# RichExplor/VIL_Fusion

Measured on AMD Instinct MI355X. Metric: sliding-window solve iters/sec (10 KF, ~5.5k factors) @1/2/4/8 GPU vs CPU, higher is better.
Workload: dtype f64

## Files before the change

### vil_fusion_amd/csrc/vilf_api.hip

```cpp
#include <hip/hip_runtime.h>
#include <string>
#include <vector>
#include <cstring>
#include <cstdio>
#include <cmath>
#include <algorithm>
#include <chrono>
#include <cstdlib>
#include <thread>
#include <atomic>
#include <type_traits>
#include "vilf_internal.hpp"
#include "vilf_kernels.hpp"
#include "vilf_sort.hpp"

namespace {

int class_plan(const vilf_window_in &in, int *cls, int *cstart, int *ccount) {
    int pcount[VB_NPAIR] = {0};
    for (int f = 0; f < in.n_features; f++) {
        const int s = in.feature_start_frame[f], n = in.feature_obs_offset[f + 1] - in.feature_obs_offset[f];
        for (int k = 1; k < n; k++) { const int j = s + k; pcount[j * (j - 1) / 2 + s]++; }
    }
    int order[VB_NPAIR], load[4] = {0, 0, 0, 0};
    for (int p = 0; p < VB_NPAIR; p++) order[p] = p;
    std::stable_sort(order, order + VB_NPAIR, [&](int a, int b) { return pcount[a] > pcount[b]; });
    for (int k = 0; k < VB_NPAIR; k++) { const int p = order[k]; int best = 0; for (int c = 1; c < 4; c++) if (load[c] < load[best]) best = c; cls[p] = best; load[best] += pcount[p]; }
    int pos[4] = {0, 0, 0, 0};
    for (int p = 0; p < VB_NPAIR; p++) { cstart[p] = pos[cls[p]]; ccount[p] = pcount[p]; pos[cls[p]] += pcount[p]; }
    const int longest = std::max(std::max(pos[0], pos[1]), std::max(pos[2], pos[3]));
    return VB_CHUNK * std::max(1, (longest + VB_CLS - 1) / VB_CLS);
}

void quat_from_R(const double *m, double *q ) {
    double t = m[0] + m[4] + m[8];
    if (t > 0) {
        t = std::sqrt(t + 1.0); q[3] = 0.5 * t; t = 0.5 / t;
        q[0] = (m[7] - m[5]) * t; q[1] = (m[2] - m[6]) * t; q[2] = (m[3] - m[1]) * t;
    } else {
        int i = 0;
        if (m[4] > m[0]) i = 1;
        if (m[8] > m[4 * i]) i = 2;
        int j = (i + 1) % 3, k = (j + 1) % 3;
        t = std::sqrt(m[4 * i] - m[4 * j] - m[4 * k] + 1.0);
        q[i] = 0.5 * t; t = 0.5 / t;
        q[3] = (m[3 * k + j] - m[3 * j + k]) * t;
        q[j] = (m[3 * j + i] + m[3 * i + j]) * t;
        q[k] = (m[3 * k + i] + m[3 * i + k]) * t;
    }
}
void quat_to_R(const double *q, double *R) {
    const double x = q[0], y = q[1], z = q[2], w = q[3];
    const double tx = 2 * x, ty = 2 * y, tz = 2 * z, twx = tx * w, twy = ty * w, twz = tz * w;
    const double txx = tx * x, txy = ty * x, txz = tz * x, tyy = ty * y, tyz = tz * y, tzz = tz * z;
    R[0] = 1 - (tyy + tzz); R[1] = txy - twz; R[2] = txz + twy;
    R[3] = txy + twz; R[4] = 1 - (txx + tzz); R[5] = tyz - twx;
    R[6] = txz - twy; R[7] = tyz + twx; R[8] = 1 - (txx + tyy);
}

}

struct UpJob { const char *src; char *dst; unsigned long long bytes; };
struct UpJobs { int n; UpJob j[40]; };
__global__ __launch_bounds__(256) void k_copy_spans(UpJobs jobs) {
    const UpJob jb = jobs.j[blockIdx.y];
    const unsigned long long stride = (unsigned long long)gridDim.x * 256, i0 = (unsigned long long)blockIdx.x * 256 + threadIdx.x;
    if ((((unsigned long long)jb.src | (unsigned long long)jb.dst) & 15ull) == 0) {
        const unsigned long long n16 = jb.bytes >> 4;
        const uint4 *s4 = reinterpret_cast<const uint4 *>(jb.src); uint4 *d4 = reinterpret_cast<uint4 *>(jb.dst);
        for (unsigned long long i = i0; i < n16; i += stride) d4[i] = s4[i];
        if (blockIdx.x == 0) for (unsigned long long i = (n16 << 4) + threadIdx.x; i < jb.bytes; i += 256) jb.dst[i] = jb.src[i];
    } else if ((((unsigned long long)jb.src | (unsigned long long)jb.dst) & 7ull) == 0) {
        const unsigned long long n8 = jb.bytes >> 3;
        const unsigned long long *s8 = reinterpret_cast<const unsigned long long *>(jb.src); unsigned long long *d8 = reinterpret_cast<unsigned long long *>(jb.dst);
        for (unsigned long long i = i0; i < n8; i += stride) d8[i] = s8[i];
        if (blockIdx.x == 0) for (unsigned long long i = (n8 << 3) + threadIdx.x; i < jb.bytes; i += 256) jb.dst[i] = jb.src[i];
    } else for (unsigned long long i = i0; i < jb.bytes; i += stride) jb.dst[i] = jb.src[i];
}

extern "C" const char *vilf_version(void) { return "vilfusion-hip 0.1 (gfx950)"; }

extern "C" void vilf_default_options(vilf_options *o) {
    std::memset(o, 0, sizeof(*o));
    o->window_size = 10;
    o->max_num_iterations = 8;
    o->max_solver_time = -1.0;
    o->focal_length = 460.0;
    o->cauchy_a = 1.0;
    o->G[2] = 9.81007;
    o->estimate_extrinsic = 0; o->estimate_td = 0; o->use_lidar_const = 1;
    const double ric[9] = {0.00781297, -0.0042792, 0.99996, -0.999859, -0.014868, 0.00774856, 0.0148343, -0.99988, -0.00439476};
    const double tic[3] = {1.1439, -0.312718, 0.726546};
    const double rcl[9] = {7.027555e-03, -9.999753e-01, 2.599616e-05, -2.254837e-03, -4.184312e-05, -9.999975e-01, 9.999728e-01, 7.027479e-03, -2.255075e-03};
    const double tcl[3] = {-7.137748e-03, -7.482656e-02, -3.336324e-01};
    double q[4], n;
    quat_from_R(ric, q); n = std::sqrt(q[0] * q[0] + q[1] * q[1] + q[2] * q[2] + q[3] * q[3]); for (double &v : q) v /= n; quat_to_R(q, o->RIC);
    quat_from_R(rcl, q); n = std::sqrt(q[0] * q[0] + q[1] * q[1] + q[2] * q[2] + q[3] * q[3]); for (double &v : q) v /= n; quat_to_R(q, o->RCL);
    for (int i = 0; i < 3; i++) { o->TIC[i] = tic[i]; o->TCL[i] = tcl[i]; }
    o->TR = 0; o->ROW = 370; o->init_depth = 5.0;
    o->edge_leaf_size = 0.4; o->surf_leaf_size = 0.8; o->huber_a = 0.1;
    o->s2m_outer_iterations = 2; o->s2m_max_iterations = 4; o->s2m_crop_half = 100.0;
}

extern "C" int vilf_create(const vilf_options *opts, int device, void *hip_stream, vilf_handle **out) {
    if (!opts || !out) return VILF_ERR_INVALID_ARGUMENT;
    *out = nullptr;
    int ndev = 0;
    if (hipGetDeviceCount(&ndev) != hipSuccess || ndev <= 0) return VILF_ERR_NO_GPU;
    if (device < 0 || device >= ndev) return VILF_ERR_INVALID_ARGUMENT;
    if (opts->window_size < 1 || opts->window_size > 4096) return VILF_ERR_UNSUPPORTED;
    vilf_handle *h = new vilf_handle();
    h->opts = *opts;
    h->device = device;
    if (hipSetDevice(device) != hipSuccess) { delete h; return VILF_ERR_DEVICE; }
// ... 122 lines not shown
    if (dirty.empty()) return VILF_OK;
    h->prior_backup_valid = false; h->prior_restore_needed = false;
    for (int w : dirty) {
        const vilf_prior &p = h->priors[w];
        h->prior_dev_newer[w] = 0;
        if (p.valid) for (int i = 0; i < p.n_blocks; i++) if (p.block_id[i] > 2 * VB_NF + (h->opts.estimate_td ? 1 : 0)) { h->err = "prior touches feature blocks (or Td without estimate_td): unsupported"; return VILF_ERR_UNSUPPORTED; }
        char dense_w = 0;
        if (p.valid) for (int i = 0; i < p.n_blocks; i++) if (p.block_id[i] > VB_NF && p.block_id[i] < 2 * VB_NF) dense_w = 1;
        if ((int)h->prior_dense.size() <= w) h->prior_dense.resize(w + 1, 0);
        h->prior_dense_count += dense_w - h->prior_dense[w]; h->prior_dense[w] = dense_w;
    }
    h->solve_dense_fallback = h->prior_dense_count > 0;
    auto fill = [&](const vilf_prior &p, int *hd, double *x0) {
        std::memset(hd, 0, VB_PRIOR_HDR * sizeof(int)); std::memset(x0, 0, VB_PRIOR_X0_LD * sizeof(double));
        if (!p.valid) return;
        hd[0] = 1; hd[1] = p.n; hd[2] = p.n_blocks; hd[75] = p.m;
        for (int i = 0; i < p.n_blocks; i++) {
            hd[3 + i] = p.block_id[i]; hd[27 + i] = p.block_size[i]; hd[51 + i] = p.block_idx[i];
            for (int k = 0; k < 9; k++) x0[i * 9 + k] = p.block_x0[i][k];
        }
    };
    if ((int)dirty.size() * 4 > B) {
        std::vector<int> hdr((size_t)B * VB_PRIOR_HDR, 0);
        std::vector<double> x0((size_t)B * VB_PRIOR_X0_LD, 0.0), J((size_t)B * VB_PRIOR_LD * VB_PRIOR_LD, 0.0), r((size_t)B * VB_PRIOR_LD, 0.0);
        if ((int)dirty.size() < B) {
            { int rcp = pull_device_priors(h); if (rcp != VILF_OK) return rcp; }
            for (int w = 0; w < B; w++) h->prior_dirty[w] = 1;
        }
        for (int w = 0; w < B; w++) {
            const vilf_prior &p = h->priors[w];
            fill(p, &hdr[(size_t)w * VB_PRIOR_HDR], &x0[(size_t)w * VB_PRIOR_X0_LD]);
            if (!p.valid) continue;
            std::memcpy(&J[(size_t)w * VB_PRIOR_LD * VB_PRIOR_LD], p.linearized_jacobians, sizeof(double) * p.n * p.n);
            std::memcpy(&r[(size_t)w * VB_PRIOR_LD], p.linearized_residuals, sizeof(double) * p.n);
        }
        HIPCHECK(h, hipMemcpyAsync(h->d[D_PHDR].p, hdr.data(), hdr.size() * sizeof(int), hipMemcpyHostToDevice, h->stream));
        HIPCHECK(h, hipMemcpyAsync(h->d[D_PX0].p, x0.data(), x0.size() * sizeof(double), hipMemcpyHostToDevice, h->stream));
        HIPCHECK(h, hipMemcpyAsync(h->d[D_PJ].p, J.data(), J.size() * sizeof(double), hipMemcpyHostToDevice, h->stream));
        HIPCHECK(h, hipMemcpyAsync(h->d[D_PR].p, r.data(), r.size() * sizeof(double), hipMemcpyHostToDevice, h->stream));
        HIPCHECK(h, hipStreamSynchronize(h->stream));
    } else {
        for (int w : dirty) {
            const vilf_prior &p = h->priors[w];
            int hd[VB_PRIOR_HDR]; double x0[VB_PRIOR_X0_LD];
            fill(p, hd, x0);
            HIPCHECK(h, hipMemcpyAsync(h->d[D_PHDR].as<int>() + (size_t)w * VB_PRIOR_HDR, hd, sizeof(hd), hipMemcpyHostToDevice, h->stream));
            HIPCHECK(h, hipMemcpyAsync(h->d[D_PX0].as<double>() + (size_t)w * VB_PRIOR_X0_LD, x0, sizeof(x0), hipMemcpyHostToDevice, h->stream));
            if (p.valid) {
                HIPCHECK(h, hipMemcpyAsync(h->d[D_PJ].as<double>() + (size_t)w * VB_PRIOR_LD * VB_PRIOR_LD, p.linearized_jacobians, sizeof(double) * p.n * p.n, hipMemcpyHostToDevice, h->stream));
                HIPCHECK(h, hipMemcpyAsync(h->d[D_PR].as<double>() + (size_t)w * VB_PRIOR_LD, p.linearized_residuals, sizeof(double) * p.n, hipMemcpyHostToDevice, h->stream));
            }
            HIPCHECK(h, hipStreamSynchronize(h->stream));
        }
    }
    hipLaunchKernelGGL(k_prior_prep, dim3(B), dim3(VB_NT), PRIOR_PREP_LDS_BYTES, h->stream, h->batch, h->d[D_PH].as<double>(), h->d[D_PG].as<double>(), (unsigned)PRIOR_PREP_LDS_BYTES, (const int *)nullptr);
    HIPCHECK(h, hipGetLastError());
    for (int w = 0; w < B; w++) h->prior_dirty[w] = 0;
    h->prior_slots_valid = std::max(h->prior_slots_valid, B);
    return VILF_OK;
}

enum ArrayUse : uint8_t {
    A_WINDOW,
    A_WINDOW_TD,
    A_SMALL,
    A_PRIOR,
    A_WORK,
};
struct BatchDims { size_t B, F, O, C; bool est_td; };
struct ArrayRow {
    int id; size_t elem;
    int k, f, o, c;
    ArrayUse use;
    int twin = -1;
    int copies = 1;
    size_t per_window(const BatchDims &d) const { return elem * (k + f * d.F + o * d.O + c * d.C); }
    size_t bytes(const BatchDims &d) const { return use == A_WINDOW_TD && !d.est_td ? 8 : copies * d.B * per_window(d); }
    bool by_range(const BatchDims &d) const { return use == A_WINDOW || (use == A_WINDOW_TD && d.est_td); }
    bool uploaded(const BatchDims &d) const { return by_range(d) || use == A_SMALL; }
};
constexpr ArrayRow kBatchArrays[] = {
    {D_POSE, 8, VB_POSE_LD, 0, 0, 0, A_WINDOW, D_POSE0}, {D_SB, 8, VB_SB_LD, 0, 0, 0, A_WINDOW, D_SB0}, {D_FEAT, 8, 0, 1, 0, 0, A_WINDOW, D_FEAT0},
    {D_FSTART, 4, 0, 1, 0, 0, A_WINDOW}, {D_FNOBS, 4, 0, 1, 0, 0, A_WINDOW}, {D_FFAC0, 4, 0, 1, 0, 0, A_WINDOW}, {D_FCONST, 1, 0, 1, 0, 0, A_WINDOW}, {D_PSSLOT, 4, 0, 0, 0, 1, A_WINDOW},
    {D_FOBS0, 4, 0, 1, 0, 0, A_WINDOW_TD}, {D_PSOBS, 4, 0, 0, 0, 1, A_WINDOW_TD},
    {D_FACREC, 8, 0, 0, 0, 8, A_WINDOW}, {D_IMU, 8, VB_IMU_LD, 0, 0, 0, A_WINDOW}, {D_LIDAR, 8, VB_LIDAR_LD, 0, 0, 0, A_WINDOW}, {D_COV, 8, VB_COV_LD, 0, 0, 0, A_WINDOW},
    {D_OBSV, 8, 0, 0, 2, 0, A_WINDOW_TD}, {D_OBSTD, 8, 0, 0, 1, 0, A_WINDOW_TD}, {D_OBSROW, 8, 0, 0, 1, 0, A_WINDOW_TD},
    {D_NFEAT, 4, 1, 0, 0, 0, A_SMALL}, {D_NFAC, 4, 1, 0, 0, 0, A_SMALL}, {D_EX, 8, VB_EX_LD, 0, 0, 0, A_SMALL}, {D_GR0, 8, 9, 0, 0, 0, A_SMALL}, {D_GP0, 8, 3, 0, 0, 0, A_SMALL},
    {D_PAIROFF, 4, VB_PTAB, 0, 0, 0, A_SMALL}, {D_MFLAG, 4, 1, 0, 0, 0, A_SMALL}, {D_TD, 8, 1, 0, 0, 0, A_SMALL},
    {D_PHDR, 4, VB_PRIOR_HDR, 0, 0, 0, A_PRIOR, D_PHDR0}, {D_PX0, 8, VB_PRIOR_X0_LD, 0, 0, 0, A_PRIOR, D_PX00}, {D_PJ, 8, VB_PRIOR_LD * VB_PRIOR_LD, 0, 0, 0, A_PRIOR, D_PJ0},
    {D_PR, 8, VB_PRIOR_LD, 0, 0, 0, A_PRIOR, D_PR0}, {D_PH, 8, VB_PRIOR_LD * VB_PRIOR_LD, 0, 0, 0, A_PRIOR, D_PH0}, {D_PG, 8, VB_PRIOR_LD, 0, 0, 0, A_PRIOR, D_PG0},
    {D_CPOSE, 8, VB_POSE_LD, 0, 0, 0, A_WORK}, {D_CSB, 8, VB_SB_LD, 0, 0, 0, A_WORK}, {D_CFEAT, 8, 0, 1, 0, 0, A_WORK}, {D_CF, 8, 0, 1, 0, 0, A_WORK},
    {D_FACW, 8, 0, 0, 0, VB_FACW, A_WORK}, {D_HPP, 8, 66 * 36, 0, 0, 0, A_WORK, -1, 2}, {D_W, 8, 0, VB_WLD, 0, 0, A_WORK, -1, 2}, {D_HF, 8, 0, 1, 0, 0, A_WORK, -1, 2},
    {D_GF, 8, 0, 1, 0, 0, A_WORK, -1, 2}, {D_IMUH, 8, 9000, 0, 0, 0, A_WORK, -1, 2}, {D_IMUG, 8, 300, 0, 0, 0, A_WORK, -1, 2}, {D_LIDH, 8, 1440, 0, 0, 0, A_WORK, -1, 2},
    {D_LIDG, 8, 120, 0, 0, 0, A_WORK, -1, 2}, {D_G, 8, VB_P, 0, 0, 0, A_WORK, -1, 2}, {D_DIAGH, 8, VB_P, 0, 0, 0, A_WORK, -1, 2}, {D_PAIRD, 8, VB_NPAIR * VB_PAIRD, 0, 0, 0, A_WORK, -1, 2},
    {D_SCALE, 8, VB_P, 1, 0, 0, A_WORK}, {D_DIAG, 8, VB_P, 1, 0, 0, A_WORK}, {D_GRAD, 8, VB_P, 1, 0, 0, A_WORK}, {D_GN, 8, VB_P, 1, 0, 0, A_WORK},
    {D_ST, sizeof(VbState), 1, 0, 0, 0, A_WORK}, {D_OPS, 8, VB_OUT3_LD, 0, 0, 0, A_WORK}, {D_ORS, 8, VB_OUTR_LD, 0, 0, 0, A_WORK}, {D_OVS, 8, VB_OUT3_LD, 0, 0, 0, A_WORK},
    {D_OBAS, 8, VB_OUT3_LD, 0, 0, 0, A_WORK}, {D_OBGS, 8, VB_OUT3_LD, 0, 0, 0, A_WORK}, {D_WORK, 8, 10 * 450, 0, 0, 0, A_WORK},
};
constexpr int upload_destinations() { int n = 0; for (const ArrayRow &r : kBatchArrays) if (r.use <= A_SMALL) n += 1 + (r.twin >= 0); return n; }
static_assert(upload_destinations() <= (int)(sizeof(UpJobs::j) / sizeof(UpJob)), "the staged upload hands every destination to ONE launch of k_copy_spans");
static size_t batch_array_bytes(int id, const BatchDims &d) { for (const ArrayRow &r : kBatchArrays) if (r.id == id) return r.bytes(d); return 0; }

static void bind_prior_pointers(vilf_handle *h) {
    VbBatch &b = h->batch;
    b.prior_hdr = h->d[D_PHDR].as<int>(); b.prior_x0 = h->d[D_PX0].as<double>(); b.prior_J = h->d[D_PJ].as<double>(); b.prior_r = h->d[D_PR].as<double>();
    b.prior_H = h->d[D_PH].as<double>(); b.prior_g = h->d[D_PG].as<double>();
}
static void swap_prior_sets(vilf_handle *h) {
    for (const ArrayRow &r : kBatchArrays) if (r.use == A_PRIOR) std::swap(h->d[r.id], h->d[r.twin]);
    bind_prior_pointers(h);
}
static void lidar_extrinsic(const vilf_options &o, VbBatch &b) {
    double M[9];
    for (int i = 0; i < 3; i++) for (int j = 0; j < 3; j++) M[3 * i + j] = o.RIC[3 * i] * o.RCL[j] + o.RIC[3 * i + 1] * o.RCL[3 + j] + o.RIC[3 * i + 2] * o.RCL[6 + j];
    quat_from_R(M, b.qil);
    for (int i = 0; i < 3; i++) b.til[i] = o.RIC[3 * i] * o.TCL[0] + o.RIC[3 * i + 1] * o.TCL[1] + o.RIC[3 * i + 2] * o.TCL[2] + o.TIC[i];
}
static void bind_batch_arrays(vilf_handle *h, const BatchDims &dm) {
    VbBatch &b = h->batch;
    std::memset(&b, 0, sizeof(b));
    const vilf_options &o = h->opts;
    b.B = (int)dm.B; b.w0 = 0; b.Fmax = (int)dm.F; b.Omax = (int)dm.O; b.FACmax = (int)dm.C;
    b.sqrt_info = o.focal_length / 1.5; b.cauchy_b = o.cauchy_a * o.cauchy_a;
    for (int i = 0; i < 3; i++) b.G[i] = o.G[i];
    lidar_extrinsic(o, b);
    b.use_lidar = o.use_lidar_const; b.max_iterations = o.max_num_iterations;
    b.min_relative_decrease = 1e-3; b.function_tolerance = 1e-6; b.gradient_tolerance = 1e-10; b.parameter_tolerance = 1e-8;
    b.min_radius = 1e-32; b.initial_radius = 1e4; b.min_lm_diagonal = 1e-6; b.max_lm_diagonal = 1e32;
    b.est_td = o.estimate_td ? 1 : 0; b.tr_over_row = o.TR / o.ROW; b.row_half = o.ROW / 2;
    DBuf *d = h->d;
    b.n_feat = d[D_NFEAT].as<int>(); b.n_fac = d[D_NFAC].as<int>(); b.pose = d[D_POSE].as<double>(); b.sb = d[D_SB].as<double>(); b.feat = d[D_FEAT].as<double>();
    b.cand_pose = d[D_CPOSE].as<double>(); b.cand_sb = d[D_CSB].as<double>(); b.cand_feat = d[D_CFEAT].as<double>();
    b.pose_init = d[D_POSE0].as<double>(); b.sb_init = d[D_SB0].as<double>(); b.feat_init = d[D_FEAT0].as<double>();
    b.ex = d[D_EX].as<double>(); b.gauge_R0 = d[D_GR0].as<double>(); b.gauge_P0 = d[D_GP0].as<double>(); b.td = d[D_TD].as<double>();
    b.f_start = d[D_FSTART].as<int>(); b.f_nobs = d[D_FNOBS].as<int>(); b.f_obs0 = d[D_FOBS0].as<int>(); b.f_fac0 = d[D_FFAC0].as<int>(); b.f_const = d[D_FCONST].as<uint8_t>();
    b.obs_vel = d[D_OBSV].as<double>(); b.obs_ctd = d[D_OBSTD].as<double>(); b.obs_row = d[D_OBSROW].as<double>(); b.ps_obs = d[D_PSOBS].as<int>(); b.ps_slot = d[D_PSSLOT].as<int>();
    b.pair_off = d[D_PAIROFF].as<int>(); b.facrec = d[D_FACREC].as<double>(); b.imu = d[D_IMU].as<double>(); b.lidar = d[D_LIDAR].as<double>();
    bind_prior_pointers(h);
    b.facw = d[D_FACW].as<double>(); b.Hpp = d[D_HPP].as<double>(); b.W = d[D_W].as<double>(); b.hf = d[D_HF].as<double>(); b.gf = d[D_GF].as<double>(); b.cf = d[D_CF].as<double>();
    b.imuH = d[D_IMUH].as<double>(); b.imug = d[D_IMUG].as<double>(); b.lidH = d[D_LIDH].as<double>(); b.lidg = d[D_LIDG].as<double>(); b.g = d[D_G].as<double>();
    b.diagH = d[D_DIAGH].as<double>(); b.pairD = d[D_PAIRD].as<double>(); b.scale = d[D_SCALE].as<double>(); b.diag = d[D_DIAG].as<double>(); b.grad = d[D_GRAD].as<double>(); b.gn = d[D_GN].as<double>();
    b.st = d[D_ST].as<VbState>(); b.out_Ps = d[D_OPS].as<double>(); b.out_Rs = d[D_ORS].as<double>(); b.out_Vs = d[D_OVS].as<double>(); b.out_Bas = d[D_OBAS].as<double>(); b.out_Bgs = d[D_OBGS].as<double>();
    b.sb_tab = d[D_SBTAB].as<int>();
}

namespace {
struct Lap {
    const bool on = std::getenv("VILF_DEBUG_TIMING") != nullptr;
    std::chrono::steady_clock::time_point t = std::chrono::steady_clock::now();
    void operator()(const char *what) { if (on) { const auto now = std::chrono::steady_clock::now(); fprintf(stderr, "[vilf_batch_upload] %-28s %.2f ms\n", what, std::chrono::duration<double, std::milli>(now - t).count()); t = now; } }
};
struct Upload {
    vilf_handle *h; const vilf_window_in *wins;
    int nthr;
    BatchDims dims;
    bool keep_inputs;
    char *image; size_t image_bytes;
    size_t at[D_COUNT], ld[D_COUNT];
    template <typename T> T *row(int id, int w) const { return reinterpret_cast<T *>(image + at[id] + (size_t)w * ld[id]); }
};
const char *check_window(const vilf_options &o, const vilf_window_in &in, int *mf) {
    if (in.n_frames != VB_NF) return "n_frames must be window_size + 1 = 11";
    if (in.n_features < 0 || in.n_features > VILF_MAX_FEATURES) return "n_features out of range";
    if (!in.para_pose || !in.para_speed_bias || !in.imu || (in.n_features && (!in.para_feature || !in.feature_const || !in.feature_start_frame || !in.feature_obs_offset || !in.obs_point)))
        return "null input array";
    if (o.use_lidar_const && !in.lidar) return "lidar constraints missing (use_lidar_const = 1)";
    if (o.estimate_td && in.n_features && (!in.obs_velocity || !in.obs_cur_td || !in.obs_row)) return "estimate_td needs obs_velocity / obs_cur_td / obs_row";
    if (in.n_obs < 0 || (in.n_features && (in.feature_obs_offset[0] != 0 || in.feature_obs_offset[in.n_features] != in.n_obs)) || (!in.n_features && in.n_obs != 0))
        return "feature_obs_offset must start at 0 and end at n_obs";
    *mf = 0;
    for (int f = 0; f < in.n_features; f++) {
        const int s = in.feature_start_frame[f], n = in.feature_obs_offset[f + 1] - in.feature_obs_offset[f];
        if (s < 0 || n < 2 || s + n > VB_NF) return "feature track outside the window";
        if (s == 0) (*mf)++;
    }
    return nullptr;
}
int plan_windows(Upload &u, int B) {
    vilf_handle *h = u.h;
    struct Local { int F = 4, O = 4, C = 4, M = 2; const char *err = nullptr; };
    std::vector<Local> loc(u.nthr);
    h->plans.resize(B);
    auto check = [&](int t) {
        Local &L = loc[t];
        for (int w = t; w < B; w += u.nthr) {
            const vilf_window_in &in = u.wins[w]; int mf = 0;
            if (const char *msg = check_window(h->opts, in, &mf)) { if (!L.err) L.err = msg; continue; }
            WindowPlan &pl = h->plans[w];
            pl.nslot = class_plan(in, pl.cls, pl.cstart, pl.ccount);
            L.C = std::max(L.C, pl.nslot); L.F = std::max(L.F, in.n_features); L.O = std::max(L.O, in.n_obs); L.M = std::max(L.M, MG_MD + mf + 1);
        }
    };
    std::vector<std::thread> pool;
    for (int t = 1; t < u.nthr; t++) pool.emplace_back(check, t);
    check(0);
    for (std::thread &th : pool) th.join();
    Local m;
    for (const Local &L : loc) {
        if (L.err) { h->err = L.err; return VILF_ERR_INVALID_ARGUMENT; }
        m.F = std::max(m.F, L.F); m.O = std::max(m.O, L.O); m.C = std::max(m.C, L.C); m.M = std::max(m.M, L.M);
    }
    u.dims = BatchDims{(size_t)B, (size_t)((m.F + 3) & ~3), (size_t)m.O, (size_t)((m.C + 63) & ~63), h->opts.estimate_td != 0};
    h->mg_Mcap = (m.M + 1) & ~1;
    return VILF_OK;
}
int reserve(Upload &u, Lap &lap) {
    vilf_handle *h = u.h;
    size_t off = 0;
    for (const ArrayRow &r : kBatchArrays) {
        const size_t bytes = r.bytes(u.dims);
        if (!h->d[r.id].ensure(bytes) || (r.twin >= 0 && r.use != A_PRIOR && !h->d[r.twin].ensure(bytes))) { h->err = "hipMalloc failed"; return VILF_ERR_DEVICE; }
        u.ld[r.id] = r.per_window(u.dims);
        if (!r.uploaded(u.dims)) continue;
        u.at[r.id] = off = (off + 63) & ~(size_t)63;
        off += u.dims.B * u.ld[r.id];
    }
    lap("validate + device buffers");
    u.image_bytes = (off + 63) & ~(size_t)63;
    if (!h->pin_up.ensure(off + 64)) { h->err = "hipHostMalloc failed (upload staging)"; return VILF_ERR_DEVICE; }
    u.image = static_cast<char *>(h->pin_up.p);
    h->h_nfeat.assign(u.dims.B, 0); h->h_ex.assign(u.dims.B * VB_EX_LD, 0.0); h->h_td.assign(u.dims.B, 0.0);
    h->own.clear(); h->own.resize(u.keep_inputs ? u.dims.B : 0);
    lap("host vectors");
    return VILF_OK;
}
void fill_imu_rec(const vilf_imu_preint &p, double *rec) {
    rec[0] = p.sum_dt;
    for (int i = 0; i < 3; i++) { rec[1 + i] = p.delta_p[i]; rec[8 + i] = p.delta_v[i]; rec[11 + i] = p.linearized_ba[i]; rec[14 + i] = p.linearized_bg[i]; }
    for (int i = 0; i < 4; i++) rec[4 + i] = p.delta_q[i];
    auto blk = [&](int off, int r0, int c0) { for (int i = 0; i < 3; i++) for (int j = 0; j < 3; j++) rec[off + 3 * i + j] = p.jacobian[(r0 + i) * 15 + c0 + j]; };
    blk(17, 0, 9); blk(26, 0, 12); blk(35, 3, 12); blk(44, 6, 9); blk(53, 6, 12);
}
void retain_window(OwnedWindow &o, const vilf_window_in &in) {
    const size_t F = in.n_features, O = in.n_obs;
    auto keep = [](auto &v, auto *&p, size_t n) { if (p) { v.assign(p, p + n); p = v.empty() ? nullptr : v.data(); } };
    o.in = in;
    keep(o.pose, o.in.para_pose, VB_POSE_LD); keep(o.sb, o.in.para_speed_bias, VB_SB_LD); keep(o.feat, o.in.para_feature, F); keep(o.fconst, o.in.feature_const, F);
    keep(o.fstart, o.in.feature_start_frame, F); keep(o.foff, o.in.feature_obs_offset, F + 1); keep(o.obs, o.in.obs_point, 3 * O);
    keep(o.vel, o.in.obs_velocity, 2 * O); keep(o.ctd, o.in.obs_cur_td, O); keep(o.row, o.in.obs_row, O);
    keep(o.imu, o.in.imu, VB_NF); keep(o.lidar, o.in.lidar, VB_NF); keep(o.gR0, o.in.gauge_R0, 9); keep(o.gP0, o.in.gauge_P0, 3);
}
void pack_window(const Upload &u, int w) {
    vilf_handle *h = u.h;
    const vilf_window_in &in = u.wins[w];
    const int F = in.n_features;
    *u.row<int>(D_NFEAT, w) = F; h->h_nfeat[w] = F; *u.row<int>(D_MFLAG, w) = in.marginalization_flag;
    *u.row<double>(D_TD, w) = in.para_td; h->h_td[w] = in.para_td;
    std::memcpy(u.row<double>(D_POSE, w), in.para_pose, VB_POSE_LD * 8); std::memcpy(u.row<double>(D_SB, w), in.para_speed_bias, VB_SB_LD * 8);
    std::memcpy(u.row<double>(D_EX, w), in.para_ex_pose, VB_EX_LD * 8); std::memcpy(&h->h_ex[(size_t)w * VB_EX_LD], in.para_ex_pose, VB_EX_LD * 8);
    if (in.gauge_R0) std::memcpy(u.row<double>(D_GR0, w), in.gauge_R0, 72); else quat_to_R(in.para_pose + 3, u.row<double>(D_GR0, w));
    std::memcpy(u.row<double>(D_GP0, w), in.gauge_P0 ? in.gauge_P0 : in.para_pose, 24);
    if (u.dims.est_td && in.n_obs) {
        std::memcpy(u.row<double>(D_OBSV, w), in.obs_velocity, (size_t)in.n_obs * 16);
        std::memcpy(u.row<double>(D_OBSTD, w), in.obs_cur_td, (size_t)in.n_obs * 8);
        std::memcpy(u.row<double>(D_OBSROW, w), in.obs_row, (size_t)in.n_obs * 8);
    }
    if (u.keep_inputs) retain_window(h->own[w], in);
    const WindowPlan &pl = h->plans[w];
    *u.row<int>(D_NFAC, w) = pl.nslot;
    int cur[VB_NPAIR], *po = u.row<int>(D_PAIROFF, w);
    for (int p = 0; p < VB_NPAIR; p++) { po[2 * p] = pl.cstart[p]; po[2 * p + 1] = pl.ccount[p] | (pl.cls[p] << 24); cur[p] = pl.cstart[p]; }
    po[2 * VB_NPAIR] = 0; po[2 * VB_NPAIR + 1] = 0;
    double *facrec = u.row<double>(D_FACREC, w), *feat = u.row<double>(D_FEAT, w);
    int *psslot = u.row<int>(D_PSSLOT, w), *fstart = u.row<int>(D_FSTART, w), *fnobs = u.row<int>(D_FNOBS, w), *ffac0 = u.row<int>(D_FFAC0, w);
    int *psobs = u.dims.est_td ? u.row<int>(D_PSOBS, w) : nullptr, *fobs0 = u.dims.est_td ? u.row<int>(D_FOBS0, w) : nullptr;
    uint8_t *fconst = u.row<uint8_t>(D_FCONST, w);
    const unsigned long long nul = 1ULL << 17;
    for (int g = 0; g < pl.nslot; g++) { double *rec = &facrec[(size_t)g * 8]; for (int k = 0; k < 7; k++) rec[k] = 0.0; std::memcpy(&rec[7], &nul, 8); psslot[g] = 0; if (psobs) psobs[g] = 0; }
    int q = 0;
    for (int f = 0; f < F; f++) {
        const int o0 = in.feature_obs_offset[f], o1 = in.feature_obs_offset[f + 1], s = in.feature_start_frame[f], cst = in.feature_const[f] ? 1 : 0;
        feat[f] = in.para_feature[f]; fconst[f] = (uint8_t)cst; fstart[f] = s; fnobs[f] = o1 - o0; ffac0[f] = q;
        if (fobs0) fobs0[f] = o0;
        const double *pi = in.obs_point + 3 * (size_t)o0;
        for (int t = o0 + 1; t < o1; t++, q++) {
            const int j = s + (t - o0), p = j * (j - 1) / 2 + s, pos = VB_SLOT(pl.cls[p], cur[p]);
            cur[p]++; psslot[pos] = q;
            if (psobs) psobs[pos] = t;
            double *rec = &facrec[(size_t)pos * 8]; const double *pj = in.obs_point + 3 * (size_t)t;
            for (int k = 0; k < 3; k++) { rec[k] = pi[k]; rec[3 + k] = pj[k]; }
            const unsigned long long a = (unsigned long long)(unsigned)f | ((unsigned long long)(unsigned)q << 32);
            const unsigned long long b2 = (unsigned long long)s | ((unsigned long long)j << 8) | ((unsigned long long)cst << 16);
            std::memcpy(&rec[6], &a, 8); std::memcpy(&rec[7], &b2, 8);
        }
    }
    for (int k = 0; k < 10; k++) {
        const vilf_imu_preint &p = in.imu[k + 1];
        double *rec = u.row<double>(D_IMU, w) + (size_t)k * IMU_REC, *l = u.row<double>(D_LIDAR, w) + 7 * k;
        fill_imu_rec(p, rec);
        rec[287] = (p.sum_dt > 10.0) ? 0.0 : 1.0;
        std::memcpy(u.row<double>(D_COV, w) + 225 * k, p.covariance, 225 * 8);
        if (in.lidar) { const vilf_lidar_constraint &c = in.lidar[k + 1]; for (int i = 0; i < 4; i++) l[i] = c.q[i]; for (int i = 0; i < 3; i++) l[4 + i] = c.t[i]; }
        else for (int i = 0; i < 7; i++) l[i] = (i == 3) ? 1.0 : 0.0;
    }
}
int copy_windows(const Upload &u, int w0, int w1) {
    vilf_handle *h = u.h;
    for (const ArrayRow &r : kBatchArrays) {
        if (!r.by_range(u.dims)) continue;
        const size_t at = (size_t)w0 * u.ld[r.id], bytes = (size_t)(w1 - w0) * u.ld[r.id];
        const char *src = u.image + u.at[r.id] + at;
        HIPCHECK(h, hipMemcpyAsync(h->d[r.id].as<char>() + at, src, bytes, hipMemcpyHostToDevice, h->stream));
        if (r.twin >= 0) HIPCHECK(h, hipMemcpyAsync(h->d[r.twin].as<char>() + at, src, bytes, hipMemcpyHostToDevice, h->stream));
    }
    return VILF_OK;
}
int pack_and_copy(const Upload &u, bool staged, Lap &lap) {
    vilf_handle *h = u.h;
    const int B = (int)u.dims.B;
    const int nchunk = (u.nthr > 1 && B >= 256) ? 4 : 1, csz = (B + nchunk - 1) / nchunk;
    std::atomic<int> next(0);
    std::vector<std::atomic<int>> done(nchunk); for (auto &d : done) d.store(0);
    auto packer = [&]() { for (int w = next.fetch_add(1); w < B; w = next.fetch_add(1)) { pack_window(u, w); done[w / csz].fetch_add(1, std::memory_order_release); } };
    std::vector<std::thread> pool;
    if (u.nthr <= 1) packer();
    else for (int t = 0; t < u.nthr; t++) pool.emplace_back(packer);
    int rc = VILF_OK;
    for (int c = 0; c < nchunk && !staged; c++) {
        const int w0 = c * csz, w1 = std::min(B, w0 + csz);
        while (done[c].load(std::memory_order_acquire) < w1 - w0) std::this_thread::yield();
        if (rc == VILF_OK) rc = copy_windows(u, w0, w1);
    }
    for (std::thread &th : pool) th.join();
    if (rc != VILF_OK) return rc;
    lap("pack + per-window copies");
    if (staged) {
        UpJobs jobs; jobs.n = 0; size_t big = 0;
        for (const ArrayRow &r : kBatchArrays) {
            if (!r.uploaded(u.dims)) continue;
            const size_t bytes = u.dims.B * u.ld[r.id];
            const char *src = h->d[D_UPSTAGE].as<char>() + u.at[r.id];
            jobs.j[jobs.n++] = UpJob{src, h->d[r.id].as<char>(), bytes};
            if (r.twin >= 0) jobs.j[jobs.n++] = UpJob{src, h->d[r.twin].as<char>(), bytes};
            big = std::max(big, bytes);
        }
        HIPCHECK(h, hipMemcpyAsync(h->d[D_UPSTAGE].p, u.image, u.image_bytes, hipMemcpyHostToDevice, h->stream));
        hipLaunchKernelGGL(k_copy_spans, dim3((unsigned)std::max<size_t>(1, std::min<size_t>(64, big / 65536 + 1)), (unsigned)jobs.n), dim3(256), 0, h->stream, jobs);
        HIPCHECK(h, hipGetLastError());
    } else {
        for (const ArrayRow &r : kBatchArrays)
            if (r.use == A_SMALL) HIPCHECK(h, hipMemcpyAsync(h->d[r.id].p, u.image + u.at[r.id], u.dims.B * u.ld[r.id], hipMemcpyHostToDevice, h->stream));
        if (!h->async_upload) HIPCHECK(h, hipStreamSynchronize(h->stream));
    }
    lap("small arrays + sync");
    return VILF_OK;
}
int build_scatter_tables(vilf_handle *h) {
    auto perm = [](int a, int l) { return l < 6 ? 6 * a + l : 66 + 9 * a + (l - 6); };
    auto off1 = [](int r, int c) { const int tr = r >> 4, tc = c >> 4; if (tr < tc) return 0; return (tr * (tr + 1) / 2 + tc) * 256 + 16 * (r & 15) + ((c & 15) ^ (r & 15)) + 1; };
    auto off = [&](int r, int c) { return off1(r, c) | (r << 15) | (c << 23); };
    std::vector<int> li(9000), ll(1440), lv(2 * 2376);
    for (int k = 0; k < 10; k++) {
        for (int e = 0; e < 900; e++) { const int p = e / 30, q = e % 30; li[900 * k + e] = off(perm(k + p / 15, p % 15), perm(k + q / 15, q % 15)); }
        for (int e = 0; e < 144; e++) { const int p = e / 12, q = e % 12; ll[144 * k + e] = off(perm(k + p / 6, p % 6), perm(k + q / 6, q % 6)); }
    }
    for (int t = 0; t < 2376; t++) {
        const int blk = t / 36, e = t % 36, l = e / 6, m = e % 6;
        int a = 0; while ((a + 1) * (a + 2) / 2 <= blk) a++;
        const int bb = blk - a * (a + 1) / 2, r = 6 * a + l, c = 6 * bb + m;
        lv[2 * t] = off(r, c);
        lv[2 * t + 1] = (a != bb && (r >> 4) == (c >> 4)) ? off1(c, r) : 0;
    }
    if (!h->d[D_LUTI].ensure(li.size() * 4) || !h->d[D_LUTL].ensure(ll.size() * 4) || !h->d[D_LUTV].ensure(lv.size() * 4)) return VILF_ERR_DEVICE;
    HIPCHECK(h, vilf_copy_sync(h, h->d[D_LUTI].p, li.data(), li.size() * 4, hipMemcpyHostToDevice));
    HIPCHECK(h, vilf_copy_sync(h, h->d[D_LUTL].p, ll.data(), ll.size() * 4, hipMemcpyHostToDevice));
    HIPCHECK(h, vilf_copy_sync(h, h->d[D_LUTV].p, lv.data(), lv.size() * 4, hipMemcpyHostToDevice));
    h->luts_ready = true;
    return VILF_OK;
}

}

extern "C" int vilf_batch_upload(vilf_handle *h, int B, const vilf_window_in *wins) {
    if (!h || B <= 0 || !wins) return VILF_ERR_INVALID_ARGUMENT;
    Lap lap;
    HIPCHECK(h, hipSetDevice(h->device));
    if (h->upload_inflight) { HIPCHECK(h, hipStreamSynchronize(h->stream)); h->upload_inflight = false; }
    const bool keep_priors = h->resident && B <= h->prior_slots_valid;
    if (!keep_priors) { int rcp = pull_device_priors(h); if (rcp != VILF_OK) return rcp; }
    Upload u{};
    u.h = h; u.wins = wins; u.keep_inputs = h->opts.estimate_extrinsic || h->opts.estimate_td;
    u.nthr = B >= 64 ? (int)std::max(1u, std::min(16u, std::thread::hardware_concurrency())) : 1;
    int rc = plan_windows(u, B);
    if (rc != VILF_OK) return rc;
    h->B = B; h->resident = false;
    if ((int)h->priors.size() < B) { vilf_prior z; std::memset(&z, 0, sizeof(z)); h->priors.resize(B, z); }
    if (!keep_priors) { h->prior_dirty.assign(h->priors.size(), 1); h->prior_dev_newer.assign(h->priors.size(), 0); h->prior_slots_valid = 0; }
    h->prior_dirty.resize(h->priors.size(), 1); h->prior_dev_newer.resize(h->priors.size(), 0);
    if ((rc = reserve(u, lap)) != VILF_OK) return rc;
    const bool staged = u.nthr <= 1 && u.image_bytes <= ((size_t)64 << 20) && !std::getenv("VILF_NO_STAGED_UPLOAD") && h->d[D_UPSTAGE].ensure(u.image_bytes + 4096);
    if ((rc = pack_and_copy(u, staged, lap)) != VILF_OK) return rc;
    bind_batch_arrays(h, u.dims);
    if (getenv("VILF_DEBUG_STAMPS")) { if (!h->d[D_DBG].ensure(3 * 32 * 8)) return VILF_ERR_DEVICE; hipMemsetAsync(h->d[D_DBG].p, 0, 3 * 32 * 8, h->stream); h->batch.dbg = h->d[D_DBG].as<long long>(); }
    HIPCHECK(h, hipMemsetAsync(h->d[D_W].p, 0, batch_array_bytes(D_W, u.dims), h->stream));
    if (!h->luts_ready && (rc = build_scatter_tables(h)) != VILF_OK) return rc;
    h->batch.lut_imu = h->d[D_LUTI].as<int>(); h->batch.lut_lid = h->d[D_LUTL].as<int>(); h->batch.lut_vis = h->d[D_LUTV].as<int>();
    const int nimu = B * 10;
    hipLaunchKernelGGL(k_imu_prep, dim3((nimu + 3) / 4), dim3(IMU_PREP_NT), 0, h->stream, nimu, h->d[D_COV].as<double>(), h->d[D_WORK].as<double>(), h->d[D_IMU].as<double>());
    HIPCHECK(h, hipGetLastError());
    if ((rc = upload_priors(h)) != VILF_OK) return rc;
    hipLaunchKernelGGL(k_reset, dim3(B), dim3(VB_NT), 0, h->stream, h->batch, 0);
    HIPCHECK(h, hipGetLastError());
    if (h->async_upload || (h->defer_upload_sync && staged)) h->upload_inflight = true;
    else HIPCHECK(h, hipStreamSynchronize(h->stream));
    h->resident = true;
    return VILF_OK;
}

extern "C" int vilf_debug_sort_pairs(vilf_handle *h, const void *keys, const int *vals, size_t n, int bits, int key64, void *keys_out, int *vals_out) {
    if (!h || !keys || !vals || !keys_out || !vals_out || n == 0) return VILF_ERR_INVALID_ARGUMENT;
    const size_t kb = key64 ? 8 : 4, tb = vilf_sort_temp_bytes(n, kb);
    void *dk = nullptr, *dk2 = nullptr, *dv = nullptr, *dv2 = nullptr, *dt = nullptr;
    int rc = VILF_OK;
    if (hipMalloc(&dk, n * kb) != hipSuccess || hipMalloc(&dk2, n * kb) != hipSuccess || hipMalloc(&dv, n * 4) != hipSuccess || hipMalloc(&dv2, n * 4) != hipSuccess || hipMalloc(&dt, tb) != hipSuccess) rc = VILF_ERR_DEVICE;
    if (rc == VILF_OK && (hipMemcpyAsync(dk, keys, n * kb, hipMemcpyHostToDevice, h->stream) != hipSuccess || hipMemcpyAsync(dv, vals, n * 4, hipMemcpyHostToDevice, h->stream) != hipSuccess)) rc = VILF_ERR_DEVICE;
    if (rc == VILF_OK) {
        const int r = key64 ? vilf_sort_pairs_u64(h->stream, dt, tb, (const unsigned long long *)dk, (unsigned long long *)dk2, (const int *)dv, (int *)dv2, n, bits)
                            : vilf_sort_pairs_u32(h->stream, dt, tb, (const unsigned *)dk, (unsigned *)dk2, (const int *)dv, (int *)dv2, n, bits);
        if (r != 0) rc = VILF_ERR_DEVICE;
    }
    if (rc == VILF_OK && (hipMemcpyAsync(keys_out, dk2, n * kb, hipMemcpyDeviceToHost, h->stream) != hipSuccess || hipMemcpyAsync(vals_out, dv2, n * 4, hipMemcpyDeviceToHost, h->stream) != hipSuccess ||
                          hipStreamSynchronize(h->stream) != hipSuccess)) rc = VILF_ERR_DEVICE;
    hipFree(dk); hipFree(dk2); hipFree(dv); hipFree(dv2); hipFree(dt);
    return rc;
}
extern "C" int vilf_debug_lds_bytes(vilf_handle *h, int out3[3]) {
    if (!h || !out3) return VILF_ERR_INVALID_ARGUMENT;
    out3[0] = VB_LIN_LDS_BYTES; out3[1] = SB_LDS_BYTES; out3[2] = std::max(VB_LIN_LDS_BYTES, SB_LDS_BYTES);
    return VILF_OK;
}
extern "C" int vilf_debug_stamps(vilf_handle *h, long long *out96) {
    if (!h || !h->batch.dbg) return VILF_ERR_INVALID_ARGUMENT;
    HIPCHECK(h, vilf_copy_sync(h, out96, h->batch.dbg, 96 * 8, hipMemcpyDeviceToHost));
    return VILF_OK;
}

extern "C" int vilf_batch_rewind(vilf_handle *h) {
    if (!h || !h->resident) return VILF_ERR_INVALID_ARGUMENT;
    hipLaunchKernelGGL(k_reset, dim3(h->B), dim3(VB_NT), 0, h->stream, h->batch, 1);
    HIPCHECK(h, hipGetLastError());
    if ((h->opts.estimate_extrinsic || h->opts.estimate_td) && (int)h->own.size() == h->B) {
        for (int w = 0; w < h->B; w++) { std::memcpy(&h->h_ex[(size_t)w * VB_EX_LD], h->own[w].in.para_ex_pose, VB_EX_LD * 8); h->h_td[w] = h->own[w].in.para_td; }
        HIPCHECK(h, hipMemcpyAsync(h->d[D_EX].p, h->h_ex.data(), (size_t)h->B * VB_EX_LD * 8, hipMemcpyHostToDevice, h->stream));
        HIPCHECK(h, hipMemcpyAsync(h->d[D_TD].p, h->h_td.data(), (size_t)h->B * 8, hipMemcpyHostToDevice, h->stream));
    }
    if (h->prior_restore_needed && h->prior_backup_valid) {
        swap_prior_sets(h);
        for (int w = 0; w < h->B; w++) { h->prior_dev_newer[w] = 1; h->prior_dirty[w] = 0; }
        h->prior_restore_needed = false;
    }
    return VILF_OK;
}

static void solve_time_resolve(vilf_handle *h) {
    if (!h->solve_time_pending) return;
    float ms = 0;
    if (hipEventElapsedTime(&ms, h->ev0, h->ev1) == hipSuccess) h->last_solve_usec = ms * 1000.0;
    h->solve_time_pending = false;
}
extern "C" int vilf_batch_solve(vilf_handle *h, int sync) {
    if (!h || !h->resident) return VILF_ERR_INVALID_ARGUMENT;
    HIPCHECK(h, hipSetDevice(h->device));
    if (h->opts.estimate_extrinsic || h->opts.estimate_td) {
        if ((int)h->own.size() != h->B) { h->err = "batch inputs not retained"; return VILF_ERR_INVALID_ARGUMENT; }
        { int rc = upload_priors(h); if (rc != VILF_OK) return rc; }
        const auto t0 = std::chrono::steady_clock::now();
        const size_t B = h->B;
        std::vector<double> bufP(B * VB_POSE_LD), bufS(B * VB_SB_LD), bufF(B * (h->batch.Fmax + 4)), Ps(B * VB_OUT3_LD), Rs(B * VB_OUTR_LD), Vs(B * VB_OUT3_LD), Bas(B * VB_OUT3_LD), Bgs(B * VB_OUT3_LD);
        std::vector<vilf_window_out> outv(B);
        std::vector<const vilf_window_in *> inp(B);
        std::vector<vilf_window_out *> outp(B);
        std::vector<int> slot1(B);
        for (size_t w = 0; w < B; w++) {
            vilf_window_out &out = outv[w];
            std::memset(&out, 0, sizeof(out));
            out.para_pose = &bufP[w * VB_POSE_LD]; out.para_speed_bias = &bufS[w * VB_SB_LD]; out.para_feature = &bufF[w * (h->batch.Fmax + 4)];
            out.Ps = &Ps[w * VB_OUT3_LD]; out.Rs = &Rs[w * VB_OUTR_LD]; out.Vs = &Vs[w * VB_OUT3_LD]; out.Bas = &Bas[w * VB_OUT3_LD]; out.Bgs = &Bgs[w * VB_OUT3_LD];
            inp[w] = &h->own[w].in; outp[w] = &out; slot1[w] = (int)w + 1;
        }
        const int rc = vilf_lw_group_solve(h, h->B, inp.data(), outp.data(), slot1.data());
        if (rc < 0) return rc;
        h->last_solve_usec = std::chrono::duration<double, std::micro>(std::chrono::steady_clock::now() - t0).count();
        h->solve_time_pending = false;
        (void)sync;
        return VILF_OK;
    }
    { int rc = upload_priors(h); if (rc != VILF_OK) return rc; }
    const dim3 grid(h->B), block(VB_NT);
    const bool dense = (h->solve_dense_fallback && !h->prior_restore_needed) || std::getenv("VILF_SOLVE_DENSE") != nullptr;
    const bool prof = h->profiling != 0;
    if (prof && h->prof_used.size() > 4096) { const int rcf = vilf_prof_flush(h); if (rcf != VILF_OK) return rcf; }
// ... 596 lines not shown
```

### vil_fusion_amd/csrc/vilf_batch.hpp

```cpp
#pragma once
#include <stdint.h>

#define VB_NF 11
#define VB_P 165
#define VB_NPOSE 66
#define VB_NPAIR 55
#define VB_PAIRD 120
#define VB_FACW 8
#define VB_WLD 80
#define VB_XLD 13
#define VB_CLS 56
#define VB_CHUNK (4 * VB_CLS)
#define VB_LIN_LDS_DOUBLES (2 * VB_CHUNK * VB_XLD + 8)
#define VB_LIN_SHARED_BYTES 33024
#define VB_LIN_LDS_BYTES (VB_LIN_LDS_DOUBLES * 8 + VB_LIN_SHARED_BYTES)
#define VB_PTAB (2 * VB_NPAIR + 2)
#define VB_SLOT(cls, x) (VB_CHUNK * ((x) / VB_CLS) + VB_CLS * (cls) + ((x) % VB_CLS))
#define VB_NT 256
#define VB_NTILE 11
#define VB_NPAD 176
#define VB_PRIOR_HDR 80
#define VB_PRIOR_LD 160
#define IMU_REC 288
#define IMU_SQRT 62
// ... 31 lines not shown
struct VbState {
    double x_cost, cand_cost, initial_cost;
    double radius, mu, alpha, dogleg_step_norm;
    double x_norm, gradient_max_norm;
    double grad_sqnorm;
    double Jg2;
    double gy;
    double gn_sqnorm;
    double mu_used;
    double model_cost_change, relative_decrease;
    int iteration, num_successful, num_linear_solves, num_consecutive_invalid;
    int termination, done, reuse, need_linearize, solve_failed, scaling_ready, started;
    int dev_error;
    int ws;
};

#define MG_RWP 113
#define MG_FCH 16
#define MG_MD 21
#define MG_NK 96
#define MG_ND (MG_MD + MG_NK)
#define MG_MROW 42
#define MG_PAIRM 400
#define QL_RCAP 12288
#define QL_ICAP 768
#define QL_LPW 16
#define MG_SLOTS 1024
#define MG_GCH 80
#define MG_PTRI 210
#define MG_MLDS 136
#define MG_INFO 128
#define MG_SWEEPS 24
struct VbMarg {
    int Mcap;
    double init_depth;
    const int *mflag;
    int *info;
    int *f0rank;
    double *st_pose, *st_sb, *st_feat, *st_ex;
    double *Mbuf;
    double *Hd, *gd;
    double *Wf;
    double *hfm, *gfm;
    double *Amm;
    double *X;
    double *rot;
    int pool, pool_round;
    double *lam;
    double *Ar, *br;
    double *qlV, *qlD, *qlLog;
    int *qlIt, *qlInfo;
    int *prior_hdr_out;
    double *prior_x0_out, *prior_J_out, *prior_r_out;
    double *prior_H_out, *prior_g_out;
};

#define VB_SPLIT_MAXCH 12
#define VB_SPLIT_MAXB 8
#define VB_SPLIT_CTL 64
#define VB_SPLIT_CNT 52
#define VB_SPLIT_SPIN_MAX (1 << 20)
#define VB_SPLIT_CARRY (VB_SPLIT_MAXCH * 4 * 64 * 8)
#define VB_SPLIT_DBL (VB_SPLIT_CARRY + (VB_SPLIT_MAXCH + 3) * 256)
struct VbBatch {
    int B, Fmax, Omax, FACmax;
    int w0;
    int *live_ctl, *live_buf; int live_it;
    int split_nr; int *split_ctl; double *split_buf;
    int split_fault;
    int split_gen;
    double sqrt_info, cauchy_b, G[3];
    double qil[4], til[3];
    int use_lidar, max_iterations;
    double min_relative_decrease, function_tolerance, gradient_tolerance, parameter_tolerance;
    double min_radius, initial_radius, min_lm_diagonal, max_lm_diagonal;
    const int *n_feat, *n_fac;
    double *pose, *sb, *feat;
    double *cand_pose, *cand_sb, *cand_feat;
    const double *pose_init, *sb_init, *feat_init;
    const double *ex;
    const double *gauge_R0, *gauge_P0;
    const int *f_start, *f_nobs, *f_obs0, *f_fac0;
    const uint8_t *f_const;
    const double *obs;
    const double *obs_vel, *obs_ctd, *obs_row;
    double *td;
    int est_td; double tr_over_row, row_half;
    const int *ps_feat, *ps_obs, *ps_slot;
    const int *pair_off;
    const double *facrec;
    const double *imu, *lidar;
    const int *sb_tab;
    const int *lut_imu, *lut_lid, *lut_vis;
    double *cf;
    const int *prior_hdr;
    const double *prior_x0, *prior_J, *prior_r, *prior_H, *prior_g;
    double *facw, *Hpp, *W, *hf, *gf, *imuH, *imug, *lidH, *lidg, *g;
    double *pairD;
    double *diagH;
    double *scale, *diag, *grad, *gn;
    VbState *st;
    double *out_Ps, *out_Rs, *out_Vs, *out_Bas, *out_Bgs;
    long long *dbg;
};
```

### vil_fusion_amd/csrc/vilf_internal.hpp

```cpp
#pragma once
#include <hip/hip_runtime.h>
#include <string>
#include <vector>
#include <cstring>
#include "../../include/vilfusion.h"
#include "vilf_batch.hpp"

struct DBuf {
    void *p = nullptr;
    size_t cap = 0;
    bool ensure(size_t bytes) {
        if (bytes <= cap) return true;
        if (p) hipFree(p);
        p = nullptr; cap = 0;
        size_t want = bytes + bytes / 8 + 256;
        if (hipMalloc(&p, want) != hipSuccess) return false;
        cap = want;
        return true;
    }
    void release() { if (p) hipFree(p); p = nullptr; cap = 0; }
    template <typename T> T *as() { return reinterpret_cast<T *>(p); }
};

enum {
    D_NFEAT, D_NFAC, D_POSE, D_SB, D_FEAT, D_CPOSE, D_CSB, D_CFEAT, D_POSE0, D_SB0, D_FEAT0, D_EX, D_GR0, D_GP0,
    D_FSTART, D_FNOBS, D_FOBS0, D_FFAC0, D_FCONST, D_PSOBS, D_PSSLOT, D_PAIROFF, D_IMU, D_LIDAR,
    D_PHDR, D_PX0, D_PJ, D_PR, D_PH, D_PG, D_FACW, D_HPP, D_W, D_HF, D_GF, D_IMUH, D_IMUG, D_LIDH, D_LIDG, D_G, D_DIAGH,
    D_SCALE, D_DIAG, D_GRAD, D_GN, D_ST, D_OPS, D_ORS, D_OVS, D_OBAS, D_OBGS, D_COV, D_WORK, D_HOOK, D_DBG, D_LUTI, D_LUTL, D_LUTV,
    D_MFLAG, D_MINFO, D_MF0, D_MSTP, D_MSTS, D_MSTF, D_MSTE, D_MBUF, D_MHD, D_MGD, D_MWF, D_MHF, D_MGF, D_MAMM, D_MX, D_MROT, D_MLAM, D_MAR, D_MBR, D_QLV, D_QLD, D_QLLOG, D_QLIT, D_QLINFO,
    D_PAIRD, D_FACREC, D_CF, D_STAMPS, D_LIVE, D_SBTAB, D_SPLITC, D_SPLITB, D_UPSTAGE, D_DNSTAGE, D_OBSV, D_OBSTD, D_OBSROW, D_TD, D_PHDR0, D_PX00, D_PJ0, D_PR0, D_PH0, D_PG0,
    D_COUNT
};

struct PinBuf {
    void *p = nullptr; size_t cap = 0;
    bool ensure(size_t bytes) {
        if (bytes <= cap) return true;
        if (p) hipHostFree(p);
        p = nullptr; cap = 0;
        const size_t want = bytes + bytes / 8 + 4096;
        if (hipHostMalloc(&p, want, hipHostMallocDefault) != hipSuccess) return false;
        std::memset(p, 0, want);
        cap = want;
        return true;
    }
    void release() { if (p) hipHostFree(p); p = nullptr; cap = 0; }
};

struct S2B;
struct FeatCtx;
struct PgCtx;
struct LwCtx;
struct ScCtx;
struct IcpCtx;
struct TrackCtx;
struct StartupCtx;
struct SfmCtx;
struct BaCtx;
struct TriCtx;

struct OwnedWindow {
    vilf_window_in in;
    std::vector<double> pose, sb, feat, obs, vel, ctd, row, gR0, gP0;
    std::vector<uint8_t> fconst;
    std::vector<int32_t> fstart, foff;
    std::vector<vilf_imu_preint> imu;
    std::vector<vilf_lidar_constraint> lidar;
};

struct WindowPlan { int cls[VB_NPAIR], cstart[VB_NPAIR], ccount[VB_NPAIR], nslot; };
struct vilf_handle {
    vilf_options opts;
    int device = 0;
    hipStream_t stream = nullptr;
    bool own_stream = false;
    std::string err;
    DBuf d[D_COUNT];
    VbBatch batch;
    int B = 0;
    bool resident = false;
    bool async_upload = false, upload_inflight = false;
    bool defer_upload_sync = false;
    std::vector<vilf_prior> priors;
    std::vector<char> prior_dirty;
    std::vector<char> prior_dense;
    int prior_dense_count = 0;
    std::vector<char> prior_dev_newer;
    int prior_slots_valid = 0;
    bool prior_backup_valid = false;
    bool prior_restore_needed = false;
    int mg_Mcap = 0;
    VbMarg marg;
    std::vector<int> h_nfeat, h_nframes;
    std::vector<double> h_ex, h_td;
    std::vector<OwnedWindow> own;
    PinBuf pin_up, pin_down;
    bool luts_ready = false;
    hipEvent_t ev0 = nullptr, ev1 = nullptr;
    int profiling = 0;
    struct ProfSpan { hipEvent_t a, b; double *ms; long *cnt; };
    std::vector<ProfSpan> prof_pending;
    std::vector<hipEvent_t> prof_used, prof_free;
    hipEvent_t wait_ev = nullptr;
    void *stamp_pinned = nullptr; size_t stamp_cap = 0; hipEvent_t stamp_ev = nullptr;
    double kernel_ms[4] = {0, 0, 0, 0};
    long kernel_launches[4] = {0, 0, 0, 0};
    std::vector<hipEvent_t> s2m_ev;
    std::vector<int> s2m_groups;
    double marg_ms[4] = {0, 0, 0, 0};
    long marg_launches[4] = {0, 0, 0, 0};
    double s2m_ms[8] = {0, 0, 0, 0, 0, 0, 0, 0};
    long s2m_launches[8] = {0, 0, 0, 0, 0, 0, 0, 0};
    std::vector<WindowPlan> plans;
// ... 68 lines not shown
```

### vil_fusion_amd/csrc/vilf_kernels.hip

```cpp
#include "vilf_device.hpp"
#include "vilf_kernels.hpp"

using namespace vd;

typedef double double4_t __attribute__((ext_vector_type(4)));
typedef double double2_t __attribute__((ext_vector_type(2)));

#define NT VB_NT
#ifdef VILF_STAMPS
#define STAMP(kid, i) do { if (b.dbg && blockIdx.x == 0 && threadIdx.x == 0) b.dbg[(kid) * 32 + (i)] = __builtin_readcyclecounter(); } while (0)
#define TICK() __builtin_readcyclecounter()
#else
#define STAMP(kid, i) do { } while (0)
#define TICK() 0LL
#endif
#define LSTAMP(i) do { if (JAC) STAMP(0, i); } while (0)
__device__ __forceinline__ int pair_index(int i, int j) { return j * (j - 1) / 2 + i; }
__device__ __forceinline__ int perm_index(int a, int l) { return l < 6 ? 6 * a + l : 66 + 9 * a + (l - 6); }
__device__ __forceinline__ void unperm(int p, int &a, int &l) {
    if (p < 66) { a = p / 6; l = p - 6 * a; } else { int q = p - 66; a = q / 9; l = 6 + q - 9 * a; }
}
__device__ __forceinline__ int tile_index(int ta, int tb) { return ta * (ta + 1) / 2 + tb; }
#define TIX(r, c) (16 * (r) + ((c) ^ (r)))

// ... 512 lines not shown
            for (int q = 0; q < 4; q++) {
                const int p = 16 * ti + (lane >> 4) + 4 * q, c = 16 * tj + (lane & 15);
                if (p < 30 && c < 30) { imuH[900 * k + 30 * p + c] = acc[q]; if (ti != tj) imuH[900 * k + 30 * c + p] = acc[q]; }
                if (p == 30 && c < 30) imug[30 * k + c] = acc[q];
                if (p == 30 && c == 30) cost_local += 0.5 * acc[q];
            }
        }
        LSTAMP(10);
        double *lidH = b.lidH + ww * 1440, *lidg = b.lidg + ww * 120;
        if (do_lp) {
        for (int idx = tid; idx < 1440; idx += NT) {
            const int k = idx / 144, e = idx - 144 * k, p = e / 12, q = e - 12 * p;
            double s = 0;
            for (int row = 0; row < 6; row++) s += s_lidJ[72 * k + 12 * row + p] * s_lidJ[72 * k + 12 * row + q];
            lidH[idx] = s;
        }
        for (int idx = tid; idx < 120; idx += NT) {
            const int k = idx / 12, p = idx - 12 * k;
            double s = 0;
            for (int row = 0; row < 6; row++) s += s_lidJ[72 * k + 12 * row + p] * s_lidr[6 * k + row];
            lidg[idx] = s;
        }
        }
    }
    if (SPLIT && do_imu) scost[tid] = cost_local;
    if (SPLIT) cost_local = 0;
    if (do_lp && tid >= 64 && tid < 74) { const int k = tid - 64; double s = 0; for (int m = 0; m < 6; m++) s += s_lidr[6 * k + m] * s_lidr[6 * k + m]; cost_local += 0.5 * s; }
    LSTAMP(11);
    if (SPLIT && do_lp) { scost[256 + tid] = cost_local; cost_local = 0; }
    double gprior = 0;
    if (!SPLIT || do_lp) {
        double pcost;
        prior_products_j<(JAC && !SPLIT)>(b, w, s_dx, s_pcol, s_red, s_grad, tid, pcost, gprior);
        if (SPLIT) scost[512 + tid] = pcost; else cost_local += pcost;
    }
    LSTAMP(13);
    lds_barrier();
    if (tid == 0) s_X[2 * VB_CHUNK * VB_XLD] = 0.0;
    LSTAMP(4);
    const int *f_start = b.f_start + (size_t)w * FM;
    const uint8_t *f_const = b.f_const + (size_t)w * FM;
    const double *facrec = b.facrec + (size_t)w * FC * 8;
    double *facw = b.facw + (size_t)w * VB_FACW * FC;
    double *W = b.W + ww * FM * VB_WLD;
    long long t_eval = 0, t_sync1 = 0, t_mfma = 0, t_sync2 = 0, t_a = 0;
    int pe[4];
#pragma unroll
    for (int q4 = 0; q4 < 4; q4++) pe[q4] = pair_elem((lane >> 4) + 4 * q4, lane & 15);
    double4_t cacc = {0, 0, 0, 0}, cacc1 = {0, 0, 0, 0};
    unsigned long long mrem = cls_mask;
    if (!JAC) {
        for (int fac = tid; fac < nfac; fac += NT) {
            const double4_t *rp = reinterpret_cast<const double4_t *>(facrec + (size_t)fac * 8);
            const double4_t ra = rp[0], rb = rp[1];
            const double pts_i[3] = {ra[0], ra[1], ra[2]}, pts_j[3] = {ra[3], rb[0], rb[1]};
            const unsigned long long ia = __double_as_longlong(rb[2]), ib = __double_as_longlong(rb[3]);
            if ((ib >> 17) & 1) continue;
            const int f = (int)(ia & 0xffffffffu), fi = (int)(ib & 0xff), fj = (int)((ib >> 8) & 0xff);
            double r[2];
            projection_eval_pair<false>(s_pt + PT_LD * pair_index(fi, fj), s_ric, s_tic, pts_i, pts_j, feat[f], b.sqrt_info, r, nullptr, nullptr, nullptr);
            double rho0, sw;
            cauchy(r[0] * r[0] + r[1] * r[1], b.cauchy_b, rho0, sw);
            cost_local += 0.5 * rho0;
        }
    } else {
    const int c_begin = SPLIT ? role * VB_CHUNK : 0, c_end = SPLIT ? (do_vis ? min(nfac, (role + 1) * VB_CHUNK) : 0) : nfac;
    double4_t ra_n = {0, 0, 0, 0}, rb_n = {0, 0, 0, 0};
    double fv_n = 0;
    if (c_begin < c_end) {
        const double4_t *rp = reinterpret_cast<const double4_t *>(facrec + (size_t)min(c_begin + tid, nfac - 1) * 8);
        ra_n = rp[0]; rb_n = rp[1];
        fv_n = feat[(int)(__double_as_longlong(rb_n[2]) & 0xffffffffu)];
    }
    for (int c0 = c_begin; c0 < c_end; c0 += VB_CHUNK) {
        t_a = TICK();
        const int q = c0 + tid;
        double *x0 = s_X + (2 * min(tid, VB_CHUNK - 1)) * VB_XLD, *x1 = x0 + VB_XLD;
        const double4_t ra = ra_n, rb = rb_n;
        const double fv = fv_n;
        const unsigned long long ia = __double_as_longlong(rb[2]), ib = __double_as_longlong(rb[3]);
        if (tid >= VB_CHUNK) {
        } else if (q < nfac && !((ib >> 17) & 1)) {
            const double pts_i[3] = {ra[0], ra[1], ra[2]}, pts_j[3] = {ra[3], rb[0], rb[1]};
            const int f = (int)(ia & 0xffffffffu), slot = (int)(ia >> 32), fi = (int)(ib & 0xff), fj = (int)((ib >> 8) & 0xff);
            const bool fc = ((ib >> 16) & 1) != 0;
            double r[2], Ji[12], Jj[12], Jf[2];
            projection_eval_pair<true>(s_pt + PT_LD * pair_index(fi, fj), s_ric, s_tic, pts_i, pts_j, fv, b.sqrt_info, r, Ji, Jj, Jf);
            double rho0, sw;
            cauchy(r[0] * r[0] + r[1] * r[1], b.cauchy_b, rho0, sw);
            cost_local += 0.5 * rho0;
#pragma unroll
            for (int c = 0; c < 6; c++) { x0[c] = sw * Jj[c]; x0[6 + c] = sw * Ji[c]; x1[c] = sw * Jj[6 + c]; x1[6 + c] = sw * Ji[6 + c]; }
            x0[12] = sw * r[0]; x1[12] = sw * r[1];
            if (!fc) {
                const double jf0 = sw * Jf[0], jf1 = sw * Jf[1];
                double2_t *Wr = reinterpret_cast<double2_t *>(W + (size_t)f * VB_WLD + 6 * fj);
                double2_t *fw = reinterpret_cast<double2_t *>(facw + (size_t)slot * VB_FACW);
#pragma unroll
                for (int c = 0; c < 6; c += 2) {
                    Wr[c >> 1] = double2_t{x0[c] * jf0 + x1[c] * jf1, x0[c + 1] * jf0 + x1[c + 1] * jf1};
                    fw[c >> 1] = double2_t{x0[6 + c] * jf0 + x1[6 + c] * jf1, x0[7 + c] * jf0 + x1[7 + c] * jf1};
                }
                fw[3] = double2_t{jf0 * jf0 + jf1 * jf1, jf0 * x0[12] + jf1 * x1[12]};
            }
        } else {
#pragma unroll
            for (int c = 0; c < VB_XLD; c++) { x0[c] = 0; x1[c] = 0; }
        }
        { long long t_b = TICK(); t_eval += t_b - t_a; t_a = t_b; }
        lds_barrier();
        { long long t_b = TICK(); t_sync1 += t_b - t_a; t_a = t_b; }
        if (c0 + VB_CHUNK < c_end) {
            const double4_t *rp = reinterpret_cast<const double4_t *>(facrec + (size_t)min(c0 + VB_CHUNK + tid, nfac - 1) * 8);
            ra_n = rp[0]; rb_n = rp[1];
        }
        const int x0c = VB_CLS * (c0 / VB_CHUNK);
        if constexpr (SPLIT) {
            double *carry_out = sbuf + ((size_t)(role * 4 + wave) * 64 + lane) * 8;
            const double *carry_in = sbuf + ((size_t)(max(role, 1) * 4 - 4 + wave) * 64 + lane) * 8;
            int *flag_out = sctl + 1 + 4 * role + wave, *flag_in = sctl + 1 + 4 * max(role - 1, 0) + wave;
#pragma unroll 1
            for (int pass = 0; pass < 3; pass++) {
                unsigned long long m = cls_mask;
                while (m) {
                    const int p = __builtin_amdgcn_readfirstlane(__builtin_ctzll(m));
                    m &= m - 1;
                    const int pst = __builtin_amdgcn_readlane(my_pst, p), pcn_ = __builtin_amdgcn_readlane(my_pcn, p);
                    if (pst + pcn_ <= x0c) continue;
                    if (pst >= x0c + VB_CLS) break;
                    const bool in = pst < x0c, out = pst + pcn_ > x0c + VB_CLS;
                    if ((in ? 2 : (out ? 0 : 1)) != pass) continue;
                    double4_t acc = {0, 0, 0, 0}, acc1 = {0, 0, 0, 0};
                    if (in) {
                        int spins = 0;
                        bool got = false;
                        for (; spins < VB_SPLIT_SPIN_MAX; spins++) {
                            if (__hip_atomic_load(flag_in, __ATOMIC_ACQUIRE, __HIP_MEMORY_SCOPE_AGENT) == b.split_gen) { got = true; break; }
                            __builtin_amdgcn_s_sleep(1);
                        }
                        if (got) {
                            const double2_t *ci = reinterpret_cast<const double2_t *>(carry_in);
                            const double2_t c0_ = ci[0], c1_ = ci[1], c2_ = ci[2], c3_ = ci[3];
                            acc = double4_t{c0_[0], c0_[1], c1_[0], c1_[1]}; acc1 = double4_t{c2_[0], c2_[1], c3_[0], c3_[1]};
                        } else if (lane == 0) __hip_atomic_store(&st->dev_error, 1, __ATOMIC_RELAXED, __HIP_MEMORY_SCOPE_AGENT);
                    }
                    const int lo = max(pst, x0c), hi = min(pst + pcn_, x0c + VB_CLS);
                    const int r_lo = 2 * (VB_CLS * wave + lo - x0c), r_hi = 2 * (VB_CLS * wave + hi - x0c);
                    auto ld4 = [&](int r0, double *a) {
#pragma unroll
                        for (int u = 0; u < 4; u++) {
                            const int row = r0 + 4 * u + (lane >> 4);
                            a[u] = s_X[(row < r_hi && (lane & 15) < VB_XLD) ? row * VB_XLD + (lane & 15) : 2 * VB_CHUNK * VB_XLD];
                        }
                    };
                    double a[4], an[4];
                    ld4(r_lo, a);
                    for (int r0 = r_lo; r0 < r_hi; r0 += 16) {
                        ld4(r0 + 16, an);
                        acc = __builtin_amdgcn_mfma_f64_16x16x4f64(a[0], a[0], acc, 0, 0, 0);
                        acc1 = __builtin_amdgcn_mfma_f64_16x16x4f64(a[1], a[1], acc1, 0, 0, 0);
                        acc = __builtin_amdgcn_mfma_f64_16x16x4f64(a[2], a[2], acc, 0, 0, 0);
                        acc1 = __builtin_amdgcn_mfma_f64_16x16x4f64(a[3], a[3], acc1, 0, 0, 0);
#pragma unroll
                        for (int u = 0; u < 4; u++) a[u] = an[u];
                    }
                    if (out) {
                        double2_t *co = reinterpret_cast<double2_t *>(carry_out);
                        co[0] = double2_t{acc[0], acc[1]}; co[1] = double2_t{acc[2], acc[3]}; co[2] = double2_t{acc1[0], acc1[1]}; co[3] = double2_t{acc1[2], acc1[3]};
                        __threadfence();
                        if (lane == 0 && !(b.split_fault && role == 0)) __hip_atomic_store(flag_out, b.split_gen, __ATOMIC_RELEASE, __HIP_MEMORY_SCOPE_AGENT);
                    } else {
#pragma unroll
                        for (int q4 = 0; q4 < 4; q4++) if (pe[q4] >= 0) pd[p * VB_PAIRD + pe[q4]] = acc[q4] + acc1[q4];
                    }
                }
            }
        } else
        while (mrem) {
            const int p = __builtin_amdgcn_readfirstlane(__builtin_ctzll(mrem));
            const int pst = __builtin_amdgcn_readlane(my_pst, p), pcn_ = __builtin_amdgcn_readlane(my_pcn, p);
            if (pst >= x0c + VB_CLS) break;
            const int lo = max(pst, x0c), hi = min(pst + pcn_, x0c + VB_CLS);
            if (lo >= hi) { mrem &= mrem - 1; continue; }
            const int r_lo = 2 * (VB_CLS * wave + lo - x0c), r_hi = 2 * (VB_CLS * wave + hi - x0c);
            double4_t acc = (pst < x0c) ? cacc : double4_t{0, 0, 0, 0}, acc1 = (pst < x0c) ? cacc1 : double4_t{0, 0, 0, 0};
            auto ld4 = [&](int r0, double *a) {
#pragma unroll
                for (int u = 0; u < 4; u++) {
                    const int row = r0 + 4 * u + (lane >> 4);
                    a[u] = s_X[(row < r_hi && (lane & 15) < VB_XLD) ? row * VB_XLD + (lane & 15) : 2 * VB_CHUNK * VB_XLD];
                }
            };
            double a[4], an[4];
            ld4(r_lo, a);
            for (int r0 = r_lo; r0 < r_hi; r0 += 16) {
                ld4(r0 + 16, an);
                acc = __builtin_amdgcn_mfma_f64_16x16x4f64(a[0], a[0], acc, 0, 0, 0);
                acc1 = __builtin_amdgcn_mfma_f64_16x16x4f64(a[1], a[1], acc1, 0, 0, 0);
                acc = __builtin_amdgcn_mfma_f64_16x16x4f64(a[2], a[2], acc, 0, 0, 0);
                acc1 = __builtin_amdgcn_mfma_f64_16x16x4f64(a[3], a[3], acc1, 0, 0, 0);
#pragma unroll
                for (int u = 0; u < 4; u++) a[u] = an[u];
            }
            if (pst + pcn_ > x0c + VB_CLS) { cacc = acc; cacc1 = acc1; break; }
            else {
#pragma unroll
                for (int q4 = 0; q4 < 4; q4++) if (pe[q4] >= 0) pd[p * VB_PAIRD + pe[q4]] = acc[q4] + acc1[q4];
                mrem &= mrem - 1;
            }
        }
        { long long t_b = TICK(); t_mfma += t_b - t_a; t_a = t_b; }
        if (c0 + VB_CHUNK < c_end) fv_n = feat[(int)(__double_as_longlong(rb_n[2]) & 0xffffffffu)];
        lds_barrier();
        { long long t_b = TICK(); t_sync2 += t_b - t_a; t_a = t_b; }
    }
    __syncthreads();
    }
    if (JAC && b.dbg && blockIdx.x == 0 && tid == 0) { b.dbg[64 + 16] = t_eval; b.dbg[64 + 17] = t_sync1; b.dbg[64 + 18] = t_mfma; b.dbg[64 + 19] = t_sync2; }
    if (SPLIT) {
        if (do_vis) scost[(3 + role) * 256 + tid] = cost_local;
        if (!arrive()) return 2;
        if (!iteration_zero && tid == 0) step_bookkeeping();
        double c = 0;
        c += __builtin_nontemporal_load(scost + tid); c += __builtin_nontemporal_load(scost + 256 + tid); c += __builtin_nontemporal_load(scost + 512 + tid);
        for (int k = 0; k < NCH; k++) c += __builtin_nontemporal_load(scost + (3 + k) * 256 + tid);
        cost_local = c;
        __syncthreads();
        if (JAC) { double pc_unused; prior_products_j<true>(b, w, s_dx, s_pcol, s_red, s_grad, tid, pc_unused, gprior); }
    }
    double gmax = 0, xsq = 0;
    if (JAC) {
    LSTAMP(5);
#define PD(p, e) pd_get(pd, s_pcn, (p), (e))
    double v5[8]; int dst5[8];
    {
        static_assert(55 * 36 <= 8 * NT, "one pass of eight entries per thread");
#pragma unroll
        for (int k = 0; k < 8; k++) {
            const int t = min(tid + k * NT, 55 * 36 - 1), ob = t / 36, e = t - 36 * ob;
            int a = 1; while (a * (a + 1) / 2 <= ob) a++;
            const int bb = ob - a * (a - 1) / 2;
            v5[k] = PD(pair_index(bb, a), 36 + e);
            dst5[k] = (tid + k * NT < 55 * 36) ? 36 * (a * (a + 1) / 2 + bb) + e : -1;
        }
    }
    LSTAMP(6);
    {
        const int *f_nobs = b.f_nobs + (size_t)w * FM, *f_fac0 = b.f_fac0 + (size_t)w * FM;
        double *hf = b.hf + ww * FM, *gf = b.gf + ww * FM;
        for (int f = tid; f < F; f += NT) {
            if (f_const[f]) { hf[f] = 0; gf[f] = 0; continue; }
            const int n = f_nobs[f] - 1, f0 = f_fac0[f];
            double acc[8] = {0, 0, 0, 0, 0, 0, 0, 0};
            for (int t0 = 0; t0 < n; t0 += 4) {
                double v[4][8];
#pragma unroll
                for (int u = 0; u < 4; u++) {
                    const double2_t *rp = reinterpret_cast<const double2_t *>(facw + (size_t)(f0 + min(t0 + u, n - 1)) * VB_FACW);
#pragma unroll
                    for (int c = 0; c < 4; c++) { const double2_t q2 = rp[c]; v[u][2 * c] = q2[0]; v[u][2 * c + 1] = q2[1]; }
                }
#pragma unroll
                for (int u = 0; u < 4; u++) if (t0 + u < n) {
#pragma unroll
                    for (int c = 0; c < 8; c++) acc[c] += v[u][c];
                }
            }
            double *Wr = W + (size_t)f * VB_WLD;
#pragma unroll
            for (int c = 0; c < 6; c++) Wr[6 * f_start[f] + c] = acc[c];
            Wr[VB_NPOSE] = acc[7];
            hf[f] = acc[6]; gf[f] = acc[7];
        }
    }
    {
        double *Hpp = b.Hpp + ww * 66 * 36;
#pragma unroll
        for (int k = 0; k < 8; k++) if (dst5[k] >= 0) Hpp[dst5[k]] = v5[k];
        for (int t = tid; t < VB_NF * 36; t += NT) {
            const int a = t / 36, e = t - 36 * a;
            double v[VB_NF - 1], s = 0;
#pragma unroll
            for (int k = 0; k < VB_NF - 1; k++) v[k] = (k < a) ? PD(pair_index(min(k, a - 1), a), e) : PD(pair_index(a, k + 1), 72 + e);
#pragma unroll
            for (int k = 0; k < VB_NF - 1; k++) s += v[k];
            Hpp[36 * (a * (a + 1) / 2 + a) + e] = s;
        }
    }
    lds_barrier();
    LSTAMP(7);
    double *gout = b.g + ww * VB_P;
    if (tid < VB_P) {
        const int a = tid / 15, l = tid - 15 * a;
        const double *imug = b.imug + ww * 300, *lidg = b.lidg + ww * 120;
        double s = 0;
        if (l < 6) {
            double v[VB_NF - 1];
#pragma unroll
            for (int k = 0; k < VB_NF - 1; k++) v[k] = (k < a) ? PD(pair_index(min(k, a - 1), a), 108 + l) : PD(pair_index(a, k + 1), 114 + l);
#pragma unroll
            for (int k = 0; k < VB_NF - 1; k++) s += v[k];
            if (a >= 1) s += lidg[12 * (a - 1) + 6 + l];
            if (a <= 9) s += lidg[12 * a + l];
        }
        if (a >= 1) s += imug[30 * (a - 1) + 15 + l];
        if (a <= 9) s += imug[30 * a + l];
        const int pc = s_pcol[tid];
        s += gprior;
        const double *imuHg = b.imuH + ww * 9000, *lidHg = b.lidH + ww * 1440;
        double dg = 0;
        if (l < 6) {
            double v[VB_NF - 1];
#pragma unroll
            for (int k = 0; k < VB_NF - 1; k++) v[k] = (k < a) ? PD(pair_index(min(k, a - 1), a), 7 * l) : PD(pair_index(a, k + 1), 72 + 7 * l);
#pragma unroll
            for (int k = 0; k < VB_NF - 1; k++) dg += v[k];
            if (a >= 1) dg += lidHg[144 * (a - 1) + 13 * (6 + l)];
            if (a <= 9) dg += lidHg[144 * a + 13 * l];
        }
        if (a >= 1) dg += imuHg[900 * (a - 1) + 31 * (15 + l)];
        if (a <= 9) dg += imuHg[900 * a + 31 * l];
        if (pc >= 0) dg += b.prior_H[(size_t)w * VB_PRIOR_LD * VB_PRIOR_LD + (size_t)pc * (VB_PRIOR_LD + 1)];
        gout[tid] = s;
        s_grad[tid] = s;
        b.diagH[ww * VB_P + tid] = dg;
    }
    lds_barrier();
    if (tid < VB_NF) {
        const double *gp = s_grad + 15 * tid;
        double d[6] = {-gp[0], -gp[1], -gp[2], -gp[3], -gp[4], -gp[5]}, xp[7];
        pose_plus(s_pose + 7 * tid, d, xp);
        for (int k = 0; k < 7; k++) { gmax = fmax(gmax, fabs(s_pose[7 * tid + k] - xp[k])); xsq += s_pose[7 * tid + k] * s_pose[7 * tid + k]; }
        for (int k = 0; k < 9; k++) { gmax = fmax(gmax, fabs(gp[6 + k])); xsq += s_sb[9 * tid + k] * s_sb[9 * tid + k]; }
    }
    {
        const double *gf = b.gf + ww * FM;
        for (int f = tid; f < F; f += NT) if (!f_const[f]) { gmax = fmax(gmax, fabs(gf[f])); xsq += feat[f] * feat[f]; }
    }
    }
    LSTAMP(8);
    const double cost = block_sum(cost_local, s_red);
    const double gm = block_max(gmax, s_red);
    const double xs = block_sum(xsq, s_red);
    if (iteration_zero) {
        if (tid == 0 && iteration_zero != 2) { st->x_cost = cost; st->gradient_max_norm = gm; st->x_norm = sqrt(xs); st->need_linearize = 0; st->reuse = 0; st->initial_cost = cost; st->ws = 0; }
        LSTAMP(9);
        return 0;
    }
    const double step_norm = sqrt(block_sum(stepsq, s_red));
    int *s_acc = reinterpret_cast<int *>(s_red);
    if (tid == 0) {
// ... 6 lines not shown
            const double rd = (x_cost - cost) / st->model_cost_change;
            st->relative_decrease = rd;
            if (rd > b.min_relative_decrease) {
                accept = 1;
                if (rd < 0.25) st->radius *= 0.5;
                if (rd > 0.75) st->radius = fmax(st->radius, 3.0 * st->dogleg_step_norm);
                st->mu = fmax(1e-8, 2.0 * st->mu / 10.0);
                st->reuse = 0;
                st->num_successful += 1;
                st->x_cost = cost;
                if (JAC) { st->gradient_max_norm = gm; st->x_norm = sqrt(xs); st->ws = wset; }
            } else {
                st->radius *= 0.5;
                st->reuse = 1;
            }
        }
        s_acc[0] = accept;
        still_live();
    }
    lds_barrier();
    if (s_acc[0]) {
        if (tid < 77) pose_g[tid] = s_pose[tid];
        if (tid < 99) sb_g[tid] = s_sb[tid];
        for (int f = tid; f < F; f += NT) feat_x[f] = cfeat[f];
    }
    LSTAMP(9);
    return 0;
}
extern "C" __global__ __launch_bounds__(NT) void k_linearize(VbBatch b, int iteration_zero) { (void)linearize_body<true>(b, iteration_zero); }
extern "C" __global__ __launch_bounds__(NT) void k_linearize_last(VbBatch b) { (void)linearize_body<false>(b, 0); }
extern "C" __global__ __launch_bounds__(NT) void k_linearize_split(VbBatch b, int iteration_zero) { (void)linearize_body<true, true>(b, iteration_zero); }


__device__ __forceinline__ void lds_add(double *p, double v) { __hip_atomic_fetch_add(p, v, __ATOMIC_RELAXED, __HIP_MEMORY_SCOPE_WORKGROUP); }

__device__ bool potrf_tile_wave(double *T, double *s_invd, int lane) {
    const int r = lane & 15;
    double v[16];
#pragma unroll
    for (int c = 0; c < 16; c++) v[c] = T[TIX(r, c)];
    bool ok = true;
    double myinv = 1.0;
#pragma unroll
    for (int j = 0; j < 16; j++) {
        const double djj = readlane_f64(v[j], j);
        if (!(djj > 0.0)) ok = false;
        const double inv = rsqrt_h3(djj);
        const double lrj = v[j] * inv;
        v[j] = lrj;
        if (r == j) myinv = inv;
#pragma unroll
        for (int c = j + 1; c < 16; c++) {
            const double lcj = readlane_f64(lrj, c);
            v[c] -= lrj * lcj;
        }
    }
#pragma unroll
    for (int c = 0; c < 16; c++) if (lane < 16) T[TIX(r, c)] = (c <= r) ? v[c] : 0.0;
    if (lane < 16) s_invd[r] = myinv;
    return ok;
}

__device__ __forceinline__ void tile_add(double *s_T, int r, int c, double v) {
    const int tr = r >> 4, tc = c >> 4;
    if (tr >= tc) s_T[tile_index(tr, tc) * 256 + TIX(r & 15, c & 15)] += v;
}

#define SNW (SNT / 64)
__device__ __forceinline__ double block_sum_s(double v, double *s_red) {
    const int tid = threadIdx.x;
    v = vilf_wave_sum64(v);
    __syncthreads();
    if ((tid & 63) == 0) s_red[tid >> 6] = v;
    __syncthreads();
    double r = 0;
#pragma unroll
    for (int k = 0; k < SNW; k++) r += s_red[k];
    __syncthreads();
    return r;
}


template <int HALF>
__device__ __forceinline__ void schur_mfma(const double *W, int F, const double *s_cf, const double *s_scale, double *s_T, double *s_y, int lane, int wave) {
    constexpr int TA[15] = {0, 1, 1, 2, 2, 2, 3, 3, 3, 3, 4, 4, 4, 4, 4};
    constexpr int TB[15] = {0, 0, 1, 0, 1, 2, 0, 1, 2, 3, 0, 1, 2, 3, 4};
    constexpr int NP = HALF ? 7 : 8, PB = HALF ? 8 : 0;
    const int c16 = lane & 15, grp = wave >> 1, g4 = lane >> 4;
    const int nsteps = ((F + 3) & ~3) / 4;
    double *s_t = s_T + SOLVE_OFF_RED;
    double sc5[5];
#pragma unroll
    for (int t5 = 0; t5 < 5; t5++) { const int col = 16 * t5 + c16; sc5[t5] = (col < VB_NPOSE) ? s_scale[col] : (col <= VB_NPOSE + 1 ? 1.0 : 0.0); }
    double4_t acc[NP];
#pragma unroll
    for (int i = 0; i < NP; i++) acc[i] = double4_t{0, 0, 0, 0};
    double ra[5], rb[5], rc[5];
#define SCHUR_ISSUE(ST, R)                                                                                                         \
    {                                                                                                                              \
        const int st_ = min((ST), nsteps - 1);                                                                                     \
        const double *Wr_ = W + (size_t)(4 * st_ + g4) * VB_WLD + c16;                                                            \
        asm volatile("global_load_dwordx2 %0, %5, off\n\tglobal_load_dwordx2 %1, %5, off offset:128\n\t"                           \
                     "global_load_dwordx2 %2, %5, off offset:256\n\tglobal_load_dwordx2 %3, %5, off offset:384\n\t"                \
                     "global_load_dwordx2 %4, %5, off offset:512"                                                                  \
                     : "=&v"(R[0]), "=&v"(R[1]), "=&v"(R[2]), "=&v"(R[3]), "=&v"(R[4]) : "v"(Wr_) : "memory");                      \
    }
#define SCHUR_WAIT(N, R) asm volatile("s_waitcnt vmcnt(" #N ")" : "+v"(R[0]), "+v"(R[1]), "+v"(R[2]), "+v"(R[3]), "+v"(R[4]) : : "memory");
#define SCHUR_STEP(ST, R)                                                                                                          \
    {                                                                                                                              \
        const double c_ = s_cf[4 * (ST) + g4];                                                                                     \
        double u[5];                                                                                                               \
        _Pragma("unroll") for (int t5 = 0; t5 < 5; t5++) u[t5] = R[t5] * c_ * sc5[t5];                                             \
        _Pragma("unroll") for (int i = 0; i < NP; i++) acc[i] = __builtin_amdgcn_mfma_f64_16x16x4f64(u[TA[PB + i]], u[TB[PB + i]], acc[i], 0, 0, 0); \
    }
    asm volatile("s_waitcnt vmcnt(0)" ::: "memory");
    SCHUR_ISSUE(grp, ra) SCHUR_ISSUE(grp + 4, rb)
    for (int st = grp; st < nsteps; st += 12) {
        SCHUR_ISSUE(st + 8, rc) SCHUR_WAIT(10, ra) SCHUR_STEP(st, ra)
        if (st + 4 < nsteps) { SCHUR_ISSUE(st + 12, ra) SCHUR_WAIT(10, rb) SCHUR_STEP(st + 4, rb) }
        if (st + 8 < nsteps) { SCHUR_ISSUE(st + 16, rb) SCHUR_WAIT(10, rc) SCHUR_STEP(st + 8, rc) }
    }
    asm volatile("s_waitcnt vmcnt(0)" : "+v"(ra[0]), "+v"(ra[1]), "+v"(ra[2]), "+v"(ra[3]), "+v"(ra[4]), "+v"(rb[0]), "+v"(rb[1]), "+v"(rb[2]), "+v"(rb[3]), "+v"(rb[4]),
                                        "+v"(rc[0]), "+v"(rc[1]), "+v"(rc[2]), "+v"(rc[3]), "+v"(rc[4]) : : "memory");
#undef SCHUR_ISSUE
#undef SCHUR_WAIT
#undef SCHUR_STEP
    for (int gsel = 0; gsel < 4; gsel++) {
        if (grp == gsel) {
#pragma unroll
            for (int i = 0; i < NP; i++) {
                const int ta = TA[PB + i], tb = TB[PB + i];
                double *T = s_T + tile_index(ta, tb) * 256;
#pragma unroll
                for (int q = 0; q < 4; q++) {
                    const int rl = g4 + 4 * q, col = 16 * tb + c16;
                    if (col >= VB_NPOSE) continue;
                    if (ta < 4 || rl < 2) lds_add(&T[TIX(rl, c16)], -acc[i][q]);
                    else if (rl == 2) lds_add(&s_y[col], -acc[i][q]);
                    else if (rl == 3) lds_add(&s_t[col], -acc[i][q]);
                }
            }
        }
        __syncthreads();
    }
}

__device__ __forceinline__ void feature_dots(const double *W, int F, const double *s_sv , double *out, int tid) {
    const int lane = tid & 63, wave = __builtin_amdgcn_readfirstlane(tid >> 6), c16 = lane & 15, g = lane >> 4;
    double sv[5];
#pragma unroll
    for (int t5 = 0; t5 < 5; t5++) sv[t5] = s_sv[16 * t5 + c16];
    const int Fk4 = (F + 3) & ~3;
    double ra[5], rb[5], rc[5];
#define FD_ISSUE(F0, R)                                                                                                            \
    {                                                                                                                              \
        const double *Wr_ = W + (size_t)min((F0) + g, Fk4 - 1) * VB_WLD + c16;                                                    \
        asm volatile("global_load_dwordx2 %0, %5, off\n\tglobal_load_dwordx2 %1, %5, off offset:128\n\t"                           \
                     "global_load_dwordx2 %2, %5, off offset:256\n\tglobal_load_dwordx2 %3, %5, off offset:384\n\t"                \
                     "global_load_dwordx2 %4, %5, off offset:512"                                                                  \
                     : "=&v"(R[0]), "=&v"(R[1]), "=&v"(R[2]), "=&v"(R[3]), "=&v"(R[4]) : "v"(Wr_) : "memory");                      \
    }
#define FD_WAIT(N, R) asm volatile("s_waitcnt vmcnt(" #N ")" : "+v"(R[0]), "+v"(R[1]), "+v"(R[2]), "+v"(R[3]), "+v"(R[4]) : : "memory");
#define FD_STEP(F0, R)                                                                                                             \
    {                                                                                                                              \
        const int f = (F0) + g;                                                                                                    \
        double acc = 0;                                                                                                            \
        _Pragma("unroll") for (int t5 = 0; t5 < 5; t5++) acc += R[t5] * sv[t5];                                                    \
        if (!(f < F)) acc = 0;                                                                                                     \
        _Pragma("unroll") for (int o = 8; o > 0; o >>= 1) acc += __shfl_xor(acc, o, 64);                                           \
        if (c16 == 0 && f < F) out[f] = acc;                                                                                       \
    }
    constexpr int RS = 4 * SNW;
    asm volatile("s_waitcnt vmcnt(0)" ::: "memory");
    FD_ISSUE(4 * wave, ra) FD_ISSUE(4 * wave + RS, rb)
    for (int f0 = 4 * wave; f0 < F; f0 += 3 * RS) {
        FD_ISSUE(f0 + 2 * RS, rc) FD_WAIT(10, ra) FD_STEP(f0, ra)
        if (f0 + RS < F) { FD_ISSUE(f0 + 3 * RS, ra) FD_WAIT(10, rb) FD_STEP(f0 + RS, rb) }
        if (f0 + 2 * RS < F) { FD_ISSUE(f0 + 4 * RS, rb) FD_WAIT(10, rc) FD_STEP(f0 + 2 * RS, rc) }
    }
    asm volatile("s_waitcnt vmcnt(0)" : "+v"(ra[0]), "+v"(ra[1]), "+v"(ra[2]), "+v"(ra[3]), "+v"(ra[4]), "+v"(rb[0]), "+v"(rb[1]), "+v"(rb[2]), "+v"(rb[3]), "+v"(rb[4]),
                                        "+v"(rc[0]), "+v"(rc[1]), "+v"(rc[2]), "+v"(rc[3]), "+v"(rc[4]) : : "memory");
#undef FD_ISSUE
#undef FD_WAIT
#undef FD_STEP
}

extern "C" __global__ __launch_bounds__(SNT) void k_solve(VbBatch b) {
    const int w = vb_window(b), tid = threadIdx.x, lane = tid & 63, wave = __builtin_amdgcn_readfirstlane(tid >> 6);
    if (w < 0) return;
    VbState *st = b.st + w;
    extern __shared__ double s_dyn[];
    double *s_T = s_dyn + SOLVE_OFF_T, *s_g = s_dyn + SOLVE_OFF_G, *s_diag = s_dyn + SOLVE_OFF_DIAG, *s_scale = s_dyn + SOLVE_OFF_SCALE;
    double *s_y = s_dyn + SOLVE_OFF_Y, *s_invd = s_dyn + SOLVE_OFF_INVD, *s_v = s_dyn + SOLVE_OFF_V, *s_red = s_dyn + SOLVE_OFF_RED;
    double *s_cf = s_dyn + SOLVE_OFF_CF;
    int *s_rng = (int *)(s_dyn + SOLVE_OFF_RNG);
    __shared__ int s_pcol[VB_P], s_pinv[VB_PRIOR_LD];
    __shared__ double s_dx[VB_PRIOR_LD];
    __shared__ int s_flag[4];

    if (tid == 0) {
        const int done = st->done, iteration = st->iteration, reuse = st->reuse;
        const double gmn = st->gradient_max_norm, radius = st->radius;
        int go = 1;
        if (done) go = 0;
        else if (iteration >= b.max_iterations) { st->done = 1; st->termination = 0; go = 0; }
        else if (gmn <= b.gradient_tolerance) { st->done = 1; st->termination = 3; go = 0; }
        else if (radius <= b.min_radius) { st->done = 1; st->termination = 4; go = 0; }
        if (go) st->iteration = iteration + 1;
        s_flag[0] = go;
        s_flag[1] = go ? reuse : 1;
    }
    __syncthreads();
    if (!s_flag[0] || s_flag[1]) return;

    STAMP(1, 0);
    const int F = b.n_feat[w];
    const size_t FM = b.Fmax;
    const size_t ww = (size_t)st->ws * b.B + w;
    const double *Hpp = b.Hpp + ww * 66 * 36;
    const double *imuH = b.imuH + ww * 9000, *lidH = b.lidH + ww * 1440;
    const double *priorH = b.prior_H + (size_t)w * VB_PRIOR_LD * VB_PRIOR_LD;
    double *W = b.W + ww * FM * VB_WLD;
    const double *hf = b.hf + ww * FM, *gf = b.gf + ww * FM;
    const uint8_t *f_const = b.f_const + (size_t)w * FM;
    const int *f_start = b.f_start + (size_t)w * FM, *f_nobs = b.f_nobs + (size_t)w * FM;
    double *scale_g = b.scale + (size_t)w * (VB_P + FM), *diag_g = b.diag + (size_t)w * (VB_P + FM);
    double *grad_g = b.grad + (size_t)w * (VB_P + FM), *gn_g = b.gn + (size_t)w * (VB_P + FM);
    const double *g_in = b.g + ww * VB_P;
    const int *phdr = b.prior_hdr + (size_t)w * VB_PRIOR_HDR;
    const int pn = phdr[0] ? phdr[1] : 0;

    prior_setup(b, w, b.pose + (size_t)w * 77, b.sb + (size_t)w * 99, s_pcol, s_dx, tid);
    if (tid < VB_PRIOR_LD) s_pinv[tid] = -1;
    __syncthreads();
    if (tid < VB_P) { const int pc = s_pcol[tid]; if (pc >= 0) { const int a = tid / 15, l = tid - 15 * a; s_pinv[pc] = perm_index(a, l); } }
    const int scaling_ready = st->scaling_ready;
    double mu = st->mu;
    int tries = 0;
    bool solved = false;
    double Jg2 = 0, G2 = 0;
    double g2 = 0;
    if (tid < VB_NPAD) {
        double sc = 1.0, d = 1.0, gs = 0.0, vv = 0.0;
        if (tid < VB_P) {
            int a, l; unperm(tid, a, l);
            const double dh = b.diagH[ww * VB_P + 15 * a + l];
            if (scaling_ready) sc = scale_g[tid]; else { sc = 1.0 / (1.0 + sqrt(dh)); scale_g[tid] = sc; }
            d = sqrt(fmin(fmax(sc * sc * dh, b.min_lm_diagonal), b.max_lm_diagonal));
            gs = g_in[15 * a + l] * sc;
            diag_g[tid] = d;
            const double gr = gs / d;
            grad_g[tid] = gr;
            g2 = gr * gr;
            vv = gr / d;
        }
        s_scale[tid] = sc; s_diag[tid] = d; s_g[tid] = gs; s_v[tid] = vv;
    }
#pragma unroll
    for (int u = 0; u < 2; u++) {
        const int f = tid + u * SNT;
        if (f < F) {
            s_rng[f] = (6 * f_start[f]) | ((6 * (f_start[f] + f_nobs[f])) << 16);
            if (!f_const[f]) {
                const double hfv = hf[f], gfv = gf[f];
                double sf;
                if (scaling_ready) sf = scale_g[VB_P + f]; else { sf = 1.0 / (1.0 + sqrt(hfv)); scale_g[VB_P + f] = sf; }
                const double d = sqrt(fmin(fmax(sf * sf * hfv, b.min_lm_diagonal), b.max_lm_diagonal));
                diag_g[VB_P + f] = d;
                const double gr = sf * gfv / d;
                grad_g[VB_P + f] = gr;
                g2 += gr * gr;
            }
        }
    }
    __syncthreads();
    STAMP(1, 1);
    for (;;) {
        double part = 0;
        for (int i = tid; i < 66 * 256; i += SNT) s_T[i] = 0.0;
        __syncthreads();
        if (tid < VB_NPAD - VB_P) s_T[tile_index(10, 10) * 256 + TIX(5 + tid, 5 + tid)] = 1.0;
        {
            const int2 *lv = (const int2 *)b.lut_vis;
            for (int t0 = tid; t0 < 66 * 36; t0 += 5 * SNT) {
                double v[5]; int2 o[5];
#pragma unroll
                for (int u = 0; u < 5; u++) { const int t = min(t0 + u * SNT, 66 * 36 - 1); v[u] = Hpp[t]; o[u] = lv[t]; }
#pragma unroll
                for (int u = 0; u < 5; u++) {
                    if (t0 + u * SNT >= 66 * 36) continue;
                    const int r = (o[u].x >> 15) & 255, c = (o[u].x >> 23) & 255;
                    const double val = v[u] * s_scale[r] * s_scale[c];
                    const int off = (o[u].x & 0x7fff) - 1;
                    if (off >= 0) lds_add(&s_T[off], val);
                    if (o[u].y > 0) lds_add(&s_T[o[u].y - 1], val);
                    part += (((r / 6) != (c / 6)) ? 2.0 : 1.0) * s_v[r] * val * s_v[c];
                }
            }
        }
        __syncthreads();
        for (int par = 0; par < 2; par++) {
            for (int t0 = tid; t0 < 5 * 900; t0 += 5 * SNT) {
                double v[5]; int o[5];
#pragma unroll
                for (int u = 0; u < 5; u++) {
                    const int t = min(t0 + u * SNT, 5 * 900 - 1);
                    const int k2 = t / 900, src = 900 * (2 * k2 + par) + (t - 900 * k2);
                    o[u] = b.lut_imu[src]; v[u] = imuH[src];
                }
#pragma unroll
                for (int u = 0; u < 5; u++) {
                    if (t0 + u * SNT >= 5 * 900) continue;
                    const int r = (o[u] >> 15) & 255, c = (o[u] >> 23) & 255;
                    const double val = v[u] * s_scale[r] * s_scale[c];
                    const int off = (o[u] & 0x7fff) - 1;
                    if (off >= 0) lds_add(&s_T[off], val);
                    part += s_v[r] * val * s_v[c];
                }
            }
            __syncthreads();
            for (int t = tid; t < 5 * 144; t += SNT) {
                const int k2 = t / 144, src = 144 * (2 * k2 + par) + (t - 144 * k2);
                const int o0 = b.lut_lid[src];
                const int r = (o0 >> 15) & 255, c = (o0 >> 23) & 255;
                const double val = lidH[src] * s_scale[r] * s_scale[c];
                const int off = (o0 & 0x7fff) - 1;
                if (off >= 0) lds_add(&s_T[off], val);
                part += s_v[r] * val * s_v[c];
            }
            __syncthreads();
        }
        if (pn > 0) for (int t0 = tid; t0 < pn * pn; t0 += 6 * SNT) {
            double v[6]; int rr[6], cc[6];
#pragma unroll
            for (int u = 0; u < 6; u++) {
                const int t = min(t0 + u * SNT, pn * pn - 1);
                const int i = t / pn, j = t - pn * i;
                rr[u] = s_pinv[i]; cc[u] = s_pinv[j]; v[u] = priorH[i * VB_PRIOR_LD + j];
            }
#pragma unroll
            for (int u = 0; u < 6; u++) {
                const int r = rr[u], c = cc[u];
                if (t0 + u * SNT >= pn * pn || r < 0 || c < 0) continue;
                const double val = v[u] * s_scale[r] * s_scale[c];
                if ((r >> 4) >= (c >> 4)) lds_add(&s_T[tile_index(r >> 4, c >> 4) * 256 + TIX(r & 15, c & 15)], val);
                part += s_v[r] * val * s_v[c];
            }
        }
        __syncthreads();
        STAMP(1, 2);
        if (tries == 0) {
#pragma unroll
            for (int u = 0; u < 2; u++) {
                const int f = tid + u * SNT;
                if (f < F) {
                    double xf = 0.0;
                    if (!f_const[f]) {
                        const double sf = scale_g[VB_P + f], df = diag_g[VB_P + f], hfv = hf[f], gfv = gf[f];
                        const double vf = sf * gfv / (df * df);
                        part += sf * sf * hfv * vf * vf;
                        xf = vf * (sf * sf * hfv + mu * df * df) / sf;
                    }
                    W[(size_t)f * VB_WLD + VB_NPOSE + 1] = xf;
                }
            }
            __threadfence_block();
            G2 = block_sum_s(g2, s_red);
            Jg2 = block_sum_s(part, s_red);
        }
        STAMP(1, 3);
        if (tid < VB_P) { const int tt = tid >> 4, e = tid & 15; s_T[tile_index(tt, tt) * 256 + TIX(e, e)] += mu * s_diag[tid] * s_diag[tid]; }
#pragma unroll
        for (int u = 0; u < 2; u++) {
            const int f = tid + u * SNT;
            if (f < F) { double c = 0; if (!f_const[f]) { const double sf = scale_g[VB_P + f], df = diag_g[VB_P + f]; c = sf * rsqrt_nr(sf * sf * hf[f] + mu * df * df); } s_cf[f] = c; }
        }
        if (tid < VB_NPAD) s_y[tid] = s_g[tid];
        __syncthreads();
        STAMP(1, 4);
        for (int f = F + tid; f < ((F + 3) & ~3); f += SNT) s_cf[f] = 0.0;
        if (tid < 80) s_red[tid] = 0.0;
        __syncthreads();
        __threadfence_block();
        if (wave & 1) schur_mfma<1>(W, F, s_cf, s_scale, s_T, s_y, lane, wave); else schur_mfma<0>(W, F, s_cf, s_scale, s_T, s_y, lane, wave);
        if (tries == 0) {
            double cr = ((lane < VB_NPOSE) ? s_v[lane] * s_red[lane] : 0.0) + ((lane + 64 < VB_NPOSE) ? s_v[lane + 64] * s_red[lane + 64] : 0.0);
            cr = vilf_wave_sum64(cr);
            Jg2 -= 2.0 * cr;
            __syncthreads();
        }
        STAMP(1, 5);
        if (tid < VB_P) s_T[tile_index(10, tid >> 4) * 256 + TIX(5, tid & 15)] = s_y[tid];
        if (tid == 0) s_T[tile_index(10, 10) * 256 + TIX(5, 5)] = 1e250;
        __syncthreads();
        bool ok = true;
        long long tc_a = TICK(), tc_trsm = 0, tc_p1 = 0, tc_p2 = 0, tc_potrf0 = 0;
        if (wave == 0) { bool o = potrf_tile_wave(s_T + tile_index(0, 0) * 256, s_invd, lane); if (lane == 0) s_flag[2] = o ? 1 : 0; }
        __syncthreads();
        { long long t = TICK(); tc_potrf0 = t - tc_a; tc_a = t; }
        for (int k = 0; k < VB_NTILE; k++) {
            if (!s_flag[2]) { ok = false; break; }
            const double *Tkk = s_T + tile_index(k, k) * 256;
            const int nrows = (VB_NTILE - 1 - k) * 16;
            if (tid < nrows) {
                const int ti = k + 1 + (tid >> 4), rr = tid & 15;
                double *Tik = s_T + tile_index(ti, k) * 256;
                double x[16];
#pragma unroll
                for (int c = 0; c < 16; c++) x[c] = Tik[TIX(rr, c)];
#pragma unroll
                for (int c = 0; c < 16; c++) {
                    double s = x[c];
#pragma unroll
                    for (int p = 0; p < c; p++) s -= x[p] * Tkk[TIX(c, p)];
                    x[c] = s * s_invd[16 * k + c];
                }
#pragma unroll
                for (int c = 0; c < 16; c++) Tik[TIX(rr, c)] = x[c];
            }
            __syncthreads();
            { long long t = TICK(); tc_trsm += t - tc_a; tc_a = t; }
            if (k == VB_NTILE - 1) break;
            const int nt = VB_NTILE - 1 - k;
            auto update_tile = [&](int ti, int tj) {
                double *C = s_T + tile_index(ti, tj) * 256;
                const double *A = s_T + tile_index(ti, k) * 256, *Bm = s_T + tile_index(tj, k) * 256;
                double4_t acc;
                double av[4], bv[4];
#pragma unroll
                for (int q = 0; q < 4; q++) acc[q] = C[TIX((lane >> 4) + 4 * q, lane & 15)];
#pragma unroll
                for (int s4 = 0; s4 < 4; s4++) { av[s4] = -A[TIX(lane & 15, 4 * s4 + (lane >> 4))]; bv[s4] = Bm[TIX(lane & 15, 4 * s4 + (lane >> 4))]; }
#pragma unroll
                for (int s4 = 0; s4 < 4; s4++) acc = __builtin_amdgcn_mfma_f64_16x16x4f64(av[s4], bv[s4], acc, 0, 0, 0);
#pragma unroll
                for (int q = 0; q < 4; q++) C[TIX((lane >> 4) + 4 * q, lane & 15)] = acc[q];
            };
            for (int ii = wave; ii < nt; ii += SNW) update_tile(k + 1 + ii, k + 1);
            __syncthreads();
            { long long t = TICK(); tc_p1 += t - tc_a; tc_a = t; }
            if (wave == 0) {
                bool o = potrf_tile_wave(s_T + tile_index(k + 1, k + 1) * 256, s_invd + 16 * (k + 1), lane);
                if (lane == 0) s_flag[2] = o ? 1 : 0;
            } else {
                const int nrest = (nt - 1) * nt / 2;
                for (int tt = wave - 1; tt < nrest; tt += SNW - 1) {
                    int ii = 0; while ((ii + 1) * (ii + 2) / 2 <= tt) ii++;
                    const int jj = tt - ii * (ii + 1) / 2;
                    update_tile(k + 2 + ii, k + 2 + jj);
                }
            }
            __syncthreads();
            { long long t = TICK(); tc_p2 += t - tc_a; tc_a = t; }
        }
        if (b.dbg && blockIdx.x == 0 && tid == 0) { b.dbg[64 + 20] = tc_potrf0; b.dbg[64 + 21] = tc_trsm; b.dbg[64 + 22] = tc_p1; b.dbg[64 + 23] = tc_p2; }
        STAMP(1, 6);
        tries++;
        if (ok) { solved = true; break; }
        mu *= 10.0;
        if (!(mu < 1.0)) break;
        __syncthreads();
    }
    if (!solved) {
        if (tid == 0) { st->solve_failed = 1; st->mu = mu; st->num_linear_solves += tries; st->scaling_ready = 1; st->grad_sqnorm = G2; st->Jg2 = Jg2; }
        return;
    }
    if (tid < VB_P) s_y[tid] = s_T[tile_index(10, tid >> 4) * 256 + TIX(5, tid & 15)];
    if (tid >= VB_P && tid < VB_NPAD) s_y[tid] = 0.0;
    __syncthreads();
    if (tid < 16) { if (tid == 5) s_T[tile_index(10, 10) * 256 + TIX(5, 5)] = 1.0; if (tid < 5) s_T[tile_index(10, 10) * 256 + TIX(5, tid)] = 0.0; }
    if (tid >= 16 && tid < 16 + 160) { const int c = tid - 16; s_T[tile_index(10, c >> 4) * 256 + TIX(5, c & 15)] = 0.0; }
    if (tid == 0) s_invd[165] = 1.0;
    __syncthreads();
    if (wave == 0) {
        const int l16 = lane & 15;
        for (int k = VB_NTILE - 1; k >= 0; k--) {
            const double *Tkk = s_T + tile_index(k, k) * 256;
            double Lc[16];
#pragma unroll
            for (int j = 0; j < 16; j++) Lc[j] = Tkk[TIX(j, l16)];
            double x = s_y[16 * k + l16];
            const double myinv = s_invd[16 * k + l16];
            double xs[16];
#pragma unroll
            for (int j = 15; j >= 0; j--) {
                if (l16 == j) x *= myinv;
                xs[j] = readlane_f64(x, j);
                if (l16 < j) x -= Lc[j] * xs[j];
            }
            if (lane < 16) s_y[16 * k + lane] = x;
            for (int col = lane; col < 16 * k; col += 64) {
                const double *T = s_T + tile_index(k, col >> 4) * 256;
                double sacc = 0;
#pragma unroll
                for (int r2 = 0; r2 < 16; r2++) sacc += T[TIX(r2, col & 15)] * xs[r2];
                s_y[col] -= sacc;
            }
            __builtin_amdgcn_fence(__ATOMIC_ACQ_REL, "wavefront");
            __builtin_amdgcn_wave_barrier();
        }
    }
    __syncthreads();
    STAMP(1, 7);
    double gy = 0, gn2 = 0;
    if (tid < VB_P) {
        const double y = s_y[tid], d = s_diag[tid];
        gn_g[tid] = -d * y;
        gy += s_g[tid] * y;
        gn2 += d * d * y * y;
    }
    if (tid < 80) s_v[tid] = (tid < VB_NPOSE) ? s_scale[tid] * s_y[tid] : 0.0;
    __syncthreads();
    feature_dots(W, F, s_v, s_cf, tid);
    __syncthreads();
#pragma unroll
    for (int u = 0; u < 2; u++) {
        const int f = tid + u * SNT;
        if (f >= F || f_const[f]) continue;
        const double sf = scale_g[VB_P + f], df = diag_g[VB_P + f];
        const double hp = sf * sf * hf[f] + mu * df * df;
        const double gt = sf * gf[f];
        const double y = (gt - sf * s_cf[f]) / hp;
        gn_g[VB_P + f] = -df * y;
        gy += gt * y;
        gn2 += df * df * y * y;
    }
    gy = block_sum_s(gy, s_red);
    gn2 = block_sum_s(gn2, s_red);
    if (tid == 0) {
        st->grad_sqnorm = G2; st->Jg2 = Jg2; st->alpha = G2 / Jg2;
        st->gy = gy; st->gn_sqnorm = gn2; st->mu = mu; st->mu_used = mu;
        st->num_linear_solves += tries; st->solve_failed = 0; st->reuse = 1; st->scaling_ready = 1;
    }
    STAMP(1, 8);
}

typedef unsigned int uint2_t __attribute__((ext_vector_type(2)));
__device__ __forceinline__ __amdgpu_buffer_rsrc_t sb_rsrc(const double *p, unsigned bytes) { return __builtin_amdgcn_make_buffer_rsrc((void *)p, 0, (int)bytes, 0x00027000); }
__device__ __forceinline__ double sb_bload(__amdgpu_buffer_rsrc_t r, int elem) {
    const uint2_t v = __builtin_amdgcn_raw_buffer_load_b64(r, elem < 0 ? 0x7ffffff0u : 8u * (unsigned)elem, 0, 0);
    return __hiloint2double((int)v.y, (int)v.x);
}
#define SBW (SBT / 64)
__device__ __forceinline__ double block_sum_sb(double v, double *s_red) {
    const int tid = threadIdx.x;
    v = vilf_wave_sum64(v);
    __syncthreads();
    if ((tid & 63) == 0) s_red[tid >> 6] = v;
    __syncthreads();
    double r = 0;
#pragma unroll
    for (int k = 0; k < SBW; k++) r += s_red[k];
    __syncthreads();
    return r;
}
__device__ __forceinline__ void block_sum2_sb(double v0, double v1, double *s_red, double &r0, double &r1) {
    const int tid = threadIdx.x;
    v0 = vilf_wave_sum64(v0); v1 = vilf_wave_sum64(v1);
    __syncthreads();
    if ((tid & 63) == 0) { s_red[tid >> 6] = v0; s_red[8 + (tid >> 6)] = v1; }
    __syncthreads();
    r0 = 0; r1 = 0;
#pragma unroll
    for (int k = 0; k < SBW; k++) { r0 += s_red[k]; r1 += s_red[8 + k]; }
    __syncthreads();
}
__device__ __forceinline__ int sb_prow(int r) { return r * (r + 1) / 2; }
__device__ __forceinline__ int sb_band_pos(int a, int c) {
    if (c < VB_NPOSE) { const int p = c - 6 * (a - 1); return (p >= 0 && p < 18) ? p : -1; }
    if (c < SB_ND) return (a == 1) ? 18 + (c - VB_NPOSE) : -1;
    return (c == SB_ND) ? SB_BRHS(a) : -1;
}

__device__ __forceinline__ constexpr int sb_t15_a(int i) { constexpr int T[15] = {0, 1, 1, 2, 2, 2, 3, 3, 3, 3, 4, 4, 4, 4, 4}; return T[i]; }
__device__ __forceinline__ constexpr int sb_t15_b(int i) { constexpr int T[15] = {0, 0, 1, 0, 1, 2, 0, 1, 2, 3, 0, 1, 2, 3, 4}; return T[i]; }
__device__ __forceinline__ constexpr int sb_y_ntl(int wv) { return wv == 3 ? 3 : 4; }
__device__ __forceinline__ constexpr int sb_y_ct(int wv, int k) { constexpr int T[4][3] = {{0, 1, 2}, {1, 2, 3}, {0, 3, 4}, {1, 2, 4}}; return T[wv][k]; }
__device__ __forceinline__ constexpr int sb_y_pa(int wv, int i) { constexpr int T[4][4] = {{0, 1, 1, 2}, {1, 1, 2, 2}, {1, 1, 2, 2}, {2, 2, 2, 2}}; return T[wv][i]; }
__device__ __forceinline__ constexpr int sb_y_pb(int wv, int i) { constexpr int T[4][4] = {{0, 0, 1, 0}, {0, 1, 0, 1}, {0, 1, 0, 1}, {0, 1, 2, 2}}; return T[wv][i]; }

__device__ __forceinline__ void sb_feature_reduce(const double *W, const double *cf, int F, int wv, const double *s_scale, double4_t (&acc)[15], int lane) {
    const int c16 = lane & 15, g4 = lane >> 4;
    const int nsteps = ((F + 3) & ~3) / 4;
    if (wv >= nsteps) return;
    double sc5[5];
#pragma unroll
    for (int t5 = 0; t5 < 4; t5++) sc5[t5] = s_scale[16 * t5 + c16];
    sc5[4] = (c16 < 2) ? s_scale[64 + c16] : ((c16 == 11 || c16 == 12) ? 1.0 : 0.0);
    const int col4 = (c16 < 2) ? 64 + c16 : (c16 == 11 ? VB_NPOSE : (c16 == 12 ? VB_NPOSE + 1 : VB_NPOSE + 2));
    double r0[5], r1[5], r2[5], r3[5], r4[5], c0, c1, c2, c3, c4;
#define SBF_ISSUE(ST, R, C)                                                                                                        \
    {                                                                                                                              \
        const int row_ = 4 * min((ST), nsteps - 1) + g4;                                                                           \
        const double *p0_ = W + (size_t)row_ * VB_WLD + c16, *p4_ = W + (size_t)row_ * VB_WLD + col4, *pc_ = cf + row_;             \
        asm volatile("global_load_dwordx2 %0, %6, off\n\tglobal_load_dwordx2 %1, %6, off offset:128\n\t"                           \
                     "global_load_dwordx2 %2, %6, off offset:256\n\tglobal_load_dwordx2 %3, %6, off offset:384\n\t"                \
                     "global_load_dwordx2 %4, %7, off\n\tglobal_load_dwordx2 %5, %8, off"                                          \
                     : "=&v"(R[0]), "=&v"(R[1]), "=&v"(R[2]), "=&v"(R[3]), "=&v"(R[4]), "=&v"(C) : "v"(p0_), "v"(p4_), "v"(pc_) : "memory"); \
    }
#define SBF_WAIT(N, R, C) asm volatile("s_waitcnt vmcnt(" #N ")" : "+v"(R[0]), "+v"(R[1]), "+v"(R[2]), "+v"(R[3]), "+v"(R[4]), "+v"(C) : : "memory");
#define SBF_STEP(R, C)                                                                                                             \
    {                                                                                                                              \
        double u[5];                                                                                                               \
        _Pragma("unroll") for (int t5 = 0; t5 < 5; t5++) u[t5] = R[t5] * C * sc5[t5];                                              \
        _Pragma("unroll") for (int i = 0; i < 15; i++) acc[i] = __builtin_amdgcn_mfma_f64_16x16x4f64(u[sb_t15_a(i)], u[sb_t15_b(i)], acc[i], 0, 0, 0); \
    }
    asm volatile("s_waitcnt vmcnt(0)" ::: "memory");
    SBF_ISSUE(wv, r0, c0) SBF_ISSUE(wv + 3, r1, c1) SBF_ISSUE(wv + 6, r2, c2) SBF_ISSUE(wv + 9, r3, c3)
    for (int st = wv; st < nsteps; st += 15) {
        SBF_ISSUE(st + 12, r4, c4) SBF_WAIT(24, r0, c0) SBF_STEP(r0, c0)
        if (st + 3 < nsteps) { SBF_ISSUE(st + 15, r0, c0) SBF_WAIT(24, r1, c1) SBF_STEP(r1, c1) }
        if (st + 6 < nsteps) { SBF_ISSUE(st + 18, r1, c1) SBF_WAIT(24, r2, c2) SBF_STEP(r2, c2) }
        if (st + 9 < nsteps) { SBF_ISSUE(st + 21, r2, c2) SBF_WAIT(24, r3, c3) SBF_STEP(r3, c3) }
        if (st + 12 < nsteps) { SBF_ISSUE(st + 24, r3, c3) SBF_WAIT(24, r4, c4) SBF_STEP(r4, c4) }
    }
    asm volatile("s_waitcnt vmcnt(0)" : "+v"(r0[0]), "+v"(r0[1]), "+v"(r0[2]), "+v"(r0[3]), "+v"(r0[4]), "+v"(r1[0]), "+v"(r1[1]), "+v"(r1[2]), "+v"(r1[3]), "+v"(r1[4]),
                                        "+v"(r2[0]), "+v"(r2[1]), "+v"(r2[2]), "+v"(r2[3]), "+v"(r2[4]), "+v"(r3[0]), "+v"(r3[1]), "+v"(r3[2]), "+v"(r3[3]), "+v"(r3[4]),
                                        "+v"(r4[0]), "+v"(r4[1]), "+v"(r4[2]), "+v"(r4[3]), "+v"(r4[4]), "+v"(c0), "+v"(c1), "+v"(c2), "+v"(c3), "+v"(c4) : : "memory");
#undef SBF_ISSUE
#undef SBF_WAIT
#undef SBF_STEP
}
template <int NTL, int PA, int PB>
__device__ __forceinline__ void sb_acc_sub(double *s_P, double *s_t, const double4_t *a, int lane, bool cauchy, double *s_dump) {
    const int c16 = lane & 15, g4 = lane >> 4;
    double v[NTL][4]; int off[NTL][4];
#pragma unroll
    for (int i = 0; i < NTL; i++)
#pragma unroll
        for (int q = 0; q < 4; q++) {
            const int r = 16 * ((PA >> (4 * i)) & 15) + g4 + 4 * q, c = 16 * ((PB >> (4 * i)) & 15) + c16;
            int o = (int)(s_dump - s_P) + lane;
            if (r < SB_NR && c <= r && c < SB_ND) o = sb_prow(r) + c;
            else if (cauchy && r == SB_NR && c < SB_ND) o = (int)(s_t - s_P) + c;
            off[i][q] = o;
            v[i][q] = s_P[o];
        }
#pragma unroll
    for (int i = 0; i < NTL; i++)
#pragma unroll
        for (int q = 0; q < 4; q++) s_P[off[i][q]] = v[i][q] - a[i][q];
}
template <int WV>
__device__ __forceinline__ void sb_y_chain(const double *s_band, const double *s_E, const double *s_zero, double4_t (&acc)[4], int lane) {
    const int c16 = lane & 15, g4 = lane >> 4;
    double4_t t[3];
#pragma unroll
    for (int ct = 0; ct < 3; ct++) t[ct] = double4_t{0, 0, 0, 0};
#pragma unroll 1
    for (int a = SB_NCH; a >= 1; a--) {
        const double *Ba = s_band + SB_BOFF(a);
        const int str = SB_BSTR(a);
        double yo[3][3];
#pragma unroll
        for (int ct = 0; ct < 3; ct++) {
            const int p = sb_band_pos(a, 16 * sb_y_ct(WV, ct) + c16);
#pragma unroll
            for (int ks = 0; ks < 3; ks++) {
                const int r = 4 * ks + g4;
                const double v = *((r < 9 && p >= 0) ? Ba + r * str + p : s_zero);
                yo[ks][ct] = v - t[ct][ks];
            }
        }
        if (a > 1) {
            const double *Na = s_E + 81 * (a - 2);
            double av[3];
// ... 63 lines not shown
            t[39 + 2 * u + 1] = 900 * (a1 + 1) + 30 * (21 + i) + 6 + j;
        }
    } else {
        for (int u = 0; u < 4; u++) {
            const int q = min(td + 192 * u, 755), nb = q / 36, e = q - 36 * nb, l1 = e / 6, l2 = e - 6 * l1;
            const bool dg = nb < 11;
            const int A = dg ? nb : nb - 10, Bf = dg ? nb : nb - 11, r = 6 * A + l1, c = 6 * Bf + l2;
            const int i0 = dg ? 900 * (A - 1) + 30 * (15 + l1) + 15 + l2 : 900 * Bf + 30 * (15 + l1) + l2, i1i = 900 * A + 30 * l1 + l2;
            const int j0 = dg ? 144 * (A - 1) + 12 * (6 + l1) + 6 + l2 : 144 * Bf + 12 * (6 + l1) + l2, j1 = 144 * A + 12 * l1 + l2;
            const bool h0 = !dg || A >= 1, h1 = dg && A <= 9;
            t[6 * u] = SB_META(SB_OFF_P + sb_prow(r) + c, r, c, td + 192 * u < 756 && c <= r);
            t[6 * u + 1] = 36 * (A * (A + 1) / 2 + Bf) + e;
            t[6 * u + 2] = h0 ? i0 : -1; t[6 * u + 3] = h1 ? i1i : -1; t[6 * u + 4] = h0 ? j0 : -1; t[6 * u + 5] = h1 ? j1 : -1;
        }
        for (int u = 0; u < 9; u++) {
            const int q = min(td + 192 * u, 1619), fb = q / 36, e = q - 36 * fb, l1 = e / 6, l2 = e - 6 * l1;
            int A2 = 0; while ((A2 + 1) * (A2 + 2) / 2 <= fb) A2++;
            const int Bf = fb - A2 * (A2 + 1) / 2, A = A2 + 2, r = 6 * A + l1, c = 6 * Bf + l2;
            t[24 + 2 * u] = SB_META(SB_OFF_P + sb_prow(r) + c, r, c, td + 192 * u < 1620);
            t[24 + 2 * u + 1] = 36 * (A * (A + 1) / 2 + Bf) + e;
        }
        for (int u = 0; u < 4; u++) {
            const int q = min(td + 192 * u, 674), i = q / 75, c = q - 75 * i, r = VB_NPOSE + i, Bf = c / 6, l2 = c - 6 * Bf;
            const int src = (c < VB_NPOSE) ? 30 * (6 + i) + (Bf == 0 ? l2 : 15 + l2) : 30 * (6 + i) + 6 + (c - VB_NPOSE);
            const bool hs = c >= VB_NPOSE || Bf <= 1;
            t[44 + 2 * u] = SB_META(SB_OFF_P + sb_prow(r) + c, r, c, td + 192 * u < 675 && c <= r);
            t[44 + 2 * u + 1] = hs ? src : -1;
        }
        for (int u = 0; u < 13; u++) {
            const int q = min(td + 192 * u, 2429), a1 = q / 243, rem = q - 243 * a1, i = rem / 27, pos = rem - 27 * i, a = a1 + 1;
            const int seg = pos / 6, m = pos - 6 * seg;
            const bool on = td + 192 * u < 2430 && (seg < 2 || (seg == 2 && a <= 9) || (seg >= 3 && a == 1));
            int s0, s1 = -1, c165;
            if (seg == 0) { s0 = 900 * a1 + 30 * (21 + i) + m; c165 = 6 * a1 + m; }
            else if (seg == 1) { s0 = 900 * a1 + 30 * (21 + i) + 15 + m; s1 = (a <= 9) ? 900 * a + 30 * (6 + i) + m : -1; c165 = 6 * a + m; }
            else if (seg == 2) { s0 = 900 * min(a, 9) + 30 * (6 + i) + 15 + m; c165 = 6 * (a + 1) + m; }
            else { s0 = 30 * (21 + i) + 6 + (pos - 18); c165 = VB_NPOSE + (pos - 18); }
            t[52 + 3 * u] = SB_META(SB_OFF_BAND + SB_BOFF(a) + i * SB_BSTR(a) + pos, VB_NPOSE + 9 * a + i, c165, on);
            t[52 + 3 * u + 1] = on ? s0 : -1;
            t[52 + 3 * u + 2] = s1;
        }
    }
    for (int k = 0; k < SB_TAB_ROWS; k++) for (int j = 0; j < 4; j++) tab[((size_t)k * 256 + tid) * 4 + j] = t[4 * k + j];
}

__device__ __forceinline__ void solve_sb_body(const VbBatch &b, int w) {
    const int tid = threadIdx.x, lane = tid & 63, wave = __builtin_amdgcn_readfirstlane(tid >> 6);
    if (w < 0) return;
    VbState *st = b.st + w;
    extern __shared__ double s_dyn[];
    double *s_P = s_dyn + SB_OFF_P, *s_D = s_dyn + SB_OFF_D, *s_E = s_dyn + SB_OFF_E, *s_band = s_dyn + SB_OFF_BAND;
    double *s_g = s_dyn + SB_OFF_VEC, *s_diag = s_g + SB_VLD, *s_scale = s_diag + SB_VLD, *s_y = s_scale + SB_VLD, *s_v = s_y + SB_VLD;
    double *s_t = s_dyn + SB_OFF_T, *s_linv = s_dyn + SB_OFF_LINV, *s_dinv = s_dyn + SB_OFF_DINV, *s_pan = s_dyn + SB_OFF_PAN, *s_u = s_dyn + SB_OFF_U, *s_w = s_dyn + SB_OFF_W;
    double *s_red = s_dyn + SB_OFF_RED;
    __shared__ int s_pcp[VB_P];
    __shared__ int s_flag[4];

    if (tid == 0) {
        const int done = st->done, iteration = st->iteration, reuse = st->reuse;
        const double gmn = st->gradient_max_norm, radius = st->radius;
        int go = 1;
        if (done) go = 0;
        else if (iteration >= b.max_iterations) { st->done = 1; st->termination = 0; go = 0; }
        else if (gmn <= b.gradient_tolerance) { st->done = 1; st->termination = 3; go = 0; }
        else if (radius <= b.min_radius) { st->done = 1; st->termination = 4; go = 0; }
        if (go) st->iteration = iteration + 1;
        s_flag[0] = go;
        s_flag[1] = go ? reuse : 1;
    }
    __syncthreads();
    if (!s_flag[0] || s_flag[1]) return;

    STAMP(1, 0);
    const int F = b.n_feat[w];
    const size_t FM = b.Fmax;
    const size_t ww = (size_t)st->ws * b.B + w;
    const double *Hpp = b.Hpp + ww * 66 * 36;
    const double *imuH = b.imuH + ww * 9000, *lidH = b.lidH + ww * 1440;
    const double *priorH = b.prior_H + (size_t)w * VB_PRIOR_LD * VB_PRIOR_LD;
    double *W = b.W + ww * FM * VB_WLD;
    double *cf = b.cf + (size_t)w * FM;
    const double *hf = b.hf + ww * FM, *gf = b.gf + ww * FM;
    const uint8_t *f_const = b.f_const + (size_t)w * FM;
    double *scale_g = b.scale + (size_t)w * (VB_P + FM), *diag_g = b.diag + (size_t)w * (VB_P + FM);
    double *grad_g = b.grad + (size_t)w * (VB_P + FM), *gn_g = b.gn + (size_t)w * (VB_P + FM);
    const double *g_in = b.g + ww * VB_P;
    const int *phdr = b.prior_hdr + (size_t)w * VB_PRIOR_HDR;
    const bool has_prior = phdr[0] != 0;
    const __amdgpu_buffer_rsrc_t rHpp = sb_rsrc(Hpp, 66 * 36 * 8), rImu = sb_rsrc(imuH, 9000 * 8), rLid = sb_rsrc(lidH, 1440 * 8), rPri = sb_rsrc(priorH, VB_PRIOR_LD * VB_PRIOR_LD * 8);

    for (int i = tid; i < SB_NCH * 81; i += SBT) s_D[i] = 0.0;
    for (int i = tid; i < 252 + 180 * (SB_NCH - 1); i += SBT) s_band[i] = 0.0;
    if (tid < 80) s_t[tid] = 0.0;
    if (tid == 0) s_P[sb_prow(SB_ND) + SB_ND] = 0.0;
    if (tid < VB_P) s_pcp[tid] = -1;
    __syncthreads();
    if (has_prior && tid < phdr[2]) {
        const int id = phdr[3 + tid], idx = phdr[51 + tid];
        if (id < VB_NF) { for (int k = 0; k < 6; k++) s_pcp[6 * id + k] = idx + k; }
        else if (id == VB_NF) { for (int k = 0; k < 9; k++) s_pcp[VB_NPOSE + k] = idx + k; }
    }
    const int scaling_ready = st->scaling_ready;
    double mu = st->mu;
    int tries = 0;
    bool solved = false;
    double Jg2 = 0, G2 = 0, g2 = 0;
    if (tid < VB_P) {
        int a, l; unperm(tid, a, l);
        const double dh = b.diagH[ww * VB_P + 15 * a + l];
        double sc;
        if (scaling_ready) sc = scale_g[tid]; else { sc = 1.0 / (1.0 + sqrt(dh)); scale_g[tid] = sc; }
        const double d = sqrt(fmin(fmax(sc * sc * dh, b.min_lm_diagonal), b.max_lm_diagonal));
        const double gs = g_in[15 * a + l] * sc;
        diag_g[tid] = d;
        const double gr = gs / d;
        grad_g[tid] = gr;
        g2 = gr * gr;
        s_scale[tid] = sc; s_diag[tid] = d; s_g[tid] = gs; s_v[tid] = gr / d;
    }
    for (int f = tid; f < F; f += SBT) {
        if (f_const[f]) continue;
        const double hfv = hf[f], gfv = gf[f];
        double sf;
        if (scaling_ready) sf = scale_g[VB_P + f]; else { sf = 1.0 / (1.0 + sqrt(hfv)); scale_g[VB_P + f] = sf; }
        const double d = sqrt(fmin(fmax(sf * sf * hfv, b.min_lm_diagonal), b.max_lm_diagonal));
        diag_g[VB_P + f] = d;
        const double gr = sf * gfv / d;
        grad_g[VB_P + f] = gr;
        g2 += gr * gr;
    }
    __threadfence_block();
    __syncthreads();
    int blk_i = 0;
    while ((blk_i + 1) * (blk_i + 2) / 2 <= tid) blk_i++;
    const int blk_j = tid - blk_i * (blk_i + 1) / 2;

    STAMP(1, 1);
    for (;;) {
        int ln = lane, bi = blk_i, bjm = blk_j, td = tid;
        asm volatile("" : "+v"(ln), "+v"(bi), "+v"(bjm), "+v"(td));
        double part = 0;
        if (td == 0) s_flag[2] = 1;
        if (wave == 3) {
            {
                double sv[25][2]; int meta[25];
                int ti[64];
                {
                    const int4 *tp = reinterpret_cast<const int4 *>(b.sb_tab) + td;
#pragma unroll
                    for (int k = 0; k < 16; k++) { const int4 v = tp[k * 256]; ti[4 * k] = v.x; ti[4 * k + 1] = v.y; ti[4 * k + 2] = v.z; ti[4 * k + 3] = v.w; }
                }
#pragma unroll
                for (int u = 0; u < 13; u++) {
                    sv[u][0] = sb_bload(rImu, ti[3 * u + 1]);
                    sv[u][1] = sb_bload(rImu, ti[3 * u + 2]);
                    meta[u] = ti[3 * u];
                }
#pragma unroll
                for (int u = 0; u < 12; u++) {
                    sv[13 + u][0] = sb_bload(rImu, ti[39 + 2 * u + 1]);
                    sv[13 + u][1] = 0.0;
                    meta[13 + u] = ti[39 + 2 * u];
                }
#pragma unroll
                for (int u = 0; u < 25; u++) {
                    if (meta[u] < 0) continue;
// ... 27 lines not shown
                    int r = 0; while ((r + 1) * (r + 2) / 2 <= ln) r++;
                    const int cc = ln - r * (r + 1) / 2;
                    double s = 0;
#pragma unroll
                    for (int i = 0; i < 9; i++) s += Ea[9 * i + r] * Ea[9 * i + cc];
                    s_D[81 * (a - 2) + 9 * r + cc] -= s;
                }
            }
            if (!ok && ln == 0) s_flag[2] = 0;
        } else {
            int tb[48];
            {
                constexpr int KN = 4, KF = 9, KT = KN + KF;
                double sn[KN][6], sf[KF][2];
                int meta[KT];
                int ti[44];
                {
                    const int4 *tp = reinterpret_cast<const int4 *>(b.sb_tab) + td;
#pragma unroll
                    for (int k = 0; k < 11; k++) { const int4 v = tp[k * 256]; ti[4 * k] = v.x; ti[4 * k + 1] = v.y; ti[4 * k + 2] = v.z; ti[4 * k + 3] = v.w; }
#pragma unroll
                    for (int k = 0; k < 12; k++) { const int4 v = tp[(11 + k) * 256]; tb[4 * k] = v.x; tb[4 * k + 1] = v.y; tb[4 * k + 2] = v.z; tb[4 * k + 3] = v.w; }
                }
#pragma unroll
                for (int u = 0; u < KN; u++) {
                    const int m = ti[6 * u], pr = s_pcp[(m >> 14) & 255], pc = s_pcp[(m >> 22) & 255];
                    sn[u][0] = sb_bload(rHpp, ti[6 * u + 1]);
                    sn[u][1] = sb_bload(rImu, ti[6 * u + 2]); sn[u][2] = sb_bload(rImu, ti[6 * u + 3]); sn[u][3] = sb_bload(rLid, ti[6 * u + 4]); sn[u][4] = sb_bload(rLid, ti[6 * u + 5]);
                    sn[u][5] = sb_bload(rPri, (pr >= 0 && pc >= 0) ? pr * VB_PRIOR_LD + pc : -1);
                    meta[u] = m;
                }
#pragma unroll
                for (int u = 0; u < KF; u++) {
                    const int m = ti[24 + 2 * u], pr = s_pcp[(m >> 14) & 255], pc = s_pcp[(m >> 22) & 255];
                    sf[u][0] = sb_bload(rHpp, ti[24 + 2 * u + 1]);
                    sf[u][1] = sb_bload(rPri, (pr >= 0 && pc >= 0) ? pr * VB_PRIOR_LD + pc : -1);
                    meta[KN + u] = m;
                }
                STAMP(1, 20);
#pragma unroll
                for (int u = 0; u < KT; u++) {
                    if (meta[u] < 0) continue;
                    const int r = (meta[u] >> 14) & 255, c = (meta[u] >> 22) & 255;
                    double raw;
                    if (u < KN) raw = ((((sn[u][0] + sn[u][1]) + sn[u][2]) + sn[u][3]) + sn[u][4]) + sn[u][5];
                    else raw = sf[u - KN][0] + sf[u - KN][1];
                    const double val = raw * s_scale[r] * s_scale[c];
                    part += ((r != c) ? 2.0 : 1.0) * s_v[r] * val * s_v[c];
                    s_dyn[meta[u] & 0x3fff] = val + ((r == c) ? mu : 0.0) * s_diag[r] * s_diag[r];
                }
            }
            STAMP(1, 21);
            {
                constexpr int KS = 4, KB2 = 13, KT = KS + KB2;
                double ss[KS][2], sb3[KB2][2];
                int meta[KT];
#pragma unroll
                for (int u = 0; u < KS; u++) {
                    const int m = tb[2 * u], pr = s_pcp[(m >> 14) & 255], pc = s_pcp[(m >> 22) & 255];
                    ss[u][0] = sb_bload(rImu, tb[2 * u + 1]);
                    ss[u][1] = sb_bload(rPri, (pr >= 0 && pc >= 0) ? pr * VB_PRIOR_LD + pc : -1);
                    meta[u] = m;
                }
#pragma unroll
                for (int u = 0; u < KB2; u++) {
                    sb3[u][0] = sb_bload(rImu, tb[8 + 3 * u + 1]);
                    sb3[u][1] = sb_bload(rImu, tb[8 + 3 * u + 2]);
                    meta[KS + u] = tb[8 + 3 * u];
                }
                STAMP(1, 22);
#pragma unroll
                for (int u = 0; u < KT; u++) {
                    if (meta[u] < 0) continue;
                    const int r = (meta[u] >> 14) & 255, c = (meta[u] >> 22) & 255;
                    const double raw = (u < KS) ? ss[u < KS ? u : 0][0] + ss[u < KS ? u : 0][1] : sb3[u >= KS ? u - KS : 0][0] + sb3[u >= KS ? u - KS : 0][1];
                    const double val = raw * s_scale[r] * s_scale[c];
                    part += ((r != c) ? 2.0 : 1.0) * s_v[r] * val * s_v[c];
                    s_dyn[meta[u] & 0x3fff] = val + ((r == c) ? mu : 0.0) * s_diag[r] * s_diag[r];
                }
            }
            STAMP(1, 23);
            if (td < SB_ND) s_P[sb_prow(SB_ND) + td] = s_g[td];
            if (td >= 96 && td < 96 + 9 * SB_NCH) { const int q = td - 96, a = q / 9 + 1, i = q - 9 * (a - 1); s_band[SB_BOFF(a) + i * SB_BSTR(a) + SB_BRHS(a)] = s_g[VB_NPOSE + 9 + q]; }
            for (int f = ln; f < ((F + 3) & ~3); f += 64) {
                double c = 0.0, xf = 0.0;
                if (f < F && !f_const[f]) {
                    const double sf = scale_g[VB_P + f], df = diag_g[VB_P + f], hfv = hf[f], gfv = gf[f];
                    const double hp = sf * sf * hfv + mu * df * df;
                    c = sf * rsqrt_nr(hp);
                    if (tries == 0) {
                        const double vf = sf * gfv / (df * df);
                        if (wave == 0) part += sf * sf * hfv * vf * vf;
                        xf = vf * hp / sf;
                    }
                }
                cf[f] = c;
                if (tries == 0 && f < F) W[(size_t)f * VB_WLD + VB_NPOSE + 1] = xf;
            }
            __threadfence_block();
        }
        STAMP(1, 2);
        STAMP(1, 24);
        double4_t acc15[15];
#pragma unroll
        for (int i = 0; i < 15; i++) acc15[i] = double4_t{0, 0, 0, 0};
        if (wave < 3) sb_feature_reduce(W, cf, F, wave, s_scale, acc15, ln);
#ifdef VILF_STAMPS
        if (b.dbg && blockIdx.x == 0 && (tid & 63) == 0) b.dbg[32 + 16 + (tid >> 6)] = __builtin_readcyclecounter();
#endif
        __syncthreads();
        STAMP(1, 3);
#define SB_P2B_GROUP(G) do { \
            if ((G) == 0) sb_acc_sub<3, 0x110, 0x100>(s_P, s_t, &acc15[0], ln, true, s_pan);        \
            else if ((G) == 1) sb_acc_sub<3, 0x222, 0x210>(s_P, s_t, &acc15[3], ln, true, s_pan);   \
            else if ((G) == 2) sb_acc_sub<3, 0x333, 0x210>(s_P, s_t, &acc15[6], ln, true, s_pan);   \
            else if ((G) == 3) sb_acc_sub<3, 0x443, 0x103>(s_P, s_t, &acc15[9], ln, true, s_pan);   \
            else sb_acc_sub<3, 0x444, 0x432>(s_P, s_t, &acc15[12], ln, true, s_pan);                \
        } while (0)
#pragma unroll
        for (int ph = 0; ph < 7; ph++) {
            if (wave == 0) { if (ph < 5) SB_P2B_GROUP(ph); }
            else if (wave == 1) { if (ph >= 1 && ph < 6) SB_P2B_GROUP(ph - 1); }
            else if (wave == 2) { if (ph >= 2) SB_P2B_GROUP(ph - 2); }
            lds_barrier();
        }
#undef SB_P2B_GROUP
        STAMP(1, 26);
        {
            double mx[9];
            {
                const int tt = min(td, 9 * SB_NCH - 1), a1 = tt / 9, c = tt - 9 * a1;
                const double *La = s_D + 81 * a1, *li = s_linv + 9 * a1;
#pragma unroll
                for (int i = 0; i < 9; i++) {
                    double sacc = (i == c) ? 1.0 : 0.0;
#pragma unroll
                    for (int j = 0; j < i; j++) sacc -= La[9 * i + j] * mx[j];
                    mx[i] = (i >= c) ? sacc * li[i] : 0.0;
                }
            }
            __syncthreads();
            if (td < 9 * SB_NCH) {
                const int a1 = td / 9, c = td - 9 * a1;
#pragma unroll
                for (int i = 0; i < 9; i++) if (i >= c) s_D[81 * a1 + 9 * i + c] = mx[i];
            }
            __syncthreads();
            if (td < 28 + 19 * (SB_NCH - 1)) {
                const int a = (td < 28) ? 1 : 2 + (td - 28) / 19, p = (td < 28) ? td : (td - 28) % 19;
                double *Bc = s_band + SB_BOFF(a) + p;
                const int str = SB_BSTR(a);
                const double *Ma = s_D + 81 * (a - 1);
                double bc[9], o[9];
#pragma unroll
                for (int kk = 0; kk < 9; kk++) bc[kk] = Bc[kk * str];
#pragma unroll
                for (int i = 0; i < 9; i++) {
                    double sacc = 0;
#pragma unroll
                    for (int kk = 0; kk <= i; kk++) sacc += Ma[9 * i + kk] * bc[kk];
                    o[i] = sacc;
                }
#pragma unroll
                for (int i = 0; i < 9; i++) Bc[i * str] = o[i];
            }
            __builtin_amdgcn_sched_barrier(0);
            double nv[3];
#pragma unroll
            for (int u = 0; u < 3; u++) {
                const int e = min(td + u * SBT, 81 * (SB_NCH - 1) - 1), a1 = e / 81, ij = e - 81 * a1, i = ij / 9, j = ij - 9 * i;
                const double *Ma = s_D + 81 * a1 + 9 * i, *Bn = s_E + 81 * a1 + 9 * j;
                double sacc = 0;
#pragma unroll
                for (int kk = 0; kk < 9; kk++) sacc += ((kk <= i) ? Ma[kk] : 0.0) * Bn[kk];
                nv[u] = sacc;
            }
            __syncthreads();
#pragma unroll
            for (int u = 0; u < 3; u++) { const int e = td + u * SBT; if (e < 81 * (SB_NCH - 1)) s_E[e] = nv[u]; }
        }
        STAMP(1, 27);
        if (tries == 0) block_sum2_sb(g2, part, s_red, G2, Jg2); else __syncthreads();
        if (tries == 0) {
            double cr = ((ln < VB_NPOSE) ? s_v[ln] * s_t[ln] : 0.0) + ((ln + 64 < VB_NPOSE) ? s_v[ln + 64] * s_t[ln + 64] : 0.0);
            cr = vilf_wave_sum64(cr);
            Jg2 -= 2.0 * cr;
        }
        STAMP(1, 4);
        double4_t acc[4];
// ... 112 lines not shown
            yb[1] = dv[2] * zb[1] + dv[4] * zb[2] + dv[7] * zb[3];
            yb[2] = dv[5] * zb[2] + dv[8] * zb[3];
            yb[3] = dv[9] * zb[3];
#pragma unroll
            for (int kk = 0; kk < 4; kk++) {
                z0 -= l0[kk] * yb[kk];
                if (lane + 64 < r0) z1 -= l1[kk] * yb[kk];
                if (lane + 64 == r0 + kk) z1 = yb[kk];
            }
        }
#pragma unroll 1
        for (int bj = 15; bj >= 0; bj--) {
            const int r0 = 4 * bj;
            double dv[10], l0[4];
#pragma unroll
            for (int q = 0; q < 10; q++) dv[q] = dvn[q];
#pragma unroll
            for (int kk = 0; kk < 4; kk++) l0[kk] = l0n[kk];
            if (bj > 0) {
                const double *d = s_dinv + 16 * (bj - 1);
                dvn[0] = d[0]; dvn[1] = d[4]; dvn[2] = d[5]; dvn[3] = d[8]; dvn[4] = d[9]; dvn[5] = d[10]; dvn[6] = d[12]; dvn[7] = d[13]; dvn[8] = d[14]; dvn[9] = d[15];
#pragma unroll
                for (int kk = 0; kk < 4; kk++) { const int r = r0 - 4 + kk; l0n[kk] = s_P[sb_prow(r) + min(lane, r)]; }
            }
            double zb[4], yb[4];
#pragma unroll
            for (int kk = 0; kk < 4; kk++) zb[kk] = readlane_f64(z0, r0 + kk);
            yb[0] = dv[0] * zb[0] + dv[1] * zb[1] + dv[3] * zb[2] + dv[6] * zb[3];
            yb[1] = dv[2] * zb[1] + dv[4] * zb[2] + dv[7] * zb[3];
            yb[2] = dv[5] * zb[2] + dv[8] * zb[3];
            yb[3] = dv[9] * zb[3];
            double upd = l0[0] * yb[0] + l0[1] * yb[1] + l0[2] * yb[2] + l0[3] * yb[3];
            const int kme = lane - r0;
            const double mine = (kme == 0) ? yb[0] : (kme == 1) ? yb[1] : (kme == 2) ? yb[2] : yb[3];
            z0 = (lane < r0) ? z0 - upd : ((kme >= 0 && kme < 4) ? mine : z0);
        }
        s_y[lane] = z0;
        if (lane + 64 < SB_ND) s_y[lane + 64] = z1;
    }
    __syncthreads();
    STAMP(1, 8);
    if (tid < 9 * SB_NCH) {
        const int a = tid / 9 + 1, i = tid - 9 * (a - 1);
        const double *Ba = s_band + SB_BOFF(a) + i * SB_BSTR(a);
        double sacc = Ba[SB_BRHS(a)];
#pragma unroll
        for (int p = 0; p < 18; p++) { const int c = 6 * (a - 1) + p; if (c < VB_NPOSE) sacc -= Ba[p] * s_y[c]; }
        if (a == 1) {
#pragma unroll
            for (int p = 0; p < 9; p++) sacc -= Ba[18 + p] * s_y[VB_NPOSE + p];
        }
        s_w[tid] = sacc;
    }
    if (tid >= 128 && tid < 128 + 80) { const int c = tid - 128; s_v[c] = (c < VB_NPOSE) ? s_scale[c] * s_y[c] : 0.0; }
    __syncthreads();
    if (wave == 0) {
        const int i9 = min(lane, 8);
        double un = 0.0;
#pragma unroll 1
        for (int a = SB_NCH; a >= 1; a--) {
            double t = s_w[9 * (a - 1) + i9];
            if (a < SB_NCH) {
                const double *Na = s_E + 81 * (a - 1) + 9 * i9;
#pragma unroll
                for (int j = 0; j < 9; j++) t -= Na[j] * readlane_f64(un, j);
            }
            un = t;
            if (lane < 9) s_u[9 * (a - 1) + i9] = t;
        }
        double wp = un;
        if (lane < 9) s_w[i9] = wp;
#pragma unroll 1
        for (int a = 1; a < SB_NCH; a++) {
            const double *Na = s_E + 81 * (a - 1);
            double t = s_u[9 * a + i9];
#pragma unroll
            for (int j = 0; j < 9; j++) t -= Na[9 * j + i9] * readlane_f64(wp, j);
            wp = t;
            if (lane < 9) s_w[9 * a + i9] = t;
        }
#ifdef VILF_STAMPS
        if (b.dbg && blockIdx.x == 0 && tid == 0) b.dbg[32 + 9] = __builtin_readcyclecounter();
#endif
    } else if (F > 0) {
        const int c16 = lane & 15, g = lane >> 4, w3 = wave - 1;
        double sv[5];
#pragma unroll
        for (int t5 = 0; t5 < 5; t5++) sv[t5] = s_v[16 * t5 + c16];
        const int Fk4 = (F + 3) & ~3;
        double ra[5], rb[5], rc[5];
#define FD_ISSUE(F0, R)                                                                                                            \
        {                                                                                                                          \
            const double *Wr_ = W + (size_t)min((F0) + g, Fk4 - 1) * VB_WLD + c16;                                                \
            asm volatile("global_load_dwordx2 %0, %5, off\n\tglobal_load_dwordx2 %1, %5, off offset:128\n\t"                       \
                         "global_load_dwordx2 %2, %5, off offset:256\n\tglobal_load_dwordx2 %3, %5, off offset:384\n\t"            \
                         "global_load_dwordx2 %4, %5, off offset:512"                                                              \
                         : "=&v"(R[0]), "=&v"(R[1]), "=&v"(R[2]), "=&v"(R[3]), "=&v"(R[4]) : "v"(Wr_) : "memory");                  \
        }
#define FD_WAIT(N, R) asm volatile("s_waitcnt vmcnt(" #N ")" : "+v"(R[0]), "+v"(R[1]), "+v"(R[2]), "+v"(R[3]), "+v"(R[4]) : : "memory");
#define FD_STEP(F0, R)                                                                                                             \
        {                                                                                                                          \
            const int f = (F0) + g;                                                                                                \
            double dacc = 0;                                                                                                       \
            _Pragma("unroll") for (int t5 = 0; t5 < 5; t5++) dacc += R[t5] * sv[t5];                                               \
            if (!(f < F)) dacc = 0;                                                                                                \
            _Pragma("unroll") for (int o = 8; o > 0; o >>= 1) dacc += __shfl_xor(dacc, o, 64);                                     \
            if (c16 == 0 && f < F) cf[f] = dacc;                                                                                   \
        }
        constexpr int RS = 4 * 3;
        asm volatile("s_waitcnt vmcnt(0)" ::: "memory");
        FD_ISSUE(4 * w3, ra) FD_ISSUE(4 * w3 + RS, rb)
        for (int f0 = 4 * w3; f0 < F; f0 += 3 * RS) {
            FD_ISSUE(f0 + 2 * RS, rc) FD_WAIT(10, ra) FD_STEP(f0, ra)
            if (f0 + RS < F) { FD_ISSUE(f0 + 3 * RS, ra) FD_WAIT(10, rb) FD_STEP(f0 + RS, rb) }
            if (f0 + 2 * RS < F) { FD_ISSUE(f0 + 4 * RS, rb) FD_WAIT(10, rc) FD_STEP(f0 + 2 * RS, rc) }
        }
        asm volatile("s_waitcnt vmcnt(0)" : "+v"(ra[0]), "+v"(ra[1]), "+v"(ra[2]), "+v"(ra[3]), "+v"(ra[4]), "+v"(rb[0]), "+v"(rb[1]), "+v"(rb[2]), "+v"(rb[3]), "+v"(rb[4]),
                                            "+v"(rc[0]), "+v"(rc[1]), "+v"(rc[2]), "+v"(rc[3]), "+v"(rc[4]) : : "memory");
#undef FD_ISSUE
#undef FD_WAIT
#undef FD_STEP
        __threadfence_block();
    }
    __syncthreads();
    if (tid < 9 * SB_NCH) {
        const int a1 = tid / 9, i = tid - 9 * a1;
        double s = 0;
#pragma unroll
        for (int k = 0; k < 9; k++) s += ((k >= i) ? s_D[81 * a1 + 9 * k + i] : 0.0) * s_w[9 * a1 + k];
        s_y[VB_NPOSE + 9 + tid] = s;
    }
    __syncthreads();
    STAMP(1, 10);
    double gy = 0, gn2 = 0;
    if (tid < VB_P) {
        const double y = s_y[tid], d = s_diag[tid];
        gn_g[tid] = -d * y;
        gy += s_g[tid] * y;
        gn2 += d * d * y * y;
    }
    for (int f = tid; f < F; f += SBT) {
        if (f_const[f]) continue;
        const double sf = scale_g[VB_P + f], df = diag_g[VB_P + f];
        const double hp = sf * sf * hf[f] + mu * df * df;
        const double gt = sf * gf[f];
        const double y = (gt - sf * cf[f]) / hp;
        gn_g[VB_P + f] = -df * y;
        gy += gt * y;
        gn2 += df * df * y * y;
    }
    block_sum2_sb(gy, gn2, s_red, gy, gn2);
    STAMP(1, 11);
    if (tid == 0) {
        st->grad_sqnorm = G2; st->Jg2 = Jg2; st->alpha = G2 / Jg2;
        st->gy = gy; st->gn_sqnorm = gn2; st->mu = mu; st->mu_used = mu;
        st->num_linear_solves += tries; st->solve_failed = 0; st->reuse = 1; st->scaling_ready = 1;
    }
}
extern "C" __global__ __launch_bounds__(SBT, 2) void k_solve_sb(VbBatch b) { solve_sb_body(b, vb_window(b)); }

extern "C" __global__ void k_finalize(VbBatch b) {
    const int w = blockIdx.x + b.w0, tid = threadIdx.x;
    if (tid >= VB_NF) return;
    const double *pose = b.pose + (size_t)w * 77, *sb = b.sb + (size_t)w * 99;
    const double *R0b = b.gauge_R0 + (size_t)w * 9, *P0b = b.gauge_P0 + (size_t)w * 3;
    double R00[9], y0[3], y00[3], rot[9];
    q_toR(q_load(pose + 3), R00);
    R2ypr(R0b, y0); R2ypr(R00, y00);
    double yd[3] = {y0[0] - y00[0], 0, 0};
    ypr2R(yd, rot);
    if (fabs(fabs(y0[1]) - 90) < 1.0 || fabs(fabs(y00[1]) - 90) < 1.0) {
        for (int i = 0; i < 3; i++) for (int j = 0; j < 3; j++) rot[3 * i + j] = R0b[3 * i] * R00[3 * j] + R0b[3 * i + 1] * R00[3 * j + 1] + R0b[3 * i + 2] * R00[3 * j + 2];
    }
    double Ri[9], Ro[9], d[3], o[3];
    q_toR(q_normalized(q_load(pose + 7 * tid + 3)), Ri);
    m3_mul(rot, Ri, Ro);
    for (int k = 0; k < 9; k++) b.out_Rs[((size_t)w * VB_NF + tid) * 9 + k] = Ro[k];
    d[0] = pose[7 * tid] - pose[0]; d[1] = pose[7 * tid + 1] - pose[1]; d[2] = pose[7 * tid + 2] - pose[2];
    m3_vec(rot, d, o);
    for (int k = 0; k < 3; k++) b.out_Ps[((size_t)w * VB_NF + tid) * 3 + k] = o[k] + P0b[k];
    m3_vec(rot, sb + 9 * tid, o);
    for (int k = 0; k < 3; k++) {
        b.out_Vs[((size_t)w * VB_NF + tid) * 3 + k] = o[k];
        b.out_Bas[((size_t)w * VB_NF + tid) * 3 + k] = sb[9 * tid + 3 + k];
        b.out_Bgs[((size_t)w * VB_NF + tid) * 3 + k] = sb[9 * tid + 6 + k];
    }
}

extern "C" __global__ void k_time_limit(VbBatch b, const int *mflag, int only_margin_old) {
    const int w = blockIdx.x + b.w0;
    if (threadIdx.x) return;
    if (only_margin_old && mflag[w] != 0) return;
    VbState *st = b.st + w;
    if (!st->done) { st->done = 1; st->termination = 0; }
}

extern "C" __global__ void k_reset(VbBatch b, int rewind_state) {
    const int w = blockIdx.x + b.w0, tid = threadIdx.x;
    if (blockIdx.x == 0 && b.live_ctl && tid < 128) b.live_ctl[tid] = 0;
    if (rewind_state) {
        if (tid < 77) b.pose[(size_t)w * 77 + tid] = b.pose_init[(size_t)w * 77 + tid];
        if (tid < 99) b.sb[(size_t)w * 99 + tid] = b.sb_init[(size_t)w * 99 + tid];
        for (int f = tid; f < b.Fmax; f += blockDim.x) b.feat[(size_t)w * b.Fmax + f] = b.feat_init[(size_t)w * b.Fmax + f];
    }
    if (tid == 0) {
        VbState s;
        s.x_cost = 0; s.cand_cost = 0; s.initial_cost = 0;
        s.radius = b.initial_radius; s.mu = 1e-8; s.alpha = 0; s.dogleg_step_norm = 0;
        s.x_norm = 0; s.gradient_max_norm = 1e300; s.grad_sqnorm = 0; s.Jg2 = 0; s.gy = 0; s.gn_sqnorm = 0; s.mu_used = 1e-8;
        s.model_cost_change = 0; s.relative_decrease = 0;
        s.iteration = 0; s.num_successful = 0; s.num_linear_solves = 0; s.num_consecutive_invalid = 0;
        s.termination = 0; s.done = 0; s.reuse = 0; s.need_linearize = 1; s.solve_failed = 0; s.scaling_ready = 0; s.started = 1; s.ws = 0; s.dev_error = 0;
        b.st[w] = s;
    }
}

extern "C" __global__ void k_hook_projection(const double *p0, const double *p1, const double *p2, double lam, const double *pi, const double *pj,
                                             double sqrt_info, double *out ) {
    if (threadIdx.x) return;
    double Ri[9], Rj[9], ric[9], pt[PT_LD];
    q_toR(q_load(p0 + 3), Ri); q_toR(q_load(p1 + 3), Rj); q_toR(q_load(p2 + 3), ric);
    pair_table(p0, Ri, p1, Rj, ric, p2, pt);
    projection_eval_pair<true>(pt, ric, p2, pi, pj, lam, sqrt_info, out, out + 2, out + 14, out + 26);
}
extern "C" __global__ void k_hook_projection_td(const double *in, double *out) {
    if (threadIdx.x) return;
    const double *p0 = in, *p1 = in + 7, *p2 = in + 14, *pi = in + 21, *pj = in + 24, *vi = in + 27, *vj = in + 29, *sc = in + 31;
    double Ri[9], Rj[9], ric[9];
    q_toR(q_load(p0 + 3), Ri); q_toR(q_load(p1 + 3), Rj); q_toR(q_load(p2 + 3), ric);
// ... 52 lines not shown
```

Measured before the change: 1.039 million.

## Compact W rows to non-constant features via host-built row map

```diff
diff --git a/vil_fusion_amd/csrc/vilf_api.hip b/vil_fusion_amd/csrc/vilf_api.hip
--- a/vil_fusion_amd/csrc/vilf_api.hip
+++ b/vil_fusion_amd/csrc/vilf_api.hip
@@ -30,6 +30,18 @@
     for (int p = 0; p < VB_NPAIR; p++) { cstart[p] = pos[cls[p]]; ccount[p] = pcount[p]; pos[cls[p]] += pcount[p]; }
     const int longest = std::max(std::max(pos[0], pos[1]), std::max(pos[2], pos[3]));
     return VB_CHUNK * std::max(1, (longest + VB_CLS - 1) / VB_CLS);
+}
+
+int w_row_map(int F, int cap, const unsigned char *fconst, int *f_wrow, int *row_feat) {
+    int cnt[3] = {0, 0, 0}, nsteps = 0;
+    for (int k = 0; k < cap; k++) row_feat[k] = -1;
+    for (int f = 0; f < F; f++) {
+        if (fconst[f]) { f_wrow[f] = -1; continue; }
+        const int c = (f >> 2) % 3, j = cnt[c]++, s = c + 3 * (j >> 2);
+        f_wrow[f] = 4 * s + (j & 3); row_feat[4 * s + (j & 3)] = f;
+        nsteps = std::max(nsteps, s + 1);
+    }
+    return 4 * nsteps;
 }
 
 void quat_from_R(const double *m, double *q ) {
@@ -318,11 +330,12 @@
 constexpr ArrayRow kBatchArrays[] = {
     {D_POSE, 8, VB_POSE_LD, 0, 0, 0, A_WINDOW, D_POSE0}, {D_SB, 8, VB_SB_LD, 0, 0, 0, A_WINDOW, D_SB0}, {D_FEAT, 8, 0, 1, 0, 0, A_WINDOW, D_FEAT0},
     {D_FSTART, 4, 0, 1, 0, 0, A_WINDOW}, {D_FNOBS, 4, 0, 1, 0, 0, A_WINDOW}, {D_FFAC0, 4, 0, 1, 0, 0, A_WINDOW}, {D_FCONST, 1, 0, 1, 0, 0, A_WINDOW}, {D_PSSLOT, 4, 0, 0, 0, 1, A_WINDOW},
+    {D_FWROW, 4, 0, 1, 0, 0, A_WINDOW}, {D_ROWFEAT, 4, 0, 1, 0, 0, A_WINDOW},
     {D_FOBS0, 4, 0, 1, 0, 0, A_WINDOW_TD}, {D_PSOBS, 4, 0, 0, 0, 1, A_WINDOW_TD},
     {D_FACREC, 8, 0, 0, 0, 8, A_WINDOW}, {D_IMU, 8, VB_IMU_LD, 0, 0, 0, A_WINDOW}, {D_LIDAR, 8, VB_LIDAR_LD, 0, 0, 0, A_WINDOW}, {D_COV, 8, VB_COV_LD, 0, 0, 0, A_WINDOW},
     {D_OBSV, 8, 0, 0, 2, 0, A_WINDOW_TD}, {D_OBSTD, 8, 0, 0, 1, 0, A_WINDOW_TD}, {D_OBSROW, 8, 0, 0, 1, 0, A_WINDOW_TD},
     {D_NFEAT, 4, 1, 0, 0, 0, A_SMALL}, {D_NFAC, 4, 1, 0, 0, 0, A_SMALL}, {D_EX, 8, VB_EX_LD, 0, 0, 0, A_SMALL}, {D_GR0, 8, 9, 0, 0, 0, A_SMALL}, {D_GP0, 8, 3, 0, 0, 0, A_SMALL},
-    {D_PAIROFF, 4, VB_PTAB, 0, 0, 0, A_SMALL}, {D_MFLAG, 4, 1, 0, 0, 0, A_SMALL}, {D_TD, 8, 1, 0, 0, 0, A_SMALL},
+    {D_PAIROFF, 4, VB_PTAB, 0, 0, 0, A_SMALL}, {D_MFLAG, 4, 1, 0, 0, 0, A_SMALL}, {D_TD, 8, 1, 0, 0, 0, A_SMALL}, {D_NROWS, 4, 1, 0, 0, 0, A_SMALL},
     {D_PHDR, 4, VB_PRIOR_HDR, 0, 0, 0, A_PRIOR, D_PHDR0}, {D_PX0, 8, VB_PRIOR_X0_LD, 0, 0, 0, A_PRIOR, D_PX00}, {D_PJ, 8, VB_PRIOR_LD * VB_PRIOR_LD, 0, 0, 0, A_PRIOR, D_PJ0},
     {D_PR, 8, VB_PRIOR_LD, 0, 0, 0, A_PRIOR, D_PR0}, {D_PH, 8, VB_PRIOR_LD * VB_PRIOR_LD, 0, 0, 0, A_PRIOR, D_PH0}, {D_PG, 8, VB_PRIOR_LD, 0, 0, 0, A_PRIOR, D_PG0},
     {D_CPOSE, 8, VB_POSE_LD, 0, 0, 0, A_WORK}, {D_CSB, 8, VB_SB_LD, 0, 0, 0, A_WORK}, {D_CFEAT, 8, 0, 1, 0, 0, A_WORK}, {D_CF, 8, 0, 1, 0, 0, A_WORK},
@@ -370,6 +383,7 @@
     b.pose_init = d[D_POSE0].as<double>(); b.sb_init = d[D_SB0].as<double>(); b.feat_init = d[D_FEAT0].as<double>();
     b.ex = d[D_EX].as<double>(); b.gauge_R0 = d[D_GR0].as<double>(); b.gauge_P0 = d[D_GP0].as<double>(); b.td = d[D_TD].as<double>();
     b.f_start = d[D_FSTART].as<int>(); b.f_nobs = d[D_FNOBS].as<int>(); b.f_obs0 = d[D_FOBS0].as<int>(); b.f_fac0 = d[D_FFAC0].as<int>(); b.f_const = d[D_FCONST].as<uint8_t>();
+    b.f_wrow = d[D_FWROW].as<int>(); b.row_feat = d[D_ROWFEAT].as<int>(); b.n_rows = d[D_NROWS].as<int>();
     b.obs_vel = d[D_OBSV].as<double>(); b.obs_ctd = d[D_OBSTD].as<double>(); b.obs_row = d[D_OBSROW].as<double>(); b.ps_obs = d[D_PSOBS].as<int>(); b.ps_slot = d[D_PSSLOT].as<int>();
     b.pair_off = d[D_PAIROFF].as<int>(); b.facrec = d[D_FACREC].as<double>(); b.imu = d[D_IMU].as<double>(); b.lidar = d[D_LIDAR].as<double>();
     bind_prior_pointers(h);
@@ -502,11 +516,14 @@
     int *psobs = u.dims.est_td ? u.row<int>(D_PSOBS, w) : nullptr, *fobs0 = u.dims.est_td ? u.row<int>(D_FOBS0, w) : nullptr;
     uint8_t *fconst = u.row<uint8_t>(D_FCONST, w);
     const unsigned long long nul = 1ULL << 17;
+    for (int f = 0; f < F; f++) fconst[f] = in.feature_const[f] ? 1 : 0;
+    int *fwrow = u.row<int>(D_FWROW, w);
+    *u.row<int>(D_NROWS, w) = w_row_map(F, (int)u.dims.F, fconst, fwrow, u.row<int>(D_ROWFEAT, w));
     for (int g = 0; g < pl.nslot; g++) { double *rec = &facrec[(size_t)g * 8]; for (int k = 0; k < 7; k++) rec[k] = 0.0; std::memcpy(&rec[7], &nul, 8); psslot[g] = 0; if (psobs) psobs[g] = 0; }
     int q = 0;
     for (int f = 0; f < F; f++) {
         const int o0 = in.feature_obs_offset[f], o1 = in.feature_obs_offset[f + 1], s = in.feature_start_frame[f], cst = in.feature_const[f] ? 1 : 0;
-        feat[f] = in.para_feature[f]; fconst[f] = (uint8_t)cst; fstart[f] = s; fnobs[f] = o1 - o0; ffac0[f] = q;
+        feat[f] = in.para_feature[f]; fstart[f] = s; fnobs[f] = o1 - o0; ffac0[f] = q;
         if (fobs0) fobs0[f] = o0;
         const double *pi = in.obs_point + 3 * (size_t)o0;
         for (int t = o0 + 1; t < o1; t++, q++) {
@@ -516,7 +533,7 @@
             double *rec = &facrec[(size_t)pos * 8]; const double *pj = in.obs_point + 3 * (size_t)t;
             for (int k = 0; k < 3; k++) { rec[k] = pi[k]; rec[3 + k] = pj[k]; }
             const unsigned long long a = (unsigned long long)(unsigned)f | ((unsigned long long)(unsigned)q << 32);
-            const unsigned long long b2 = (unsigned long long)s | ((unsigned long long)j << 8) | ((unsigned long long)cst << 16);
+            const unsigned long long b2 = (unsigned long long)s | ((unsigned long long)j << 8) | ((unsigned long long)cst << 16) | (cst ? 0ULL : (unsigned long long)fwrow[f] << 18);
             std::memcpy(&rec[6], &a, 8); std::memcpy(&rec[7], &b2, 8);
         }
     }
@@ -643,6 +660,10 @@
     return VILF_OK;
 }
 
+extern "C" int vilf_debug_w_row_map(int F, int cap, const unsigned char *feature_const, int *f_wrow, int *row_feat) {
+    if (F < 0 || cap < ((F + 3) & ~3) || !f_wrow || !row_feat || (F && !feature_const)) return VILF_ERR_INVALID_ARGUMENT;
+    return w_row_map(F, cap, feature_const, f_wrow, row_feat);
+}
 extern "C" int vilf_debug_sort_pairs(vilf_handle *h, const void *keys, const int *vals, size_t n, int bits, int key64, void *keys_out, int *vals_out) {
     if (!h || !keys || !vals || !keys_out || !vals_out || n == 0) return VILF_ERR_INVALID_ARGUMENT;
     const size_t kb = key64 ? 8 : 4, tb = vilf_sort_temp_bytes(n, kb);
diff --git a/vil_fusion_amd/csrc/vilf_batch.hpp b/vil_fusion_amd/csrc/vilf_batch.hpp
--- a/vil_fusion_amd/csrc/vilf_batch.hpp
+++ b/vil_fusion_amd/csrc/vilf_batch.hpp
@@ -137,6 +137,7 @@
     const double *gauge_R0, *gauge_P0;
     const int *f_start, *f_nobs, *f_obs0, *f_fac0;
     const uint8_t *f_const;
+    const int *f_wrow, *row_feat, *n_rows;
     const double *obs;
     const double *obs_vel, *obs_ctd, *obs_row;
     double *td;
diff --git a/vil_fusion_amd/csrc/vilf_internal.hpp b/vil_fusion_amd/csrc/vilf_internal.hpp
--- a/vil_fusion_amd/csrc/vilf_internal.hpp
+++ b/vil_fusion_amd/csrc/vilf_internal.hpp
@@ -29,6 +29,7 @@
     D_SCALE, D_DIAG, D_GRAD, D_GN, D_ST, D_OPS, D_ORS, D_OVS, D_OBAS, D_OBGS, D_COV, D_WORK, D_HOOK, D_DBG, D_LUTI, D_LUTL, D_LUTV,
     D_MFLAG, D_MINFO, D_MF0, D_MSTP, D_MSTS, D_MSTF, D_MSTE, D_MBUF, D_MHD, D_MGD, D_MWF, D_MHF, D_MGF, D_MAMM, D_MX, D_MROT, D_MLAM, D_MAR, D_MBR, D_QLV, D_QLD, D_QLLOG, D_QLIT, D_QLINFO,
     D_PAIRD, D_FACREC, D_CF, D_STAMPS, D_LIVE, D_SBTAB, D_SPLITC, D_SPLITB, D_UPSTAGE, D_DNSTAGE, D_OBSV, D_OBSTD, D_OBSROW, D_TD, D_PHDR0, D_PX00, D_PJ0, D_PR0, D_PH0, D_PG0,
+    D_FWROW, D_ROWFEAT, D_NROWS,
     D_COUNT
 };
 
diff --git a/vil_fusion_amd/csrc/vilf_kernels.hip b/vil_fusion_amd/csrc/vilf_kernels.hip
--- a/vil_fusion_amd/csrc/vilf_kernels.hip
+++ b/vil_fusion_amd/csrc/vilf_kernels.hip
@@ -618,7 +618,7 @@
         if (tid >= VB_CHUNK) {
         } else if (q < nfac && !((ib >> 17) & 1)) {
             const double pts_i[3] = {ra[0], ra[1], ra[2]}, pts_j[3] = {ra[3], rb[0], rb[1]};
-            const int f = (int)(ia & 0xffffffffu), slot = (int)(ia >> 32), fi = (int)(ib & 0xff), fj = (int)((ib >> 8) & 0xff);
+            const int slot = (int)(ia >> 32), fi = (int)(ib & 0xff), fj = (int)((ib >> 8) & 0xff);
             const bool fc = ((ib >> 16) & 1) != 0;
             double r[2], Ji[12], Jj[12], Jf[2];
             projection_eval_pair<true>(s_pt + PT_LD * pair_index(fi, fj), s_ric, s_tic, pts_i, pts_j, fv, b.sqrt_info, r, Ji, Jj, Jf);
@@ -630,7 +630,7 @@
             x0[12] = sw * r[0]; x1[12] = sw * r[1];
             if (!fc) {
                 const double jf0 = sw * Jf[0], jf1 = sw * Jf[1];
-                double2_t *Wr = reinterpret_cast<double2_t *>(W + (size_t)f * VB_WLD + 6 * fj);
+                double2_t *Wr = reinterpret_cast<double2_t *>(W + (size_t)(ib >> 18) * VB_WLD + 6 * fj);
                 double2_t *fw = reinterpret_cast<double2_t *>(facw + (size_t)slot * VB_FACW);
 #pragma unroll
                 for (int c = 0; c < 6; c += 2) {
@@ -782,7 +782,7 @@
     }
     LSTAMP(6);
     {
-        const int *f_nobs = b.f_nobs + (size_t)w * FM, *f_fac0 = b.f_fac0 + (size_t)w * FM;
+        const int *f_nobs = b.f_nobs + (size_t)w * FM, *f_fac0 = b.f_fac0 + (size_t)w * FM, *f_wrow = b.f_wrow + (size_t)w * FM;
         double *hf = b.hf + ww * FM, *gf = b.gf + ww * FM;
         for (int f = tid; f < F; f += NT) {
             if (f_const[f]) { hf[f] = 0; gf[f] = 0; continue; }
@@ -802,7 +802,7 @@
                     for (int c = 0; c < 8; c++) acc[c] += v[u][c];
                 }
             }
-            double *Wr = W + (size_t)f * VB_WLD;
+            double *Wr = W + (size_t)f_wrow[f] * VB_WLD;
 #pragma unroll
             for (int c = 0; c < 6; c++) Wr[6 * f_start[f] + c] = acc[c];
             Wr[VB_NPOSE] = acc[7];
@@ -975,12 +975,12 @@
 
 
 template <int HALF>
-__device__ __forceinline__ void schur_mfma(const double *W, int F, const double *s_cf, const double *s_scale, double *s_T, double *s_y, int lane, int wave) {
+__device__ __forceinline__ void schur_mfma(const double *W, int NR, const double *s_cf, const double *s_scale, double *s_T, double *s_y, int lane, int wave) {
     constexpr int TA[15] = {0, 1, 1, 2, 2, 2, 3, 3, 3, 3, 4, 4, 4, 4, 4};
     constexpr int TB[15] = {0, 0, 1, 0, 1, 2, 0, 1, 2, 3, 0, 1, 2, 3, 4};
     constexpr int NP = HALF ? 7 : 8, PB = HALF ? 8 : 0;
     const int c16 = lane & 15, grp = wave >> 1, g4 = lane >> 4;
-    const int nsteps = ((F + 3) & ~3) / 4;
+    const int nsteps = NR / 4;
     double *s_t = s_T + SOLVE_OFF_RED;
     double sc5[5];
 #pragma unroll
@@ -1007,7 +1007,7 @@
         _Pragma("unroll") for (int i = 0; i < NP; i++) acc[i] = __builtin_amdgcn_mfma_f64_16x16x4f64(u[TA[PB + i]], u[TB[PB + i]], acc[i], 0, 0, 0); \
     }
     asm volatile("s_waitcnt vmcnt(0)" ::: "memory");
-    SCHUR_ISSUE(grp, ra) SCHUR_ISSUE(grp + 4, rb)
+    if (nsteps > 0) { SCHUR_ISSUE(grp, ra) SCHUR_ISSUE(grp + 4, rb) }
     for (int st = grp; st < nsteps; st += 12) {
         SCHUR_ISSUE(st + 8, rc) SCHUR_WAIT(10, ra) SCHUR_STEP(st, ra)
         if (st + 4 < nsteps) { SCHUR_ISSUE(st + 12, ra) SCHUR_WAIT(10, rb) SCHUR_STEP(st + 4, rb) }
@@ -1038,16 +1038,16 @@
     }
 }
 
-__device__ __forceinline__ void feature_dots(const double *W, int F, const double *s_sv , double *out, int tid) {
+__device__ __forceinline__ void feature_dots(const double *W, int NR, const double *s_sv , double *out, int tid) {
+    if (NR <= 0) return;
     const int lane = tid & 63, wave = __builtin_amdgcn_readfirstlane(tid >> 6), c16 = lane & 15, g = lane >> 4;
     double sv[5];
 #pragma unroll
     for (int t5 = 0; t5 < 5; t5++) sv[t5] = s_sv[16 * t5 + c16];
-    const int Fk4 = (F + 3) & ~3;
     double ra[5], rb[5], rc[5];
 #define FD_ISSUE(F0, R)                                                                                                            \
     {                                                                                                                              \
-        const double *Wr_ = W + (size_t)min((F0) + g, Fk4 - 1) * VB_WLD + c16;                                                    \
+        const double *Wr_ = W + (size_t)min((F0) + g, NR - 1) * VB_WLD + c16;                                                    \
         asm volatile("global_load_dwordx2 %0, %5, off\n\tglobal_load_dwordx2 %1, %5, off offset:128\n\t"                           \
                      "global_load_dwordx2 %2, %5, off offset:256\n\tglobal_load_dwordx2 %3, %5, off offset:384\n\t"                \
                      "global_load_dwordx2 %4, %5, off offset:512"                                                                  \
@@ -1056,20 +1056,19 @@
 #define FD_WAIT(N, R) asm volatile("s_waitcnt vmcnt(" #N ")" : "+v"(R[0]), "+v"(R[1]), "+v"(R[2]), "+v"(R[3]), "+v"(R[4]) : : "memory");
 #define FD_STEP(F0, R)                                                                                                             \
     {                                                                                                                              \
-        const int f = (F0) + g;                                                                                                    \
+        const int k = (F0) + g;                                                                                                    \
         double acc = 0;                                                                                                            \
         _Pragma("unroll") for (int t5 = 0; t5 < 5; t5++) acc += R[t5] * sv[t5];                                                    \
-        if (!(f < F)) acc = 0;                                                                                                     \
         _Pragma("unroll") for (int o = 8; o > 0; o >>= 1) acc += __shfl_xor(acc, o, 64);                                           \
-        if (c16 == 0 && f < F) out[f] = acc;                                                                                       \
+        if (c16 == 0 && k < NR) out[k] = acc;                                                                                       \
     }
     constexpr int RS = 4 * SNW;
     asm volatile("s_waitcnt vmcnt(0)" ::: "memory");
     FD_ISSUE(4 * wave, ra) FD_ISSUE(4 * wave + RS, rb)
-    for (int f0 = 4 * wave; f0 < F; f0 += 3 * RS) {
+    for (int f0 = 4 * wave; f0 < NR; f0 += 3 * RS) {
         FD_ISSUE(f0 + 2 * RS, rc) FD_WAIT(10, ra) FD_STEP(f0, ra)
-        if (f0 + RS < F) { FD_ISSUE(f0 + 3 * RS, ra) FD_WAIT(10, rb) FD_STEP(f0 + RS, rb) }
-        if (f0 + 2 * RS < F) { FD_ISSUE(f0 + 4 * RS, rb) FD_WAIT(10, rc) FD_STEP(f0 + 2 * RS, rc) }
+        if (f0 + RS < NR) { FD_ISSUE(f0 + 3 * RS, ra) FD_WAIT(10, rb) FD_STEP(f0 + RS, rb) }
+        if (f0 + 2 * RS < NR) { FD_ISSUE(f0 + 4 * RS, rb) FD_WAIT(10, rc) FD_STEP(f0 + 2 * RS, rc) }
     }
     asm volatile("s_waitcnt vmcnt(0)" : "+v"(ra[0]), "+v"(ra[1]), "+v"(ra[2]), "+v"(ra[3]), "+v"(ra[4]), "+v"(rb[0]), "+v"(rb[1]), "+v"(rb[2]), "+v"(rb[3]), "+v"(rb[4]),
                                         "+v"(rc[0]), "+v"(rc[1]), "+v"(rc[2]), "+v"(rc[3]), "+v"(rc[4]) : : "memory");
@@ -1117,6 +1116,8 @@
     const double *hf = b.hf + ww * FM, *gf = b.gf + ww * FM;
     const uint8_t *f_const = b.f_const + (size_t)w * FM;
     const int *f_start = b.f_start + (size_t)w * FM, *f_nobs = b.f_nobs + (size_t)w * FM;
+    const int *f_wrow = b.f_wrow + (size_t)w * FM, *row_feat = b.row_feat + (size_t)w * FM;
+    const int NR = b.n_rows[w];
     double *scale_g = b.scale + (size_t)w * (VB_P + FM), *diag_g = b.diag + (size_t)w * (VB_P + FM);
     double *grad_g = b.grad + (size_t)w * (VB_P + FM), *gn_g = b.gn + (size_t)w * (VB_P + FM);
     const double *g_in = b.g + ww * VB_P;
@@ -1246,15 +1247,11 @@
 #pragma unroll
             for (int u = 0; u < 2; u++) {
                 const int f = tid + u * SNT;
-                if (f < F) {
-                    double xf = 0.0;
-                    if (!f_const[f]) {
-                        const double sf = scale_g[VB_P + f], df = diag_g[VB_P + f], hfv = hf[f], gfv = gf[f];
-                        const double vf = sf * gfv / (df * df);
-                        part += sf * sf * hfv * vf * vf;
-                        xf = vf * (sf * sf * hfv + mu * df * df) / sf;
-                    }
-                    W[(size_t)f * VB_WLD + VB_NPOSE + 1] = xf;
+                if (f < F && !f_const[f]) {
+                    const double sf = scale_g[VB_P + f], df = diag_g[VB_P + f], hfv = hf[f], gfv = gf[f];
+                    const double vf = sf * gfv / (df * df);
+                    part += sf * sf * hfv * vf * vf;
+                    W[(size_t)f_wrow[f] * VB_WLD + VB_NPOSE + 1] = vf * (sf * sf * hfv + mu * df * df) / sf;
                 }
             }
             __threadfence_block();
@@ -1266,16 +1263,16 @@
 #pragma unroll
         for (int u = 0; u < 2; u++) {
             const int f = tid + u * SNT;
-            if (f < F) { double c = 0; if (!f_const[f]) { const double sf = scale_g[VB_P + f], df = diag_g[VB_P + f]; c = sf * rsqrt_nr(sf * sf * hf[f] + mu * df * df); } s_cf[f] = c; }
+            if (f < F && !f_const[f]) { const double sf = scale_g[VB_P + f], df = diag_g[VB_P + f]; s_cf[f_wrow[f]] = sf * rsqrt_nr(sf * sf * hf[f] + mu * df * df); }
         }
         if (tid < VB_NPAD) s_y[tid] = s_g[tid];
         __syncthreads();
         STAMP(1, 4);
-        for (int f = F + tid; f < ((F + 3) & ~3); f += SNT) s_cf[f] = 0.0;
+        for (int k = tid; k < NR; k += SNT) if (row_feat[k] < 0) s_cf[k] = 0.0;
         if (tid < 80) s_red[tid] = 0.0;
         __syncthreads();
         __threadfence_block();
-        if (wave & 1) schur_mfma<1>(W, F, s_cf, s_scale, s_T, s_y, lane, wave); else schur_mfma<0>(W, F, s_cf, s_scale, s_T, s_y, lane, wave);
+        if (wave & 1) schur_mfma<1>(W, NR, s_cf, s_scale, s_T, s_y, lane, wave); else schur_mfma<0>(W, NR, s_cf, s_scale, s_T, s_y, lane, wave);
         if (tries == 0) {
             double cr = ((lane < VB_NPOSE) ? s_v[lane] * s_red[lane] : 0.0) + ((lane + 64 < VB_NPOSE) ? s_v[lane + 64] * s_red[lane + 64] : 0.0);
             cr = vilf_wave_sum64(cr);
@@ -1404,7 +1401,7 @@
     }
     if (tid < 80) s_v[tid] = (tid < VB_NPOSE) ? s_scale[tid] * s_y[tid] : 0.0;
     __syncthreads();
-    feature_dots(W, F, s_v, s_cf, tid);
+    feature_dots(W, NR, s_v, s_cf, tid);
     __syncthreads();
 #pragma unroll
     for (int u = 0; u < 2; u++) {
@@ -1413,7 +1410,7 @@
         const double sf = scale_g[VB_P + f], df = diag_g[VB_P + f];
         const double hp = sf * sf * hf[f] + mu * df * df;
         const double gt = sf * gf[f];
-        const double y = (gt - sf * s_cf[f]) / hp;
+        const double y = (gt - sf * s_cf[f_wrow[f]]) / hp;
         gn_g[VB_P + f] = -df * y;
         gy += gt * y;
         gn2 += df * df * y * y;
@@ -1472,9 +1469,9 @@
 __device__ __forceinline__ constexpr int sb_y_pa(int wv, int i) { constexpr int T[4][4] = {{0, 1, 1, 2}, {1, 1, 2, 2}, {1, 1, 2, 2}, {2, 2, 2, 2}}; return T[wv][i]; }
 __device__ __forceinline__ constexpr int sb_y_pb(int wv, int i) { constexpr int T[4][4] = {{0, 0, 1, 0}, {0, 1, 0, 1}, {0, 1, 0, 1}, {0, 1, 2, 2}}; return T[wv][i]; }
 
-__device__ __forceinline__ void sb_feature_reduce(const double *W, const double *cf, int F, int wv, const double *s_scale, double4_t (&acc)[15], int lane) {
+__device__ __forceinline__ void sb_feature_reduce(const double *W, const double *cf, int NR, int wv, const double *s_scale, double4_t (&acc)[15], int lane) {
     const int c16 = lane & 15, g4 = lane >> 4;
-    const int nsteps = ((F + 3) & ~3) / 4;
+    const int nsteps = NR / 4;
     if (wv >= nsteps) return;
     double sc5[5];
 #pragma unroll
@@ -1704,6 +1701,8 @@
     double *cf = b.cf + (size_t)w * FM;
     const double *hf = b.hf + ww * FM, *gf = b.gf + ww * FM;
     const uint8_t *f_const = b.f_const + (size_t)w * FM;
+    const int *f_wrow = b.f_wrow + (size_t)w * FM, *row_feat = b.row_feat + (size_t)w * FM;
+    const int NR = b.n_rows[w];
     double *scale_g = b.scale + (size_t)w * (VB_P + FM), *diag_g = b.diag + (size_t)w * (VB_P + FM);
     double *grad_g = b.grad + (size_t)w * (VB_P + FM), *gn_g = b.gn + (size_t)w * (VB_P + FM);
     const double *g_in = b.g + ww * VB_P;
@@ -1897,20 +1896,31 @@
             STAMP(1, 23);
             if (td < SB_ND) s_P[sb_prow(SB_ND) + td] = s_g[td];
             if (td >= 96 && td < 96 + 9 * SB_NCH) { const int q = td - 96, a = q / 9 + 1, i = q - 9 * (a - 1); s_band[SB_BOFF(a) + i * SB_BSTR(a) + SB_BRHS(a)] = s_g[VB_NPOSE + 9 + q]; }
-            for (int f = ln; f < ((F + 3) & ~3); f += 64) {
-                double c = 0.0, xf = 0.0;
-                if (f < F && !f_const[f]) {
-                    const double sf = scale_g[VB_P + f], df = diag_g[VB_P + f], hfv = hf[f], gfv = gf[f];
-                    const double hp = sf * sf * hfv + mu * df * df;
-                    c = sf * rsqrt_nr(hp);
-                    if (tries == 0) {
-                        const double vf = sf * gfv / (df * df);
-                        if (wave == 0) part += sf * sf * hfv * vf * vf;
-                        xf = vf * hp / sf;
+            for (int k0 = ln; k0 < NR; k0 += 256) {
+                int rf[4];
+#pragma unroll
+                for (int u = 0; u < 4; u++) rf[u] = row_feat[min(k0 + 64 * u, NR - 1)];
+                double sfu[4], dfu[4], hfu[4], gfu[4];
+#pragma unroll
+                for (int u = 0; u < 4; u++) { const int f = max(rf[u], 0); sfu[u] = scale_g[VB_P + f]; dfu[u] = diag_g[VB_P + f]; hfu[u] = hf[f]; gfu[u] = gf[f]; }
+#pragma unroll
+                for (int u = 0; u < 4; u++) {
+                    const int k = k0 + 64 * u;
+                    if (k >= NR) break;
+                    double c = 0.0, xf = 0.0;
+                    if (rf[u] >= 0) {
+                        const double sf = sfu[u], df = dfu[u], hfv = hfu[u], gfv = gfu[u];
+                        const double hp = sf * sf * hfv + mu * df * df;
+                        c = sf * rsqrt_nr(hp);
+                        if (tries == 0) {
+                            const double vf = sf * gfv / (df * df);
+                            if (wave == 0) part += sf * sf * hfv * vf * vf;
+                            xf = vf * hp / sf;
+                        }
                     }
-                }
-                cf[f] = c;
-                if (tries == 0 && f < F) W[(size_t)f * VB_WLD + VB_NPOSE + 1] = xf;
+                    cf[k] = c;
+                    if (tries == 0 && rf[u] >= 0) W[(size_t)k * VB_WLD + VB_NPOSE + 1] = xf;
+                }
             }
             __threadfence_block();
         }
@@ -1919,7 +1929,7 @@
         double4_t acc15[15];
 #pragma unroll
         for (int i = 0; i < 15; i++) acc15[i] = double4_t{0, 0, 0, 0};
-        if (wave < 3) sb_feature_reduce(W, cf, F, wave, s_scale, acc15, ln);
+        if (wave < 3) sb_feature_reduce(W, cf, NR, wave, s_scale, acc15, ln);
 #ifdef VILF_STAMPS
         if (b.dbg && blockIdx.x == 0 && (tid & 63) == 0) b.dbg[32 + 16 + (tid >> 6)] = __builtin_readcyclecounter();
 #endif
@@ -2198,16 +2208,15 @@
 #ifdef VILF_STAMPS
         if (b.dbg && blockIdx.x == 0 && tid == 0) b.dbg[32 + 9] = __builtin_readcyclecounter();
 #endif
-    } else if (F > 0) {
+    } else if (NR > 0) {
         const int c16 = lane & 15, g = lane >> 4, w3 = wave - 1;
         double sv[5];
 #pragma unroll
         for (int t5 = 0; t5 < 5; t5++) sv[t5] = s_v[16 * t5 + c16];
-        const int Fk4 = (F + 3) & ~3;
         double ra[5], rb[5], rc[5];
 #define FD_ISSUE(F0, R)                                                                                                            \
         {                                                                                                                          \
-            const double *Wr_ = W + (size_t)min((F0) + g, Fk4 - 1) * VB_WLD + c16;                                                \
+            const double *Wr_ = W + (size_t)min((F0) + g, NR - 1) * VB_WLD + c16;                                                \
             asm volatile("global_load_dwordx2 %0, %5, off\n\tglobal_load_dwordx2 %1, %5, off offset:128\n\t"                       \
                          "global_load_dwordx2 %2, %5, off offset:256\n\tglobal_load_dwordx2 %3, %5, off offset:384\n\t"            \
                          "global_load_dwordx2 %4, %5, off offset:512"                                                              \
@@ -2216,20 +2225,19 @@
 #define FD_WAIT(N, R) asm volatile("s_waitcnt vmcnt(" #N ")" : "+v"(R[0]), "+v"(R[1]), "+v"(R[2]), "+v"(R[3]), "+v"(R[4]) : : "memory");
 #define FD_STEP(F0, R)                                                                                                             \
         {                                                                                                                          \
-            const int f = (F0) + g;                                                                                                \
+            const int k = (F0) + g;                                                                                                \
             double dacc = 0;                                                                                                       \
             _Pragma("unroll") for (int t5 = 0; t5 < 5; t5++) dacc += R[t5] * sv[t5];                                               \
-            if (!(f < F)) dacc = 0;                                                                                                \
             _Pragma("unroll") for (int o = 8; o > 0; o >>= 1) dacc += __shfl_xor(dacc, o, 64);                                     \
-            if (c16 == 0 && f < F) cf[f] = dacc;                                                                                   \
+            if (c16 == 0 && k < NR) cf[k] = dacc;                                                                                   \
         }
         constexpr int RS = 4 * 3;
         asm volatile("s_waitcnt vmcnt(0)" ::: "memory");
         FD_ISSUE(4 * w3, ra) FD_ISSUE(4 * w3 + RS, rb)
-        for (int f0 = 4 * w3; f0 < F; f0 += 3 * RS) {
+        for (int f0 = 4 * w3; f0 < NR; f0 += 3 * RS) {
             FD_ISSUE(f0 + 2 * RS, rc) FD_WAIT(10, ra) FD_STEP(f0, ra)
-            if (f0 + RS < F) { FD_ISSUE(f0 + 3 * RS, ra) FD_WAIT(10, rb) FD_STEP(f0 + RS, rb) }
-            if (f0 + 2 * RS < F) { FD_ISSUE(f0 + 4 * RS, rb) FD_WAIT(10, rc) FD_STEP(f0 + 2 * RS, rc) }
+            if (f0 + RS < NR) { FD_ISSUE(f0 + 3 * RS, ra) FD_WAIT(10, rb) FD_STEP(f0 + RS, rb) }
+            if (f0 + 2 * RS < NR) { FD_ISSUE(f0 + 4 * RS, rb) FD_WAIT(10, rc) FD_STEP(f0 + 2 * RS, rc) }
         }
         asm volatile("s_waitcnt vmcnt(0)" : "+v"(ra[0]), "+v"(ra[1]), "+v"(ra[2]), "+v"(ra[3]), "+v"(ra[4]), "+v"(rb[0]), "+v"(rb[1]), "+v"(rb[2]), "+v"(rb[3]), "+v"(rb[4]),
                                             "+v"(rc[0]), "+v"(rc[1]), "+v"(rc[2]), "+v"(rc[3]), "+v"(rc[4]) : : "memory");
@@ -2256,11 +2264,12 @@
         gn2 += d * d * y * y;
     }
     for (int f = tid; f < F; f += SBT) {
-        if (f_const[f]) continue;
+        const int k = f_wrow[f];
+        if (k < 0) continue;
         const double sf = scale_g[VB_P + f], df = diag_g[VB_P + f];
         const double hp = sf * sf * hf[f] + mu * df * df;
         const double gt = sf * gf[f];
-        const double y = (gt - sf * cf[f]) / hp;
+        const double y = (gt - sf * cf[k]) / hp;
         gn_g[VB_P + f] = -df * y;
         gy += gt * y;
         gn2 += df * df * y * y;
```

Measured after the change: 1.062 million (median of 6 runs). 1.02x the previous value.
